# bwvdnbro/CMacIonize

Hardware: AMD Instinct MI355X
Metric: photon packets/sec, 256^3 stromgren (higher is better)
Workload: dtype f64

## Files before the change

### cmacionize_amd/csrc/engine.hip

```cpp
#include "../../include/cmi_gpu.h"

#include "atomic_data.h"
#include "linecooling_data.h"
#include "kernels.h"
#include "dust_kernels.h"
#include "line_image_kernels.h"
#include "line_cube_kernels.h"
#include "sky_image_kernels.h"
#include "sky_cube_kernels.h"
#include "dust_cube_kernels.h"
#include "continuum_kernels.h"
#include "absorbing_cube_kernels.h"
#include "lyman_alpha_kernels.h"
#include "absorption_kernels.h"
#include "sort.h"

#include <algorithm>
#include <climits>
#include <cmath>
#include <cstdarg>
#include <cstdlib>
#include <cstdio>
#include <cstring>
#include <new>
#include <string>
#include <type_traits>
#include <vector>

namespace {

thread_local std::string g_last_error;

int fail(int code, const char *fmt, ...) {
  char buf[512];
  va_list ap;
  va_start(ap, fmt);
  vsnprintf(buf, sizeof buf, fmt, ap);
  va_end(ap);
  g_last_error = buf;
  return code;
}

#define HIP_TRY(expr)                                                          \
  do {                                                                         \
    hipError_t err__ = (expr);                                                 \
    if (err__ != hipSuccess)                                                   \
      return fail(CMI_GPU_EDEVICE, "%s failed: %s (%s:%d)", #expr,             \
                  hipGetErrorString(err__), __FILE__, __LINE__);               \
  } while (0)
#define CMI_TRY(expr)                                                          \
  do {                                                                         \
    const int rc__ = (expr);                                                   \
    if (rc__)                                                                  \
      return rc__;                                                             \
  } while (0)

struct EventPair {
  hipEvent_t start = nullptr, stop = nullptr;
  uint64_t packets = 0;
};

}

struct cmi_gpu_engine {
  cmi_gpu_config config;
  int device = 0;
  hipStream_t stream = nullptr;
  bool own_stream = false;
  int num_cu = 0;

  GridDev grid;
  ModelDev model;
  CellsDev cells_unsettled;
  int64_t ncell = 0;

  double *state_block = nullptr;
  double *acc_block = nullptr;
  bool own_acc = false;
  double2 *opacity = nullptr;
  CountersDev *counters = nullptr;
  TablesDev *tables = nullptr;
  TablesDev *host_tables = nullptr;
  SpectraDev *spectra = nullptr;
  bool spectra_dirty = true;
  double *user_table[4] = {nullptr, nullptr, nullptr, nullptr};
  std::vector<double> user_table_host[4];
  unsigned int *mailbox = nullptr, *mailbox_dev = nullptr;
  double *source_position = nullptr;
  double *source_cumulative = nullptr;
  std::vector<double> source_position_host;
  double discrete_luminosity = 0., continuous_luminosity = 0.;
  bool have_continuous_spectrum = false;

  bool have_sources = false, have_spectrum = false, have_xsec = false,
       have_recomb = false, have_cells = false;
  bool full_ions = false;
  cmi_gpu_temperature_params tparams;

  unsigned int *select_count = nullptr;
  uint32_t *select_ids = nullptr;
  uint64_t select_capacity = 0;
  double *select_rows = nullptr;
  uint64_t select_rows_capacity = 0;
  uint32_t *sort_keys[2] = {nullptr, nullptr};
  uint32_t *sort_ids[2] = {nullptr, nullptr};
  void *sort_temp = nullptr;
  size_t sort_temp_bytes = 0;
  uint64_t sort_capacity = 0;
  uint32_t *span_cursor = nullptr;
#ifdef CMI_EXPERIMENTS
  unsigned long long *phase_clock = nullptr;
  size_t phase_clock_capacity = 0;
  unsigned phase_blocks = 0;
#endif

  double *queue_block = nullptr;
  uint64_t queue_capacity = 0;
  QueueDev ended_queue, ready_queue;
  double *export_rows = nullptr;
  uint64_t export_capacity = 0;
  unsigned int *export_count = nullptr;
  bool own_export_rows = false;
  double *import_rows = nullptr;
  uint64_t import_capacity = 0;
  unsigned int *queue_counts = nullptr;
  char *tile_block = nullptr;
  uint64_t tile_capacity = 0;
  bool tile_has_weights = false;
  FlightRowsDev tile_rows[2];
  uint32_t *tile_iota = nullptr;
  TileItemDev *tile_items = nullptr;
  uint32_t *tile_begin = nullptr;
  uint32_t *tile_blockhist = nullptr, *tile_total = nullptr;
  uint32_t *tile_new_slots = nullptr;
  TrackersDev trackers = {};
  bool trackers_enabled = false;
  EscapeDev escape = {};
  bool escape_counting = false;
  EscapeDev escape_staged = {};
  double *pad_H = nullptr;
  bool pad_valid = false;
  int32_t last_first_build = 0;
  bool last_pad_uniform = false;
  unsigned long long *metal_gate = nullptr;
  bool metals_pending = false;
  bool state_pointer_escaped = false;
  char *temp_pipe_block = nullptr;
  uint32_t temp_pipe_capacity = 0;
  unsigned int *temp_pipe_counts = nullptr;
  uint32_t *tile_ended_slot = nullptr;
  uint32_t *tile_ended_pos = nullptr;
  uint32_t *tile_slot_of[2] = {nullptr, nullptr};
  unsigned int *tile_absorbed_count = nullptr;
  unsigned int *tile_absorbed_before = nullptr;
  unsigned int *tile_counts = nullptr;
  uint64_t tile_rounds_run = 0;
  bool acc_block_dirty = false;

  struct Tuning {
    bool sort_packets = true;
    int sort_tau_bits = -1;
    int sort_dir_bits = -1;
    int class_order = -1;
    int aggregate = CMI_AGG_BLOCK;
    int aggregate_reemit = CMI_AGG_NONE;
    int refill_threshold = CMI_REFILL_THRESHOLD;
    uint32_t chunk = 64;
    int max_blocks_per_cu = 8;
    uint64_t max_packets_per_launch = 1ull << 27;
    int exp_no_atomics = 0;
    bool exact_dda = false;
    bool reemit_passes = true;
    int refill_threshold_reemit = 32;
    int64_t reemit_inline_below = -1;
    int reemit_max_passes = 12;
    bool tile_rounds = true;
    uint64_t tile_min_flights = 100000;
    int tile_min_per_item = -1;
    int tile_refill_threshold = 48;
    bool tile_counting_sort = true;
    bool update_reuse = true;
    bool defer_metals = true;
    bool update_writes_pad = true;
    bool defer_weights = true;
    bool pre_emission = true;
    bool pad_march = true;
    bool pad_uniform = true;
    bool xcd_remap = false;
    bool temperature_pipeline = true;
    uint32_t temperature_finish_slots = 1024;
    int tile_compact_ratio = -1;
    bool park_in_place = true;
    bool span_claim = CMI_SPAN_CLAIM_DEFAULT;
    bool emit_before_flush = CMI_EMIT_BEFORE_FLUSH_DEFAULT;
    bool phase_stamps = false;
    int continuum_channel_block = CMI_CONTINUUM_FB;
    int64_t continuum_launch_rays = 0;
    int absorbing_cube_channel_block = CMI_ABSORBING_CB;
    int absorbing_cube_expm1_call = CMI_ABSORBING_EXPM1_CALL;
    int absorbing_cube_window_skip = 1;
    int64_t absorbing_cube_launch_rays = 0;
    int absorption_slab_rows = 0;
    int absorption_edge_sharing = CMI_ABSORPTION_EDGE_SHARING;
    int absorption_skips = 1;
  } tune;

  DustDev dust = {};
  double dust_kappa = 0.;
  bool have_dust_scattering = false, have_ccd = false, have_dust_source = false;
  double *dust_image = nullptr;
  double *dust_cdf = nullptr;
  double2 *dust_opacity = nullptr;
  DustCountersDev *dust_counters = nullptr;
  bool dust_per_hydrogen = false;
  int dust_source = DUST_SOURCE_GALAXY;
  CellSourceDev cell_source = {};
  double *cell_source_cells = nullptr, *cell_source_blocks = nullptr;
  double *cell_velocities = nullptr;
  std::vector<double> cell_source_blocks_host;
  bool have_cell_source = false, cell_source_from_cells = false;
  uint64_t cells_epoch = 0, cell_source_epoch = 0;
  int dust_camera = DUST_CAMERA_PARALLEL;
  SkyCameraDev sky_camera = {};
  int32_t dust_nviews = 1, dust_probe_view = 0;
  std::vector<DustViewDev> dust_views;
  std::vector<SkyObserverDev> sky_views;
  void *dust_views_dev = nullptr;
  unsigned long long *dust_view_counters = nullptr;
  DustCubeDev dust_cube = {};
  int32_t dust_cube_nviews = 0;
  const char *dust_cube_stale = nullptr;
  int32_t cell_source_line = -1;
  LyaDev lya = {};
  DustDev lya_dust = {};
  int32_t lya_nviews = 0;
  unsigned long long *lya_next = nullptr;
  LyaCountersDev *lya_counters = nullptr;
  const char *lya_stale = nullptr;
  double *lya_field = nullptr;

  bool timing = false;
  unsigned long long *launch_steps = nullptr;
  std::vector<EventPair> shoot_events, update_events, kernel_events;
  std::vector<EventPair> event_pool;
};

namespace {

inline CellsDev &cells_of_iteration(cmi_gpu_engine *e) {
  return e->cells_unsettled;
}
inline const CellsDev &cells_of_iteration(const cmi_gpu_engine *e) {
  return e->cells_unsettled;
}

int settle_metal_fractions(cmi_gpu_engine *e);

template <class T, class N>
int grow(cmi_gpu_engine *e, T *&ptr, N &capacity, N want, size_t bytes) {
  if (capacity >= want)
    return CMI_GPU_OK;
  HIP_TRY(hipStreamSynchronize(e->stream));
  (void)hipFree(ptr);
  ptr = nullptr;
  capacity = 0;
  HIP_TRY(hipMalloc(&ptr, bytes));
  capacity = want;
  return CMI_GPU_OK;
}

#define CMI_MAX_TIMED_LAUNCHES 65536
int timer_begin(cmi_gpu_engine *e, EventPair &ev) {
  ev = EventPair();
  if (!e->timing)
    return CMI_GPU_OK;
  if (!e->event_pool.empty()) {
    ev = e->event_pool.back();
    e->event_pool.pop_back();
  } else {
    HIP_TRY(hipEventCreate(&ev.start));
    hipError_t err = hipEventCreate(&ev.stop);
    if (err != hipSuccess) {
      (void)hipEventDestroy(ev.start);
      HIP_TRY(err);
    }
  }
  hipError_t err = hipEventRecord(ev.start, e->stream);
  if (err != hipSuccess) {
    e->event_pool.push_back(ev);
    HIP_TRY(err);
  }
  return CMI_GPU_OK;
}

__global__ void mailbox_kernel(const unsigned int *src, unsigned int *dst,
                               int n) {
  if ((int)threadIdx.x < n)
    dst[threadIdx.x] = src[threadIdx.x];
}
__global__ void snapshot_steps_kernel(const CountersDev *counters,
                                      unsigned long long *dst) {
  unsigned long long sum = 0;
  for (int k = threadIdx.x; k < CMI_COUNTER_SHARDS; k += 64)
    sum += counters[k].nsteps;
  for (int off = 32; off > 0; off >>= 1)
    sum += __shfl_down(sum, off, 64);
  if (threadIdx.x == 0)
    *dst = sum;
}

__global__ void __launch_bounds__(256)
    counters_sum_kernel(const CountersDev *shards, CountersDev *out) {
  __shared__ CountersDev partial[256];
  CountersDev mine = CountersDev();
  for (int k = threadIdx.x; k < CMI_COUNTER_SHARDS; k += 256) {
    const CountersDev c = shards[k];
// ... 617 lines not shown
  if (config->stream) {
    e->stream = (hipStream_t)config->stream;
  } else {
    HIP_TRY(hipStreamCreateWithFlags(&e->stream, hipStreamNonBlocking));
    e->own_stream = true;
  }

  GridDev &g = e->grid;
  const bool decomposed = config->sub_ncell[0] > 0 || config->sub_ncell[1] > 0 ||
                          config->sub_ncell[2] > 0;
  for (int a = 0; a < 3; ++a) {
    g.anchor[a] = config->anchor[a];
    g.box_sides[a] = config->sides[a];
    g.global_ncell[a] = config->ncell[a];
    g.ncell[a] = decomposed ? config->sub_ncell[a] : config->ncell[a];
    g.offset[a] = decomposed ? config->sub_offset[a] : 0;
    g.global_periodic[a] = config->periodic[a] ? 1 : 0;
    g.periodic[a] = (config->periodic[a] && !decomposed) ? 1 : 0;
    g.cellside[a] = config->sides[a] / config->ncell[a];
    g.inv_cellside[a] = 1. / g.cellside[a];
  }
  g.decomposed = decomposed ? 1 : 0;
  g.copy_rank = 0;
  g.copy_count = 1;
  e->ncell = (int64_t)g.ncell[0] * g.ncell[1] * g.ncell[2];
  g.ncell_total = e->ncell;

  const size_t field_bytes = (size_t)e->ncell * sizeof(double);
  HIP_TRY(hipMalloc(&e->state_block, 16 * field_bytes));
  HIP_TRY(hipMemsetAsync(e->state_block, 0, 16 * field_bytes, e->stream));
  if (config->external_accumulators) {
    e->acc_block = (double *)config->external_accumulators;
  } else {
    HIP_TRY(hipMalloc(&e->acc_block, CMI_NACC * field_bytes));
    e->own_acc = true;
  }
  HIP_TRY(hipMemsetAsync(e->acc_block, 0, CMI_NACC * field_bytes, e->stream));
  HIP_TRY(hipMalloc(&e->opacity, (size_t)e->ncell * sizeof(double2)));
  HIP_TRY(hipMalloc(&e->counters, sizeof(CountersDev) * CMI_COUNTER_SHARDS +
                                      sizeof(EscapeDev)));
  HIP_TRY(hipMemsetAsync(e->counters, 0,
                         sizeof(CountersDev) * CMI_COUNTER_SHARDS +
                             sizeof(EscapeDev),
                         e->stream));
  HIP_TRY(hipMalloc(&e->tables, sizeof(TablesDev)));
  {
    e->host_tables = new TablesDev;
    build_tables(*e->host_tables);
    HIP_TRY(hipMemcpy(e->tables, e->host_tables, sizeof(TablesDev),
                      hipMemcpyHostToDevice));
  }

  CellsDev &c = cells_of_iteration(e);
  c.number_density = e->state_block;
  c.temperature = e->state_block + e->ncell;
  for (int i = 0; i < CMI_NION; ++i)
    c.x[i] = e->state_block + (int64_t)(2 + i) * e->ncell;
  c.acc_base = e->acc_block;
  c.acc_field_stride = e->ncell;
  c.acc_cell_stride = 1;
  c.opacity = e->opacity;

  ModelDev &m = e->model;
  memset(&m, 0, sizeof m);
  m.tables = e->tables;
  m.nu_H = eV_to_Hz(13.6);
  m.nu_He = eV_to_Hz(24.6);
  m.reemit_type = CMI_GPU_REEMIT_NONE;
  m.photon_weight[0] = 1.;
  m.photon_weight[1] = 1.;

  cmi_gpu_temperature_params &tp = e->tparams;
  tp.do_temperature_calculation = 0;
  tp.minimum_number_of_iterations = 3;
  tp.epsilon_convergence = 1.e-3;
  tp.maximum_number_of_iterations = 100;
  tp.pah_heating_factor = 0.;
  tp.cosmic_ray_heating_factor = 0.;
  tp.cosmic_ray_heating_limit = 0.75;
  tp.cosmic_ray_heating_scale_length = 1.33333 * 3.086e19;
  tp.minimum_ionized_temperature = 4000.;
  m.t_epsilon = tp.epsilon_convergence;
  m.t_max_iterations = tp.maximum_number_of_iterations;
  m.crlim = tp.cosmic_ray_heating_limit;
  m.crscale = tp.cosmic_ray_heating_scale_length;
  m.t_min_ionized = tp.minimum_ionized_temperature;

  HIP_TRY(hipStreamSynchronize(e->stream));
  if (const char *env = std::getenv("CMI_GPU_TUNING")) {
    std::string all(env);
    size_t at = 0;
    while (at < all.size()) {
      size_t end = all.find(',', at);
      if (end == std::string::npos)
        end = all.size();
      const std::string item = all.substr(at, end - at);
      const size_t eq = item.find('=');
      if (eq != std::string::npos) {
        const int rc = cmi_gpu_set_tuning(e, item.substr(0, eq).c_str(),
                                          std::atoll(item.c_str() + eq + 1));
        if (rc) {
          cmi_gpu_destroy(e);
          return rc;
        }
      }
      at = end + 1;
    }
  }
  *out = e;
  return CMI_GPU_OK;
}

int cmi_gpu_destroy(cmi_gpu_engine *e) {
  if (!e)
    return CMI_GPU_OK;
  (void)hipSetDevice(e->device);
  (void)hipStreamSynchronize(e->stream);
  release_events(e, e->shoot_events);
  release_events(e, e->update_events);
  release_events(e, e->kernel_events);
  for (auto &p : e->event_pool) {
    (void)hipEventDestroy(p.start);
    (void)hipEventDestroy(p.stop);
  }
  (void)hipFree(e->state_block);
  if (e->own_acc)
    (void)hipFree(e->acc_block);
  (void)hipFree(e->opacity);
  (void)hipFree(e->counters);
  (void)hipFree(e->trackers.counts);
  (void)hipFree(e->trackers.absorption);
  (void)hipFree(e->trackers.flux);
  (void)hipFree(e->escape.sky);
  (void)hipFree(e->temp_pipe_block);
  (void)hipFree(e->pad_H);
  (void)hipFree(e->metal_gate);
  (void)hipFree(e->temp_pipe_counts);
  (void)hipFree(e->tables);
  (void)hipFree(e->spectra);
  for (int k = 0; k < 4; ++k)
    (void)hipFree(e->user_table[k]);
  delete e->host_tables;
  (void)hipFree(e->source_position);
  (void)hipFree(e->source_cumulative);
  (void)hipFree(e->sort_keys[0]);
  (void)hipFree(e->select_count);
  (void)hipFree(e->span_cursor);
#ifdef CMI_EXPERIMENTS
  (void)hipFree(e->phase_clock);
#endif
  (void)hipFree(e->select_ids);
  (void)hipFree(e->select_rows);
  (void)hipFree(e->sort_temp);
  (void)hipFree(e->queue_block);
  (void)hipFree(e->queue_counts);
  if (e->mailbox)
    (void)hipHostFree(e->mailbox);
  (void)hipFree(e->export_count);
  if (e->own_export_rows)
    (void)hipFree(e->export_rows);
  (void)hipFree(e->import_rows);
  (void)hipFree(e->tile_block);
  (void)hipFree(e->tile_counts);
  (void)hipFree(e->launch_steps);
  (void)hipFree(e->dust_image);
  (void)hipFree(e->dust_views_dev);
  (void)hipFree(e->dust_view_counters);
  (void)hipFree(e->dust_cdf);
  (void)hipFree(e->dust_opacity);
  (void)hipFree(e->dust_counters);
  (void)hipFree(e->cell_source_cells);
  (void)hipFree(e->cell_velocities);
  (void)hipFree(const_cast<double *>(e->dust_cube.s2));
  (void)hipFree(const_cast<double *>(e->dust_cube.obs_velocity));
  (void)hipFree(e->dust_cube.cube);
  (void)hipFree(e->cell_source_blocks);
  (void)hipFree(const_cast<LyaRecord *>(e->lya.records));
  (void)hipFree(e->lya.image);
  (void)hipFree(e->lya.cube);
  (void)hipFree(e->lya_next);
  (void)hipFree(e->lya_counters);
  (void)hipFree(e->lya_field);
  if (e->own_stream)
    (void)hipStreamDestroy(e->stream);
  delete e;
  return CMI_GPU_OK;
}

int cmi_gpu_synchronize(cmi_gpu_engine *e) {
  if (!e)
    return fail(CMI_GPU_EINVAL, "null engine");
  HIP_TRY(hipStreamSynchronize(e->stream));
  return CMI_GPU_OK;
}

int64_t cmi_gpu_number_of_cells(const cmi_gpu_engine *e) {
  return e ? e->ncell : -1;
}

static void mix_sources(cmi_gpu_engine *e) {
  ModelDev &m = e->model;
  const double discrete = m.nsource > 0 ? e->discrete_luminosity : 0.;
  const double continuous =
      m.continuous_type != 0 ? e->continuous_luminosity : 0.;
  m.total_luminosity = discrete + continuous;
  m.continuous_probability = 0.;
  m.photon_weight[0] = 1.;
  m.photon_weight[1] = 1.;
  if (m.total_luminosity > 0.) {
    if (discrete > 0.) {
      m.continuous_probability = continuous > 0. ? 0.5 : 0.;
      m.photon_weight[0] = 1.;
      m.photon_weight[1] =
          continuous > 0. ? (1. - m.continuous_probability) * continuous /
                                m.continuous_probability / discrete
                          : 1.;
    } else {
      m.continuous_probability = 1.;
      m.photon_weight[0] = 0.;
      m.photon_weight[1] = 1.;
    }
  }
  e->have_sources = m.total_luminosity > 0.;
}

int cmi_gpu_set_sources(cmi_gpu_engine *e, int32_t n, const double *positions,
                        const double *weights, double total_luminosity) {
  if (!e || n < 0 || (n > 0 && (!positions || !weights)))
    return fail(CMI_GPU_EINVAL, "cmi_gpu_set_sources: bad argument");
  HIP_TRY(hipSetDevice(e->device));
  HIP_TRY(hipStreamSynchronize(e->stream));
  (void)hipFree(e->source_position);
  (void)hipFree(e->source_cumulative);
  e->source_position = nullptr;
  e->source_cumulative = nullptr;
  e->source_position_host.clear();
  e->model.nsource = 0;
  e->model.source_position = nullptr;
  e->model.source_cumulative = nullptr;
  e->discrete_luminosity = 0.;
  if (n == 0) {
    mix_sources(e);
    return CMI_GPU_OK;
  }
  std::vector<double> cumulative(n);
  for (int i = 0; i < n; ++i)
    cumulative[i] = (i > 0 ? cumulative[i - 1] : 0.) + weights[i];
  if (std::abs(cumulative.back() - 1.) > 1.e-9) {
    mix_sources(e);
    return fail(CMI_GPU_EINVAL,
                "Discrete source weights do not sum to 1.0 (%g)!",
                cumulative.back());
  }
  cumulative.back() = 1.;
  HIP_TRY(hipMalloc(&e->source_position, sizeof(double) * 3 * n));
  HIP_TRY(hipMalloc(&e->source_cumulative, sizeof(double) * n));
  HIP_TRY(hipMemcpy(e->source_position, positions, sizeof(double) * 3 * n,
                    hipMemcpyHostToDevice));
  HIP_TRY(hipMemcpy(e->source_cumulative, cumulative.data(),
                    sizeof(double) * n, hipMemcpyHostToDevice));
  e->source_position_host.assign(positions, positions + 3 * (size_t)n);
  e->model.nsource = n;
  e->model.source_position = e->source_position;
  e->model.source_cumulative = e->source_cumulative;
  e->discrete_luminosity = total_luminosity;
  mix_sources(e);
  return CMI_GPU_OK;
}

int cmi_gpu_set_continuous_source(cmi_gpu_engine *e, int32_t type,
                                  double luminosity) {
  if (!e || (type != CMI_GPU_CONTINUOUS_NONE &&
             type != CMI_GPU_CONTINUOUS_ISOTROPIC) ||
      (type != CMI_GPU_CONTINUOUS_NONE && !(luminosity > 0.)))
    return fail(CMI_GPU_EINVAL, "cmi_gpu_set_continuous_source: bad argument");
  e->model.continuous_type = type;
  e->continuous_luminosity = type != CMI_GPU_CONTINUOUS_NONE ? luminosity : 0.;
  e->spectra_dirty = true;
  mix_sources(e);
  return CMI_GPU_OK;
}

int cmi_gpu_set_continuous_source_planar(cmi_gpu_engine *e, int32_t axis,
                                         double intercept,
                                         const double *anchor,
                                         const double *sides,
                                         double luminosity) {
  if (!e || axis < 0 || axis > 2 || !anchor || !sides || !(sides[0] > 0.) ||
      !(sides[1] > 0.) || !(luminosity > 0.))
    return fail(CMI_GPU_EINVAL,
                "cmi_gpu_set_continuous_source_planar: bad argument");
  ModelDev &m = e->model;
  m.continuous_type = CMI_GPU_CONTINUOUS_PLANAR;
  m.continuous_axis = axis;
  m.continuous_intercept = intercept;
  for (int k = 0; k < 2; ++k) {
    m.continuous_anchor[k] = anchor[k];
    m.continuous_side[k] = sides[k];
  }
  e->continuous_luminosity = luminosity;
  e->spectra_dirty = true;
  mix_sources(e);
  return CMI_GPU_OK;
}

int cmi_gpu_set_continuous_spectrum_monochromatic(cmi_gpu_engine *e,
// ... 200 lines not shown
  m.t_min_ionized = params->minimum_ionized_temperature;
  return CMI_GPU_OK;
}

int cmi_gpu_upload_cells(cmi_gpu_engine *e, const double *number_density,
                         const double *temperature,
                         const double *ionic_fractions) {
  if (!e || !number_density || !temperature)
    return fail(CMI_GPU_EINVAL, "upload_cells: bad argument");
  HIP_TRY(hipSetDevice(e->device));
  ++e->cells_epoch;
  CellsDev *cells;
  CMI_TRY(cells_settled(e, cells));
  const size_t bytes = (size_t)e->ncell * sizeof(double);
  HIP_TRY(hipMemcpyAsync(cells->number_density, number_density, bytes,
                         hipMemcpyHostToDevice, e->stream));
  HIP_TRY(hipMemcpyAsync(cells->temperature, temperature, bytes,
                         hipMemcpyHostToDevice, e->stream));
  if (ionic_fractions) {
    HIP_TRY(hipMemcpyAsync(cells->x[0], ionic_fractions, CMI_NION * bytes,
                           hipMemcpyHostToDevice, e->stream));
  } else {
    HIP_TRY(hipMemsetAsync(cells->x[0], 0, CMI_NION * bytes, e->stream));
  }
  CMI_TRY(rebuild_opacity(e));
  HIP_TRY(hipStreamSynchronize(e->stream));
  e->have_cells = true;
  return CMI_GPU_OK;
}

int cmi_gpu_upload_field(cmi_gpu_engine *e, int32_t field,
                         const double *values) {
  if (!e || !values)
    return fail(CMI_GPU_EINVAL, "upload_field: bad argument");
  double *dst = field_pointer(e, field);
  if (!dst)
    return fail(CMI_GPU_EINVAL, "upload_field: unknown field %d", field);
  HIP_TRY(hipSetDevice(e->device));
  if (field < CMI_GPU_FIELD_MEAN_INTENSITY) {
    ++e->cells_epoch;
    CMI_TRY(settle_metal_fractions(e));
  }
  const int64_t stride = field_stride(e, field);
  if (stride == 1) {
    HIP_TRY(hipMemcpyAsync(dst, values, (size_t)e->ncell * sizeof(double),
                           hipMemcpyHostToDevice, e->stream));
  } else {
    double *tmp = nullptr;
    HIP_TRY(hipMalloc(&tmp, (size_t)e->ncell * sizeof(double)));
    hipError_t err = hipMemcpyAsync(tmp, values,
                                    (size_t)e->ncell * sizeof(double),
                                    hipMemcpyHostToDevice, e->stream);
    if (err == hipSuccess) {
      scatter_strided_kernel<<<grid_blocks(e, e->ncell, 8), CMI_BLOCK, 0,
                               e->stream>>>(tmp, dst, stride, e->ncell);
      err = hipGetLastError();
    }
    if (err == hipSuccess)
      err = hipStreamSynchronize(e->stream);
    (void)hipFree(tmp);
    HIP_TRY(err);
  }
  if (field >= CMI_GPU_FIELD_MEAN_INTENSITY)
    e->acc_block_dirty = true;
  if (field == CMI_GPU_FIELD_NUMBER_DENSITY ||
      field == CMI_GPU_FIELD_IONIC_FRACTION + ION_H_n ||
      field == CMI_GPU_FIELD_IONIC_FRACTION + ION_He_n) {
    CMI_TRY(rebuild_opacity(e));
  }
  HIP_TRY(hipStreamSynchronize(e->stream));
  return CMI_GPU_OK;
}

int cmi_gpu_download_field(cmi_gpu_engine *e, int32_t field, double *values) {
  if (!e || !values)
    return fail(CMI_GPU_EINVAL, "download_field: bad argument");
  double *src = field_pointer(e, field);
  if (!src)
    return fail(CMI_GPU_EINVAL, "download_field: unknown field %d", field);
  HIP_TRY(hipSetDevice(e->device));
  if (field >= CMI_GPU_FIELD_IONIC_FRACTION + ION_C_p1 &&
      field < CMI_GPU_FIELD_MEAN_INTENSITY)
    CMI_TRY(settle_metal_fractions(e));
  const int64_t stride = field_stride(e, field);
  if (stride == 1) {
    HIP_TRY(hipMemcpyAsync(values, src, (size_t)e->ncell * sizeof(double),
                           hipMemcpyDeviceToHost, e->stream));
    HIP_TRY(hipStreamSynchronize(e->stream));
  } else {
    double *tmp = nullptr;
    HIP_TRY(hipMalloc(&tmp, (size_t)e->ncell * sizeof(double)));
    gather_strided_kernel<<<grid_blocks(e, e->ncell, 8), CMI_BLOCK, 0,
                            e->stream>>>(src, stride, tmp, e->ncell);
    hipError_t err = hipGetLastError();
    if (err == hipSuccess)
      err = hipMemcpyAsync(values, tmp, (size_t)e->ncell * sizeof(double),
                           hipMemcpyDeviceToHost, e->stream);
    if (err == hipSuccess)
      err = hipStreamSynchronize(e->stream);
    (void)hipFree(tmp);
    HIP_TRY(err);
  }
  return CMI_GPU_OK;
}

int cmi_gpu_accumulator_layout(cmi_gpu_engine *e, int64_t *field_stride_out,
                               int64_t *cell_stride_out) {
  if (!e)
    return fail(CMI_GPU_EINVAL, "null engine");
  if (field_stride_out)
    *field_stride_out = cells_of_iteration(e).acc_field_stride;
  if (cell_stride_out)
    *cell_stride_out = cells_of_iteration(e).acc_cell_stride;
  return CMI_GPU_OK;
}

void *cmi_gpu_field_device_pointer(cmi_gpu_engine *e, int32_t field) {
  if (!e)
    return nullptr;
  if (field >= 0 && field < CMI_GPU_FIELD_MEAN_INTENSITY) {
    if (settle_metal_fractions(e) != CMI_GPU_OK)
      return nullptr;
    e->state_pointer_escaped = true;
  }
  return field_pointer(e, field);
}

int cmi_gpu_get_update_state(cmi_gpu_engine *e, int32_t *metals_pending,
                             int32_t *pad_records_valid,
                             int32_t *deferral_allowed) {
  if (!e)
    return fail(CMI_GPU_EINVAL, "null engine");
  if (metals_pending)
    *metals_pending = e->metals_pending ? 1 : 0;
  if (pad_records_valid)
    *pad_records_valid = e->pad_valid ? 1 : 0;
  if (deferral_allowed)
    *deferral_allowed =
        (e->tune.defer_metals && !e->state_pointer_escaped) ? 1 : 0;
  return CMI_GPU_OK;
}

int cmi_gpu_get_transport_plan(cmi_gpu_engine *e, int32_t *first_build,
                               int32_t *uniform_weight) {
  if (!e)
    return fail(CMI_GPU_EINVAL, "null engine");
  if (first_build)
    *first_build = e->last_first_build;
  if (uniform_weight)
    *uniform_weight = e->last_pad_uniform ? 1 : 0;
  return CMI_GPU_OK;
}

int cmi_gpu_reset_grid(cmi_gpu_engine *e) {
  if (!e)
    return fail(CMI_GPU_EINVAL, "null engine");
  HIP_TRY(hipSetDevice(e->device));
  const size_t field_bytes = (size_t)e->ncell * sizeof(double);
  if (e->full_ions || e->acc_block_dirty) {
    HIP_TRY(hipMemsetAsync(e->acc_block, 0, CMI_NACC * field_bytes,
                           e->stream));
    e->acc_block_dirty = false;
  } else {
    HIP_TRY(hipMemsetAsync(e->acc_block, 0, field_bytes, e->stream));
    if (e->config.track_heating)
      HIP_TRY(hipMemsetAsync(e->acc_block + (size_t)CMI_NION * e->ncell, 0,
                             2 * field_bytes, e->stream));
  }
  HIP_TRY(hipMemsetAsync(e->counters, 0,
                         sizeof(CountersDev) * CMI_COUNTER_SHARDS, e->stream));
  return CMI_GPU_OK;
}

int cmi_gpu_set_tuning(cmi_gpu_engine *e, const char *key, int64_t value) {
  if (!e || !key)
    return fail(CMI_GPU_EINVAL, "set_tuning: bad argument");
  const std::string k(key);
  if (k == "sort_packets")
    e->tune.sort_packets = value != 0;
  else if (k == "sort_dir_bits")
    e->tune.sort_dir_bits =
        (int)(value < 0 ? -1 : (value < 2 ? 2 : (value > 22 ? 22 : value)));
  else if (k == "sort_tau_bits")
    e->tune.sort_tau_bits = (int)(value < 0 ? -1 : (value > 3 ? 3 : value));
  else if (k == "class_order")
    e->tune.class_order = (int)(value < 0 ? -1 : (value != 0 ? 1 : 0));
  else if (k == "aggregate")
    e->tune.aggregate = (int)(value < 0 ? 0 : (value > 2 ? 2 : value));
  else if (k == "aggregate_reemit")
    e->tune.aggregate_reemit = (int)(value < 0 ? 0 : (value > 2 ? 2 : value));
  else if (k == "refill_threshold")
    e->tune.refill_threshold = (int)(value < 1 ? 1 : (value > 64 ? 64 : value));
  else if (k == "chunk")
    e->tune.chunk = (uint32_t)(value < 64 ? 64 : value);
  else if (k == "max_blocks_per_cu")
    e->tune.max_blocks_per_cu = (int)(value < 1 ? 1 : value);
  else if (k == "max_packets_per_launch")
    e->tune.max_packets_per_launch =
        (uint64_t)(value < 1024 ? 1024 : (value > (1ll << 30) ? (1ll << 30) : value));
  else if (k == "exp_no_atomics")
    e->tune.exp_no_atomics = (int)value;
  else if (k == "exact_dda")
    e->tune.exact_dda = value != 0;
  else if (k == "reemit_passes")
    e->tune.reemit_passes = value != 0;
  else if (k == "refill_threshold_reemit")
    e->tune.refill_threshold_reemit =
        (int)(value < 1 ? 1 : (value > 64 ? 64 : value));
  else if (k == "reemit_inline_below")
    e->tune.reemit_inline_below = value < 0 ? -1 : value;
  else if (k == "reemit_max_passes")
    e->tune.reemit_max_passes = (int)(value < 1 ? 1 : value);
  else if (k == "timing")
    e->timing = value != 0;
  else if (k == "tile_rounds")
    e->tune.tile_rounds = value != 0;
  else if (k == "tile_min_flights")
    e->tune.tile_min_flights = (uint64_t)(value < 0 ? 0 : value);
  else if (k == "tile_min_per_item")
    e->tune.tile_min_per_item = (int)(value < 0 ? -1 : value);
  else if (k == "tile_refill_threshold")
    e->tune.tile_refill_threshold =
        (int)(value < 1 ? 1 : (value > 64 ? 64 : value));
  else if (k == "tile_compact_ratio")
    e->tune.tile_compact_ratio = (int)(value < -1 ? -1 : value);
  else if (k == "park_in_place")
    e->tune.park_in_place = value != 0;
  else if (k == "accumulators_dirty")
    e->acc_block_dirty = e->acc_block_dirty || value != 0;
  else if (k == "temperature_finish_slots")
    e->tune.temperature_finish_slots = (uint32_t)(value < 0 ? 0 : value);
  else if (k == "temperature_pipeline")
    e->tune.temperature_pipeline = value != 0;
  else if (k == "pad_march")
    e->tune.pad_march = value != 0;
  else if (k == "pad_uniform")
    e->tune.pad_uniform = value != 0;
  else if (k == "xcd_remap")
    e->tune.xcd_remap = value != 0;
  else if (k == "pre_emission")
    e->tune.pre_emission = value != 0;
  else if (k == "defer_weights")
    e->tune.defer_weights = value != 0;
  else if (k == "tile_counting_sort")
    e->tune.tile_counting_sort = value != 0;
  else if (k == "update_reuse")
    e->tune.update_reuse = value != 0;
  else if (k == "defer_metals")
    e->tune.defer_metals = value != 0;
  else if (k == "update_writes_pad")
    e->tune.update_writes_pad = value != 0;
  else if (k == "span_claim")
    e->tune.span_claim = value != 0;
  else if (k == "emit_before_flush")
    e->tune.emit_before_flush = value != 0;
  else if (k == "phase_stamps")
    e->tune.phase_stamps = value != 0;
  else if (k == "continuum_channel_block") {
    if (value != 4 && value != 8 && value != 16)
      return fail(CMI_GPU_EINVAL, "set_tuning: continuum_channel_block is 4, "
                  "8 or 16 (%lld asked for)", (long long)value);
    e->tune.continuum_channel_block = (int)value;
  } else if (k == "continuum_launch_rays")
    e->tune.continuum_launch_rays = value < 0 ? 0 : value;
  else if (k == "absorbing_cube_channel_block") {
    if (value != 4 && value != 8)
      return fail(CMI_GPU_EINVAL, "set_tuning: absorbing_cube_channel_block "
                  "is 4 or 8 (%lld asked for)", (long long)value);
    e->tune.absorbing_cube_channel_block = (int)value;
  } else if (k == "absorbing_cube_expm1_call")
    e->tune.absorbing_cube_expm1_call = value != 0;
  else if (k == "absorbing_cube_window_skip")
    e->tune.absorbing_cube_window_skip = value != 0;
  else if (k == "absorbing_cube_launch_rays")
    e->tune.absorbing_cube_launch_rays = value < 0 ? 0 : value;
  else if (k == "absorption_slab_rows") {
    if (value != 0 && value != 1 && value != 2 && value != 4)
      return fail(CMI_GPU_EINVAL, "set_tuning: absorption_slab_rows is 1, 2 "
                  "or 4, or 0 for the default (%lld asked for)",
                  (long long)value);
    e->tune.absorption_slab_rows = (int)value;
  } else if (k == "absorption_edge_sharing")
    e->tune.absorption_edge_sharing = value != 0;
  else if (k == "absorption_skips")
    e->tune.absorption_skips = value != 0;
  else
    return fail(CMI_GPU_EINVAL, "set_tuning: unknown key '%s'", key);
  return CMI_GPU_OK;
}

__global__ void iota_kernel(uint32_t *out, uint64_t n) {
  const uint64_t stride = (uint64_t)gridDim.x * blockDim.x;
  for (uint64_t i = (uint64_t)blockIdx.x * blockDim.x + threadIdx.x; i < n;
       i += stride)
    out[i] = (uint32_t)i;
}

static int read_counters(cmi_gpu_engine *e, const unsigned int *src, int n,
                         unsigned int *out) {
  CMI_TRY(ensure_mailbox(e));
  mailbox_kernel<<<1, 16, 0, e->stream>>>(src, e->mailbox_dev, n);
  HIP_TRY(hipGetLastError());
  HIP_TRY(hipStreamSynchronize(e->stream));
  for (int k = 0; k < n; ++k)
    out[k] = ((volatile unsigned int *)e->mailbox)[k];
  return CMI_GPU_OK;
}

#include "transport_driver.h"

int cmi_gpu_shoot(cmi_gpu_engine *e, uint32_t seed, uint32_t iteration,
                  uint64_t first_packet, uint64_t n_packets) {
  return shoot_impl(e, seed, iteration, first_packet, n_packets, nullptr);
}

int cmi_gpu_shoot_flights(cmi_gpu_engine *e, uint32_t seed, uint32_t iteration,
                          uint64_t first_packet, const void *flights,
                          uint64_t n_flights) {
  if (!e || (!flights && n_flights))
    return fail(CMI_GPU_EINVAL, "shoot_flights: bad argument");
  if (!e->grid.decomposed)
    return fail(CMI_GPU_ESTATE,
                "shoot_flights: the engine is not a block of a decomposed "
                "grid");
  return shoot_impl(e, seed, iteration, first_packet, n_flights,
                    (const double *)flights);
}

int cmi_gpu_set_export_buffer(cmi_gpu_engine *e, void *rows,
                              uint64_t capacity) {
  if (!e || capacity >= (1ull << 32))
    return fail(CMI_GPU_EINVAL, "set_export_buffer: bad argument");
  HIP_TRY(hipSetDevice(e->device));
  HIP_TRY(hipStreamSynchronize(e->stream));
  if (!e->export_count)
    HIP_TRY(hipMalloc(&e->export_count, sizeof(unsigned int)));
  HIP_TRY(hipMemsetAsync(e->export_count, 0, sizeof(unsigned int), e->stream));
  if (e->own_export_rows) {
    (void)hipFree(e->export_rows);
    e->own_export_rows = false;
  }
  e->export_rows = (double *)rows;
  if (!rows && capacity) {
    HIP_TRY(hipMalloc(&e->export_rows,
                      sizeof(double) * CMI_FLIGHT_DOUBLES * capacity));
    e->own_export_rows = true;
  }
  e->export_capacity = capacity;
  return CMI_GPU_OK;
}

int cmi_gpu_get_export_count(cmi_gpu_engine *e, uint64_t *count) {
  if (!e || !count)
    return fail(CMI_GPU_EINVAL, "get_export_count: bad argument");
  *count = 0;
  if (!e->export_count)
    return CMI_GPU_OK;
  HIP_TRY(hipSetDevice(e->device));
  unsigned int n = 0;
  HIP_TRY(hipMemcpyAsync(&n, e->export_count, sizeof n, hipMemcpyDeviceToHost,
                         e->stream));
  HIP_TRY(hipStreamSynchronize(e->stream));
  if (n > e->export_capacity)
    return fail(CMI_GPU_ENOMEM,
                "export buffer overflow: %u flights left the block, room for "
                "%llu - flights were lost, the iteration is invalid",
                n, (unsigned long long)e->export_capacity);
  *count = n;
  return CMI_GPU_OK;
}

int cmi_gpu_download_exports(cmi_gpu_engine *e, double *host_rows,
                             uint64_t capacity, uint64_t *count) {
  if (!e || !count || (!host_rows && capacity))
    return fail(CMI_GPU_EINVAL, "download_exports: bad argument");
  uint64_t n = 0;
  CMI_TRY(cmi_gpu_get_export_count(e, &n));
  *count = n;
  if (n > capacity)
    return fail(CMI_GPU_ENOMEM,
                "download_exports: %llu flights, room for %llu",
                (unsigned long long)n, (unsigned long long)capacity);
  if (n) {
    HIP_TRY(hipMemcpyAsync(host_rows, e->export_rows,
                           sizeof(double) * CMI_FLIGHT_DOUBLES * n,
                           hipMemcpyDeviceToHost, e->stream));
    HIP_TRY(hipStreamSynchronize(e->stream));
  }
  return CMI_GPU_OK;
}

int cmi_gpu_shoot_flights_host(cmi_gpu_engine *e, uint32_t seed,
                               uint32_t iteration, uint64_t first_packet,
                               const double *host_rows, uint64_t n_flights) {
  if (!e || (!host_rows && n_flights))
    return fail(CMI_GPU_EINVAL, "shoot_flights_host: bad argument");
  if (n_flights == 0)
    return CMI_GPU_OK;
  HIP_TRY(hipSetDevice(e->device));
  CMI_TRY(grow(e, e->import_rows, e->import_capacity, n_flights,
               sizeof(double) * CMI_FLIGHT_DOUBLES * n_flights));
  HIP_TRY(hipStreamSynchronize(e->stream));
  HIP_TRY(hipMemcpyAsync(e->import_rows, host_rows,
                         sizeof(double) * CMI_FLIGHT_DOUBLES * n_flights,
                         hipMemcpyHostToDevice, e->stream));
  return cmi_gpu_shoot_flights(e, seed, iteration, first_packet, e->import_rows,
                               n_flights);
}

int cmi_gpu_reset_exports(cmi_gpu_engine *e) {
  if (!e)
    return fail(CMI_GPU_EINVAL, "null engine");
  if (!e->export_count)
    return CMI_GPU_OK;
  HIP_TRY(hipSetDevice(e->device));
  HIP_TRY(hipMemsetAsync(e->export_count, 0, sizeof(unsigned int), e->stream));
  return CMI_GPU_OK;
}

int cmi_gpu_get_counters(cmi_gpu_engine *e, double *totweight,
                         double *typecount, uint64_t *nsteps) {
  if (!e)
    return fail(CMI_GPU_EINVAL, "null engine");
  HIP_TRY(hipSetDevice(e->device));
  CountersDev host;
  CMI_TRY(download_counters(e, host));
  if (totweight)
    *totweight = host.totweight;
  if (typecount)
    for (int i = 0; i < 4; ++i)
      typecount[i] = host.typecount[i];
  if (nsteps)
    *nsteps = host.nsteps;
  return CMI_GPU_OK;
}

int cmi_gpu_get_atomic_count(cmi_gpu_engine *e, uint64_t *natomics) {
  if (!e || !natomics)
    return fail(CMI_GPU_EINVAL, "get_atomic_count: bad argument");
  HIP_TRY(hipSetDevice(e->device));
  CountersDev host;
  CMI_TRY(download_counters(e, host));
  *natomics = host.natomics;
  return CMI_GPU_OK;
}

int cmi_gpu_get_phase_clocks(cmi_gpu_engine *e, uint64_t *out,
                             int64_t capacity, int64_t *count) {
  if (!e || !count || capacity < 0 || (!out && capacity))
    return fail(CMI_GPU_EINVAL, "get_phase_clocks: bad argument");
#ifdef CMI_EXPERIMENTS
  if (!e->phase_clock || !e->phase_blocks)
    return fail(CMI_GPU_ESTATE,
                "get_phase_clocks: no launch with phase_stamps yet");
  HIP_TRY(hipSetDevice(e->device));
  HIP_TRY(hipStreamSynchronize(e->stream));
  const int64_t n = CMI_PHASE_COUNT + 1 + (int64_t)e->phase_blocks;
  *count = n;
  if (capacity)
    HIP_TRY(hipMemcpy(out, e->phase_clock,
                      sizeof(uint64_t) * (size_t)(capacity < n ? capacity : n),
                      hipMemcpyDeviceToHost));
  return CMI_GPU_OK;
#else
  return fail(CMI_GPU_ESTATE,
              "get_phase_clocks: not a build with -DCMI_EXPERIMENTS");
#endif
}
// ... 886 lines not shown
```

### cmacionize_amd/csrc/kernels.h

```cpp
#ifndef CMI_KERNELS_H
#define CMI_KERNELS_H

#include "device_transport.h"
#include "device_reemit.h"
#include "device_thermal.h"
#include "device_emissivity.h"

#ifndef CMI_BLOCK
#define CMI_BLOCK 256
#endif
#ifdef CMI_EXPERIMENTS
#define CMI_EXP(a) ((a).exp_no_atomics)
#else
#define CMI_EXP(a) 0
#endif
#ifndef CMI_TABLE_BITS
#define CMI_TABLE_BITS 10
#endif
#define CMI_TABLE_SLOTS (1 << CMI_TABLE_BITS)
#ifndef CMI_TABLE_BLOCK
#define CMI_TABLE_BLOCK 512
#endif
#ifndef CMI_TABLE_BLOCK_BITS
#define CMI_TABLE_BLOCK_BITS 11
// ... 2333 lines not shown
      continue;
    float s;
    if (t.shell <= t.ninn || nu >= t.einn) {
      const float y = (float)(nu * t.A_E_0_inv);
      s = (float)t.A_sigma_0 * ((y - 1.f) * (y - 1.f) + (float)t.A_y_w_sq) *
          __powf(y, (float)t.A_Plconst) *
          __powf(1.f + sqrtf(y * (float)t.A_y_a_inv), -(float)t.A_P);
    } else {
      const float x = (float)(nu * t.B_E_0_inv - t.B_y_0);
      const float y = sqrtf(x * x + (float)t.B_y_1_sq);
      s = (float)t.B_sigma_0 * ((x - 1.f) * (x - 1.f) + (float)t.B_y_w_sq) *
          __powf(y, 0.5f * (float)t.B_P - 5.5f) *
          __powf(1.f + sqrtf(y * (float)t.B_y_a_inv), -(float)t.B_P);
    }
    sum += (t.ion == ION_H_n) ? s : (float)m.abundance[0] * s;
  }
  return sum;
}

__device__ __forceinline__ uint32_t key_class_field(const KeyArgs &a,
                                                    uint32_t hi,
                                                    uint32_t tau_class) {
  const uint32_t top = (1u << a.tau_bits) - 1u;
  return tau_class ^ ((a.class_order != 0u && (hi & 1u) != 0u) ? top : 0u);
}

#ifndef CMI_KEY_WAVES
#define CMI_KEY_WAVES 3
#endif
template <int TRIPS>
__device__ __forceinline__ void
order_by_verner_class(const uint32_t (&cls)[TRIPS], unsigned int n,
                      uint32_t *s_count ,
                      uint16_t *order) {
  if (threadIdx.x < CMI_VERNER_NCLASS)
    s_count[threadIdx.x] = 0;
  __syncthreads();
#pragma unroll
  for (int k = 0; k < TRIPS; ++k)
    if ((unsigned int)k * CMI_BLOCK + threadIdx.x < n)
      atomicAdd(&s_count[cls[k]], 1u);
  __syncthreads();
  if (threadIdx.x == 0) {
    uint32_t at = 0;
    for (int c = 0; c < CMI_VERNER_NCLASS; ++c) {
      const uint32_t here = s_count[c];
      s_count[c] = at;
      at += here;
    }
  }
  __syncthreads();
#pragma unroll
  for (int k = 0; k < TRIPS; ++k) {
    const unsigned int local = (unsigned int)k * CMI_BLOCK + threadIdx.x;
    if (local < n)
      order[atomicAdd(&s_count[cls[k]], 1u)] = (uint16_t)local;
  }
  __syncthreads();
}

#ifndef CMI_KEY_BATCH
#define CMI_KEY_BATCH 8
#endif
__device__ __forceinline__ void
direction_key_batches(const KeyArgs &a) {
  constexpr int TRIPS = CMI_KEY_BATCH;
  constexpr unsigned int BATCH = TRIPS * CMI_BLOCK;
  __shared__ double s_nu[BATCH], s_tau[BATCH];
  __shared__ uint32_t s_src[BATCH], s_morton[BATCH];
  __shared__ uint16_t s_order[BATCH];
  __shared__ uint32_t s_count[CMI_VERNER_NCLASS];
  const uint32_t lo_bits = a.dir_bits - a.dir_hi_bits;
  const uint64_t stride = (uint64_t)gridDim.x * BATCH;
  const PacketOrigin from(a.model);
  for (uint64_t base = (uint64_t)blockIdx.x * BATCH; base < a.n_packets;
       base += stride) {
    const unsigned int n = a.n_packets - base < BATCH
                               ? (unsigned int)(a.n_packets - base)
                               : BATCH;
    uint32_t cls[TRIPS];
#pragma unroll
    for (int k = 0; k < TRIPS; ++k) {
      const unsigned int local = (unsigned int)k * CMI_BLOCK + threadIdx.x;
      cls[k] = 0;
      if (local >= n)
        continue;
      PacketRng rng;
      const uint64_t id =
          a.select ? (uint64_t)a.select[base + local] : base + local;
      rng.init(a.seed, a.iteration, a.first_packet + id);
      uint32_t src;
      const uint32_t origin = from.draw(a.model, rng, src);
      if (origin != 0) {
        (void)rng.next();
        (void)rng.next();
        if (a.model.continuous_type == 1)
          (void)rng.next();
      }
      const double u_cost = rng.next();
      const double u_phi = rng.next();
      const uint32_t ic = (uint32_t)(u_cost * 2048.);
      const uint32_t ip = (uint32_t)(u_phi * 2048.);
      const double nu = sample_source_spectrum(a.model, rng, origin);
      s_nu[local] = nu;
      s_tau[local] = -log(rng.next());
      s_src[local] = src;
      s_morton[local] = (spread_bits_11(ic) | (spread_bits_11(ip) << 1)) >>
                        (22u - a.dir_bits);
      cls[k] = verner_class(a.model, nu);
    }
    order_by_verner_class<TRIPS>(cls, n, s_count, s_order);
    for (unsigned int j = threadIdx.x; j < n; j += CMI_BLOCK) {
      const unsigned int local = s_order[j];
      const uint64_t i = base + local;
      Packet<true> q;
      double weights[CMI_NACC];
      q.nu = s_nu[local];
      set_cross_sections<true>(a.model, q, weights);
      const double tau = s_tau[local];
      weights[CMI_NION] = q.nu;
      weights[CMI_NION + 1] = tau;
      const uint32_t id = a.select ? a.select[i] : (uint32_t)i;
      double4 *row =
          reinterpret_cast<double4 *>(a.pre_rows + (size_t)CMI_NACC * id);
#pragma unroll
      for (int k = 0; k < CMI_NACC; k += 4)
        row[k >> 2] = make_double4(weights[k], weights[k + 1], weights[k + 2],
                                   weights[k + 3]);
      uint32_t tau_class = 0;
      if (a.tau_bits != 0) {
        const double range = tau * a.sigma_ref / (q.sigma_H + q.sigma_He_corr);
        const int octave = (int)floor(log2(range)) + (1 << (a.tau_bits - 1));
        const int top = (1 << a.tau_bits) - 1;
        tau_class = (uint32_t)(octave < 0 ? 0 : (octave > top ? top : octave));
      }
      const uint32_t morton = s_morton[local];
      const uint32_t hi = morton >> lo_bits;
      const uint32_t lo = morton & ((1u << lo_bits) - 1u);
      a.keys[i] = ((s_src[local] & a.source_mask)
                   << (a.dir_bits + a.tau_bits)) |
                  (hi << (a.tau_bits + lo_bits)) |
                  (key_class_field(a, hi, tau_class) << lo_bits) | lo;
      a.ids[i] = id;
    }
    __syncthreads();
  }
}

__global__ void __launch_bounds__(CMI_BLOCK, CMI_KEY_WAVES)
    emission_key_kernel(const KeyArgs a) {
  direction_key_batches(a);
}

__global__ void __launch_bounds__(CMI_BLOCK, 5)
    direction_key_kernel(const KeyArgs a) {
  const uint64_t stride = (uint64_t)gridDim.x * blockDim.x;
  const uint32_t lo_bits = a.dir_bits - a.dir_hi_bits;
  const PacketOrigin from(a.model);
  for (uint64_t i = (uint64_t)blockIdx.x * blockDim.x + threadIdx.x;
       i < a.n_packets; i += stride) {
    PacketRng rng;
    const uint64_t id = a.select ? (uint64_t)a.select[i] : i;
    rng.init(a.seed, a.iteration, a.first_packet + id);
    uint32_t src;
    const uint32_t origin = from.draw(a.model, rng, src);
    if (origin != 0) {
      (void)rng.next();
      (void)rng.next();
      if (a.model.continuous_type == 1)
        (void)rng.next();
    }
    const double u_cost = rng.next();
    const double u_phi = rng.next();
    const uint32_t ic = (uint32_t)(u_cost * 2048.);
    const uint32_t ip = (uint32_t)(u_phi * 2048.);
    const uint32_t morton =
        (spread_bits_11(ic) | (spread_bits_11(ip) << 1)) >> (22u - a.dir_bits);
    uint32_t tau_class = 0;
    if (a.tau_bits != 0) {
      if (!a.full_ions) {
        (void)sample_source_spectrum(a.model, rng, origin);
        const double u_tau = rng.next();
        tau_class = (uint32_t)(u_tau * (double)(1u << a.tau_bits));
      } else {
        const double nu = sample_source_spectrum(a.model, rng, origin);
        const double tau = -log(rng.next());
        const float sigma = approximate_opacity_cross_section(a.model, nu);
        const float range = (float)(tau * a.sigma_ref) / sigma;
        const int octave = (int)floorf(log2f(range)) + (1 << (a.tau_bits - 1));
        const int top = (1 << a.tau_bits) - 1;
        tau_class = (uint32_t)(octave < 0 ? 0 : (octave > top ? top : octave));
      }
    }
    const uint32_t hi = morton >> lo_bits;
    const uint32_t lo = morton & ((1u << lo_bits) - 1u);
    a.keys[i] = ((src & a.source_mask) << (a.dir_bits + a.tau_bits)) |
                (hi << (a.tau_bits + lo_bits)) |
                (key_class_field(a, hi, tau_class) << lo_bits) | lo;
    a.ids[i] = (uint32_t)id;
  }
}


struct UpdateArgs {
  GridDev grid;
  ModelDev model;
  CellsDev cells;
  double jfac;
  double hfac;
  int64_t first, count;
};

#ifndef CMI_IONIZATION_WAVES
#define CMI_IONIZATION_WAVES 4
#endif
template <bool FULL, bool HEATING>
__device__ __forceinline__ void
ionization_load_cell(const UpdateArgs &a, int64_t c, double (&J)[CMI_NION],
                     double (&heating)[2]) {
  if (FULL) {
#pragma unroll
    for (int i = 0; i < CMI_NION; ++i)
      J[i] = (*acc_at(a.cells, i, c));
  } else {
    J[0] = (*acc_at(a.cells, 0, c));
#pragma unroll
    for (int i = 1; i < CMI_NION; ++i)
      J[i] = 0.;
  }
  heating[0] = HEATING ? (*acc_at(a.cells, CMI_NION, c)) : 0.;
  heating[1] = HEATING ? (*acc_at(a.cells, CMI_NION + 1, c)) : 0.;
}
template <bool HEATING, class Terms>
__device__ __forceinline__ void
ionization_update_cell(const UpdateArgs &a, int64_t c, double ntot, double T,
                       const double (&J)[CMI_NION], double (&heating)[2],
                       const Terms &terms) {
  double x[CMI_NION];
  cmi_ionization_state_cell_from(a.model, terms, a.jfac, a.hfac, ntot, T, J,
                                 heating, x);
#pragma unroll
  for (int i = 0; i < CMI_NION; ++i)
    a.cells.x[i][c] = x[i];
  if (HEATING) {
    (*acc_at(a.cells, CMI_NION, c)) = heating[0];
    (*acc_at(a.cells, CMI_NION + 1, c)) = heating[1];
  }
  a.cells.opacity[c] = (ntot > 0.)
                           ? make_double2(ntot * x[ION_H_n], ntot * x[ION_He_n])
                           : make_double2(-1., 0.);
}

template <bool FULL, bool HEATING = true>
__global__ void __launch_bounds__(CMI_BLOCK, FULL ? 2 : CMI_IONIZATION_WAVES)
    ionization_kernel(const UpdateArgs a) {
  const int64_t stride = (int64_t)gridDim.x * blockDim.x;
  for (int64_t c = a.first + (int64_t)blockIdx.x * blockDim.x + threadIdx.x;
       c < a.first + a.count; c += stride) {
    const double ntot = a.cells.number_density[c];
    const double T = a.cells.temperature[c];
    double J[CMI_NION], heating[2];
    ionization_load_cell<FULL, HEATING>(a, c, J, heating);
    const MetalTermsEvaluated terms = {a.model, T, T * 1.e-4};
    ionization_update_cell<HEATING>(a, c, ntot, T, J, heating, terms);
  }
}

#ifndef CMI_UPDATE_CHUNK_ROWS
#define CMI_UPDATE_CHUNK_ROWS 8
#endif
template <bool FULL, bool HEATING>
__global__ void __launch_bounds__(CMI_BLOCK, CMI_IONIZATION_WAVES)
    ionization_kernel(const UpdateArgs a, const int reuse) {
  static_assert(!FULL, "the reuse path is the hydrogen-only update's");
  constexpr int WAVES = CMI_BLOCK / 64;
  __shared__ MetalTerms s_terms[WAVES];
  const int wave_in_block =
      __builtin_amdgcn_readfirstlane((int)(threadIdx.x >> 6));
  MetalTerms &stored = s_terms[wave_in_block];
  const int64_t rows = (a.count + 63) >> 6;
  const int64_t chunks =
      (rows + CMI_UPDATE_CHUNK_ROWS - 1) / CMI_UPDATE_CHUNK_ROWS;
  const int64_t nwaves = (int64_t)gridDim.x * WAVES;
  const int64_t end = a.first + a.count;
  unsigned long long stored_for = 0;
  bool have = false;
  for (int64_t chunk = (int64_t)blockIdx.x * WAVES + wave_in_block;
       chunk < chunks; chunk += nwaves) {
    for (int64_t row = chunk * CMI_UPDATE_CHUNK_ROWS;
         row < (chunk + 1) * CMI_UPDATE_CHUNK_ROWS && row < rows; ++row) {
      const int64_t c = a.first + (row << 6) + (int64_t)(threadIdx.x & 63u);
      if (c >= end)
        continue;
      const double ntot = a.cells.number_density[c];
      const double T = a.cells.temperature[c];
      double J[CMI_NION], heating[2];
      ionization_load_cell<FULL, HEATING>(a, c, J, heating);
      const unsigned long long bits =
          (unsigned long long)__double_as_longlong(T);
      const unsigned long long first =
          ((unsigned long long)__builtin_amdgcn_readfirstlane(
               (uint32_t)(bits >> 32))
           << 32) |
          __builtin_amdgcn_readfirstlane((uint32_t)bits);
      bool use_stored = false;
      if (reuse != 0 && wave_ballot(bits != first) == 0ull) {
        if (!(have && stored_for == first) &&
            wave_ballot(a.jfac * J[ION_H_n] > 0. && ntot > 0.) != 0ull) {
          cmi_metal_terms(a.model, T, stored);
          __builtin_amdgcn_fence(__ATOMIC_RELEASE, "wavefront");
          __builtin_amdgcn_wave_barrier();
          __builtin_amdgcn_fence(__ATOMIC_ACQUIRE, "wavefront");
          stored_for = first;
          have = true;
        }
        use_stored = have && stored_for == first;
      }
      if (use_stored) {
        const MetalTermsStored terms = {&stored};
        ionization_update_cell<HEATING>(a, c, ntot, T, J, heating, terms);
      } else {
        const MetalTermsEvaluated terms = {a.model, T, T * 1.e-4};
        ionization_update_cell<HEATING>(a, c, ntot, T, J, heating, terms);
      }
    }
  }
}

struct HydrogenUpdateArgs {
  UpdateArgs u;
  unsigned long long *gate;
  double *pad_H;
  double pad_sigma;
  uint32_t ny, nz;
};

#ifndef CMI_HYDROGEN_UPDATE_WAVES
#define CMI_HYDROGEN_UPDATE_WAVES 4
#endif
template <bool HEATING>
__global__ void __launch_bounds__(CMI_BLOCK, CMI_HYDROGEN_UPDATE_WAVES)
    hydrogen_update_kernel(const HydrogenUpdateArgs h) {
  constexpr int WAVES = CMI_BLOCK / 64;
  const UpdateArgs &a = h.u;
  const int64_t rows = (a.count + 63) >> 6;
  const int64_t nwaves = (int64_t)gridDim.x * WAVES;
  const uint32_t lane = threadIdx.x & 63u;
  for (int64_t row = (int64_t)blockIdx.x * WAVES + (threadIdx.x >> 6);
       row < rows; row += nwaves) {
    const int64_t c = (row << 6) + (int64_t)lane;
    bool gate = false;
    if (c < a.count) {
      const double ntot = a.cells.number_density[c];
      const double T = a.cells.temperature[c];
// ... 433 lines not shown
```

### cmacionize_amd/csrc/transport_driver.h

```cpp
#ifndef CMI_TRANSPORT_DRIVER_H
#define CMI_TRANSPORT_DRIVER_H

static int reserve_sort_buffers(cmi_gpu_engine *e, uint64_t n) {
  if (e->sort_capacity >= n)
    return CMI_GPU_OK;
  HIP_TRY(hipStreamSynchronize(e->stream));
  (void)hipFree(e->sort_keys[0]);
  (void)hipFree(e->sort_temp);
  e->sort_keys[0] = nullptr;
  e->sort_temp = nullptr;
  e->sort_capacity = 0;
  uint32_t *block = nullptr;
  HIP_TRY(hipMalloc(&block, sizeof(uint32_t) * 4 * n));
  e->sort_keys[0] = block;
  e->sort_keys[1] = block + n;
  e->sort_ids[0] = block + 2 * n;
  e->sort_ids[1] = block + 3 * n;
  size_t bytes = 0;
  HIP_TRY(cmi_sort_pairs_temp_bytes(n, 32, &bytes));
  e->sort_temp_bytes = bytes;
  HIP_TRY(hipMalloc(&e->sort_temp, bytes ? bytes : 16));
  e->sort_capacity = n;
  return CMI_GPU_OK;
}

static int reserve_queues(cmi_gpu_engine *e, uint64_t n) {
  if (e->queue_capacity >= n)
    return CMI_GPU_OK;
  const size_t ended_doubles = 6, ready_doubles = 9;
  CMI_TRY(grow(e, e->queue_block, e->queue_capacity, n,
               sizeof(double) * (ended_doubles + ready_doubles) * n));
  if (!e->queue_counts) {
    HIP_TRY(hipMalloc(&e->queue_counts, 2 * sizeof(unsigned int)));
  }
  QueueDev &q = e->ended_queue;
  double *base = e->queue_block;
  for (int a = 0; a < 3; ++a) {
    q.pos[a] = base + (size_t)a * n;
    q.dir[a] = nullptr;
  }
  q.tau = nullptr;
  q.nu = base + (size_t)3 * n;
  q.cell = (int32_t *)(base + (size_t)4 * n);
  q.id = (uint32_t *)q.cell + n;
  q.meta = q.id + n;
  q.count = e->queue_counts;
  QueueDev &r = e->ready_queue;
  base = e->queue_block + ended_doubles * n;
  for (int a = 0; a < 3; ++a) {
    r.pos[a] = base + (size_t)a * n;
    r.dir[a] = base + (size_t)(3 + a) * n;
  }
  r.tau = base + (size_t)6 * n;
  r.nu = base + (size_t)7 * n;
  r.cell = nullptr;
  r.id = (uint32_t *)(base + (size_t)8 * n);
  r.meta = r.id + n;
  r.count = e->queue_counts + 1;
  return CMI_GPU_OK;
}

static TileGridDev tile_grid(const cmi_gpu_engine *e) {
  TileGridDev t;
  const bool heat = e->config.track_heating != 0;
  if (e->full_ions) {
    t.log2[0] = TileShape<true, true>::LX;
    t.log2[1] = TileShape<true, true>::LY;
    t.log2[2] = TileShape<true, true>::LZ;
  } else if (heat) {
    t.log2[0] = TileShape<false, true>::LX;
    t.log2[1] = TileShape<false, true>::LY;
    t.log2[2] = TileShape<false, true>::LZ;
  } else {
    t.log2[0] = TileShape<false, false>::LX;
    t.log2[1] = TileShape<false, false>::LY;
    t.log2[2] = TileShape<false, false>::LZ;
  }
  int64_t total = 1;
  for (int a = 0; a < 3; ++a) {
    const int side = 1 << t.log2[a];
    t.ntile[a] = (e->grid.ncell[a] + side - 1) / side;
    total *= t.ntile[a];
  }
  t.ntiles = (int32_t)total;
  return t;
}

static int reserve_tile_buffers(cmi_gpu_engine *e, uint64_t n) {
  const bool weights = e->full_ions;
  if (e->tile_capacity >= n && (e->tile_has_weights || !weights))
    return CMI_GPU_OK;
  HIP_TRY(hipStreamSynchronize(e->stream));
  (void)hipFree(e->tile_block);
  e->tile_block = nullptr;
  e->tile_capacity = 0;
  const TileGridDev t = tile_grid(e);
  const size_t row_bytes = sizeof(double) * CMI_FLIGHT_DOUBLES * n;
  const size_t weight_bytes = weights ? sizeof(double) * CMI_NACC * n : 0;
  const size_t key_bytes = (sizeof(uint32_t) * n + 255) & ~(size_t)255;
  const size_t nitems =
      (size_t)t.ntiles + n / CMI_TILE_ITEM_FLIGHTS_FULL + 4;
  const size_t item_bytes = sizeof(TileItemDev) * nitems;
  const size_t begin_bytes =
      (sizeof(uint32_t) * ((size_t)t.ntiles + 2) + 255) & ~(size_t)255;
  const size_t count_bytes =
      (sizeof(unsigned int) * nitems + 255) & ~(size_t)255;
  const bool counting = t.ntiles <= CMI_TILE_SORT_MAX_TILES;
  const size_t hist_bytes =
      counting ? sizeof(uint32_t) * (size_t)t.ntiles * CMI_TILE_SORT_BLOCKS : 0;
  const size_t total = 2 * (row_bytes + weight_bytes + key_bytes) +
                       6 * key_bytes + 2 * begin_bytes + 2 * count_bytes +
                       item_bytes + hist_bytes;
  HIP_TRY(hipMalloc(&e->tile_block, total));
  if (!e->tile_counts)
    HIP_TRY(hipMalloc(&e->tile_counts, 8 * sizeof(unsigned int)));
  char *at = e->tile_block;
  for (int k = 0; k < 2; ++k) {
    FlightRowsDev &r = e->tile_rows[k];
    r.rows = (double *)at;
    at += row_bytes;
    r.weights = weights ? (double *)at : nullptr;
    at += weight_bytes;
    r.keys = (uint32_t *)at;
    at += key_bytes;
    r.count = e->tile_counts + k;
    r.capacity = (unsigned int)n;
  }
  e->tile_iota = (uint32_t *)at;
  at += key_bytes;
  e->tile_ended_slot = (uint32_t *)at;
  at += key_bytes;
  e->tile_ended_pos = (uint32_t *)at;
  at += key_bytes;
  for (int k = 0; k < 2; ++k) {
    e->tile_slot_of[k] = (uint32_t *)at;
    at += key_bytes;
  }
  e->tile_new_slots = (uint32_t *)at;
  at += key_bytes;
  e->tile_begin = (uint32_t *)at;
  at += begin_bytes;
  e->tile_total = counting ? (uint32_t *)at : nullptr;
  at += begin_bytes;
  e->tile_absorbed_count = (unsigned int *)at;
  at += count_bytes;
  e->tile_absorbed_before = (unsigned int *)at;
  at += count_bytes;
  e->tile_items = (TileItemDev *)at;
  at += item_bytes;
  e->tile_blockhist = counting ? (uint32_t *)at : nullptr;
  iota_kernel<<<grid_blocks(e, (int64_t)n, 8), CMI_BLOCK, 0, e->stream>>>(
      e->tile_iota, n);
  HIP_TRY(hipGetLastError());
  e->tile_capacity = n;
  e->tile_has_weights = weights;
  return CMI_GPU_OK;
}

static bool block_emits_nothing(const cmi_gpu_engine *e) {
  if (e->model.continuous_type != 0)
    return false;
  const GridDev &g = e->grid;
  const bool at_origin = (g.offset[0] | g.offset[1] | g.offset[2]) == 0;
  for (int32_t s = 0; s < e->model.nsource; ++s) {
    bool near = true, in_grid = true;
    for (int a = 0; a < 3; ++a) {
      const double x = e->source_position_host[3 * (size_t)s + a];
      const double lo = g.anchor[a] + g.cellside[a] * (g.offset[a] - 1);
      const double hi =
          g.anchor[a] + g.cellside[a] * (g.offset[a] + g.ncell[a] + 1);
      near &= (x >= lo && x <= hi);
      in_grid &= (x >= g.anchor[a] + g.cellside[a] &&
                  x <= g.anchor[a] + g.box_sides[a] - g.cellside[a]);
    }
    if (near || (!in_grid && at_origin))
      return false;
  }
  return e->model.nsource > 0;
}

static uint64_t reemit_inline_below(const cmi_gpu_engine *e) {
  if (e->tune.reemit_inline_below >= 0)
    return (uint64_t)e->tune.reemit_inline_below;
  return e->grid.decomposed ? 262144u : 4096u;
}

typedef void (*ShootKernel)(const ShootArgs);
typedef void (*TileKernel)(const TileArgs);

enum FirstBuild {
  FIRST_GENERIC,
  FIRST_TABLE,
  FIRST_PAD,
  FIRST_PAD_BIG,
  FIRST_PRE
};

struct LaunchPlan {
  bool heat, reemit;
  bool exact;
  bool tracking;
  bool passes;
  bool tiles;
  bool sorted;
  bool select_mode;
  int agg, agg_reemit;
  FirstBuild first;
  bool pad, pad_big;
  bool pad_uniform;
  double uniform_scale;
  int64_t padded_cells;
  ShootKernel kernel, kernel_inline, kernel_first;
  int blocks_per_cu, blocks_per_cu_inline, blocks_per_cu_first;
  int first_threads;
  uint32_t tau_bits, source_bits, dir_bits;
  int key_bits;
  double sigma_ref;
  TileKernel tile_kernel;
  int tile_threads, tile_blocks_per_cu;
};

static ShootKernel shoot_build(bool full, bool heat, bool reemit, bool exact,
                               bool track, FirstBuild first,
                               bool uniform = false) {
  static const ShootKernel generic[2][4][2] = {
      {{shoot_kernel<false, false, false, false>,
        shoot_kernel<false, false, true, false>},
       {shoot_kernel<false, true, false, false>,
        shoot_kernel<false, true, true, false>},
       {shoot_kernel<true, false, false, false>,
        shoot_kernel<true, false, true, false>},
       {shoot_kernel<true, true, false, false>,
        shoot_kernel<true, true, true, false>}},
      {{shoot_kernel<false, false, false, true>,
        shoot_kernel<false, false, true, true>},
       {shoot_kernel<false, true, false, true>,
        shoot_kernel<false, true, true, true>},
       {shoot_kernel<true, false, false, true>,
        shoot_kernel<true, false, true, true>},
       {shoot_kernel<true, true, false, true>,
        shoot_kernel<true, true, true, true>}}};
  static const ShootKernel tracked[4][2] = {
      {shoot_kernel<false, false, false, false, false, false, false, true>,
       shoot_kernel<false, false, true, false, false, false, false, true>},
      {shoot_kernel<false, true, false, false, false, false, false, true>,
       shoot_kernel<false, true, true, false, false, false, false, true>},
      {shoot_kernel<true, false, false, false, false, false, false, true>,
       shoot_kernel<true, false, true, false, false, false, false, true>},
      {shoot_kernel<true, true, false, false, false, false, false, true>,
       shoot_kernel<true, true, true, false, false, false, false, true>}};
  static const ShootKernel table[2][2] = {
      {shoot_kernel<true, true, false, false, true>,
       shoot_kernel<true, false, false, false, true>},
      {shoot_kernel<false, true, false, false, true>,
       shoot_kernel<false, false, false, false, true>}};
  static const ShootKernel pad_big[3] = {
      shoot_kernel<false, true, false, false, true, false, true, false, true>,
      shoot_kernel<false, false, false, false, true, false, true, false, true>,
      shoot_kernel<false, false, false, false, true, false, true, true, true>};
  static const ShootKernel pad[3] = {
      shoot_kernel<false, true, false, false, true, false, true>,
      shoot_kernel<false, false, false, false, true, false, true>,
      shoot_kernel<false, false, false, false, true, false, true, true>};
  static const ShootKernel pre[2] = {
      shoot_kernel<true, true, false, false, true, true>,
      shoot_kernel<true, false, false, false, true, true>};
  switch (first) {
  case FIRST_TABLE:
    return table[!full][!heat];
  case FIRST_PAD:
    return pad[!heat + (!heat && uniform)];
  case FIRST_PAD_BIG:
    return pad_big[!heat + (!heat && uniform)];
  case FIRST_PRE:
    return pre[!heat];
  case FIRST_GENERIC:
    break;
  }
  return track ? tracked[2 * full + heat][reemit]
               : generic[exact][2 * full + heat][reemit];
}

extern "C++" {
template <class Kernel>
static int blocks_per_cu_of(Kernel kernel, int threads, int most, int &out) {
  out = 0;
  HIP_TRY(hipOccupancyMaxActiveBlocksPerMultiprocessor(&out, kernel, threads,
                                                       0));
  if (out < 1)
    out = 1;
  if (out > most)
    out = most;
  return CMI_GPU_OK;
}
}

static int plan_launches(cmi_gpu_engine *e, uint64_t n_packets,
                         const double *flights, LaunchPlan &p) {
  const cmi_gpu_engine::Tuning &tune = e->tune;
  p.heat = e->config.track_heating != 0;
  p.reemit = e->model.reemit_type != CMI_GPU_REEMIT_NONE;
  const bool small_grid = e->ncell < CMI_FAST_MARCHER_MAX_CELLS;
  p.agg = small_grid ? tune.aggregate : CMI_AGG_NONE;
  p.agg_reemit = small_grid ? tune.aggregate_reemit : CMI_AGG_NONE;
  p.tracking = e->trackers_enabled &&
               (e->trackers.n != 0 || e->escape.sky != nullptr);
  p.exact = tune.exact_dda || !small_grid ||
            (p.tracking && !e->grid.decomposed);
  p.passes = p.reemit && tune.reemit_passes &&
             !(flights && n_packets < reemit_inline_below(e));
  p.sorted = tune.sort_packets && !flights;
  p.tiles = p.passes && tune.tile_rounds && !p.exact && !p.tracking;
  p.select_mode = p.sorted && e->grid.decomposed;

  const bool table =
      !flights && !p.exact && !p.tracking && p.agg == CMI_AGG_BLOCK &&
      (p.passes || !p.reemit) &&
      !(e->grid.periodic[0] | e->grid.periodic[1] | e->grid.periodic[2]);
  p.padded_cells = ((int64_t)e->grid.ncell[0] + 2 * CMI_PAD_LAYERS) *
                   ((int64_t)e->grid.ncell[1] + 2 * CMI_PAD_LAYERS) *
                   ((int64_t)e->grid.ncell[2] + 2 * CMI_PAD_LAYERS);
  const double sigma_H = e->model.xsec_fixed[ION_H_n];
  p.pad = table && !e->full_ions && tune.pad_march &&
          p.padded_cells < ((int64_t)1 << 29) && sigma_H >= 0. &&
          std::isfinite(sigma_H);
  p.pad_big = p.pad && e->ncell > CMI_TABLE_BIG_CELLS;
  const double pc = e->model.continuous_probability;
  const double *pw = e->model.photon_weight;
  p.pad_uniform = p.pad && !p.heat && tune.pad_uniform &&
                  (pc <= 0. || pc >= 1. || pw[0] == pw[1]);
  p.uniform_scale = (pc >= 1. ? pw[1] : pw[0]) * sigma_H;
  p.first = FIRST_GENERIC;
  if (p.pad)
    p.first = p.pad_big ? FIRST_PAD_BIG : FIRST_PAD;
  else if (table && e->full_ions && tune.pre_emission && p.sorted &&
           p.tiles)
    p.first = FIRST_PRE;
  else if (table)
    p.first = FIRST_TABLE;
  p.first_threads = (table && !e->full_ions)
                        ? (p.pad_big ? shoot_block_threads<false, true, true>()
                                     : shoot_block_threads<false, true>())
                        : CMI_BLOCK;

  const bool track = p.tracking && !p.exact;
  p.kernel_inline =
      shoot_build(e->full_ions, p.heat, true, p.exact, track, FIRST_GENERIC);
  p.kernel = (p.reemit && !p.passes)
                 ? p.kernel_inline
                 : shoot_build(e->full_ions, p.heat, false, p.exact, track,
                               FIRST_GENERIC);
  p.kernel_first = table ? shoot_build(e->full_ions, p.heat, false, false,
                                       false, p.first, p.pad_uniform)
                         : p.kernel;
  CMI_TRY(blocks_per_cu_of(p.kernel, CMI_BLOCK, tune.max_blocks_per_cu,
                           p.blocks_per_cu));
  CMI_TRY(blocks_per_cu_of(p.kernel_inline, CMI_BLOCK, tune.max_blocks_per_cu,
                           p.blocks_per_cu_inline));
  p.blocks_per_cu_first = p.blocks_per_cu;
  if (table)
    CMI_TRY(blocks_per_cu_of(p.kernel_first, p.first_threads,
                             tune.max_blocks_per_cu, p.blocks_per_cu_first));
  p.tile_kernel = nullptr;
  p.tile_threads = p.tile_blocks_per_cu = 0;
  if (p.tiles) {
    if (e->full_ions)
      p.tile_kernel =
          p.heat ? tile_kernel<true, true> : tile_kernel<true, false>;
    else
      p.tile_kernel =
          p.heat ? tile_kernel<false, true> : tile_kernel<false, false>;
    p.tile_threads = e->full_ions
                         ? TileShape<true, true>::THREADS
                         : (p.heat ? TileShape<false, true>::THREADS
                                   : TileShape<false, false>::THREADS);
    CMI_TRY(blocks_per_cu_of(p.tile_kernel, p.tile_threads, INT_MAX,
                             p.tile_blocks_per_cu));
  }

  const uint64_t max_launch = tune.max_packets_per_launch;
  const uint64_t per_source =
      (n_packets < max_launch ? n_packets : max_launch) /
      (uint64_t)(e->model.nsource > 0 ? e->model.nsource : 1);
  if (tune.sort_tau_bits >= 0)
    p.tau_bits = (uint32_t)tune.sort_tau_bits;
  else
    p.tau_bits = per_source >= (1ull << 24)
                     ? (e->full_ions ? 2u : 3u)
                     : (per_source >= (1ull << 22) ? 2u : 0u);
  p.sigma_ref = 1.;
  if (e->full_ions) {
    double sigma_He;
    const ModelDev host_model = host_model_of(e);
    cmi_cross_sections_H_He(host_model, 1.0001 * e->model.nu_H, p.sigma_ref,
                            sigma_He);
  }
  p.source_bits = 0;
  for (int s = e->model.nsource - (e->model.continuous_type != 0 ? 0 : 1);
       s > 0; s >>= 1)
    ++p.source_bits;
  if (p.source_bits > 10u - p.tau_bits)
    p.source_bits = 10u - p.tau_bits;
  p.dir_bits = 22u;
  if (tune.sort_dir_bits >= 0) {
    p.dir_bits = (uint32_t)tune.sort_dir_bits;
  } else {
    const uint32_t over = (22u + p.tau_bits + p.source_bits) % 8u;
    if (over == 1u || over == 2u)
      p.dir_bits = 22u - over;
  }
  p.key_bits = (int)(p.dir_bits + p.tau_bits + p.source_bits);
  return CMI_GPU_OK;
}

static int reserve_for(cmi_gpu_engine *e, const LaunchPlan &p, uint64_t cap) {
  if (!e->span_cursor)
    HIP_TRY(hipMalloc(&e->span_cursor, sizeof(uint32_t) * CMI_SPAN_CURSORS));
  if (p.sorted || p.tiles)
    CMI_TRY(reserve_sort_buffers(e, cap));
  if (p.passes)
    CMI_TRY(reserve_queues(e, cap));
  if (p.tiles)
    CMI_TRY(reserve_tile_buffers(e, cap));
  return CMI_GPU_OK;
}

static unsigned transport_blocks(const cmi_gpu_engine *e, uint64_t n,
                                 uint32_t chunk, int blocks_per_cu,
                                 int threads) {
  const uint64_t nchunks = (n + chunk - 1) / chunk;
  int64_t blocks = (int64_t)e->num_cu * blocks_per_cu;
  const int64_t need =
      (int64_t)((nchunks + (threads / 64) - 1) / (threads / 64));
  if (blocks > need)
    blocks = need;
  if (blocks < 1)
    blocks = 1;
  return (unsigned)blocks;
}

static QueueDev no_queue() {
  QueueDev q;
  memset(&q, 0, sizeof q);
  return q;
}

static int publish_escape(cmi_gpu_engine *e, bool count) {
  count = count && e->escape.sky != nullptr;
  if (count == e->escape_counting)
    return CMI_GPU_OK;
  e->escape_staged = e->escape;
  if (!count)
    e->escape_staged.sky = nullptr;
  HIP_TRY(hipMemcpyAsync(cmi_escape_of(e->counters), &e->escape_staged,
                         sizeof(EscapeDev), hipMemcpyHostToDevice,
                         e->stream));
  HIP_TRY(hipStreamSynchronize(e->stream));
  e->escape_counting = count;
  return CMI_GPU_OK;
}

static ShootArgs shoot_args(const cmi_gpu_engine *e, const LaunchPlan &p,
                            uint32_t seed, uint32_t iteration,
                            uint64_t first_packet, uint64_t done,
                            uint64_t nids, const double *flights) {
  ShootArgs a;
  a.grid = e->grid;
  a.model = e->model;
  a.cells = cells_of_iteration(e);
  a.counters = e->counters;
  a.first_packet = first_packet;
  a.batch_offset = done;
  a.n_packets = nids;
  a.order = nullptr;
  a.pre_rows = nullptr;
  a.xin = flights ? flights + (size_t)CMI_FLIGHT_DOUBLES * done : nullptr;
  a.xin_local = 0;
  a.xout.rows = e->export_rows;
  a.xout.count = e->export_count;
  a.xout.capacity = (unsigned int)e->export_capacity;
  a.pad_H = p.pad ? e->pad_H : nullptr;
  a.uniform_scale = p.uniform_scale;
  a.xcd_remap = (p.sorted && e->tune.xcd_remap) ? 1 : 0;
  a.pad_ny = e->grid.ncell[1] + 2 * CMI_PAD_LAYERS;
  a.pad_nz = e->grid.ncell[2] + 2 * CMI_PAD_LAYERS;
  a.pad_inv_yz = 1. / ((double)a.pad_ny * (double)a.pad_nz);
  a.pad_inv_z = 1. / (double)a.pad_nz;
  a.chunk = e->tune.chunk;
  a.seed = seed;
  a.iteration = iteration;
  a.refill_threshold = flights ? e->tune.refill_threshold_reemit
                               : e->tune.refill_threshold;
  a.exp_no_atomics = e->tune.exp_no_atomics;
  a.trackers = e->trackers;
  if (!p.tracking)
    a.trackers.n = 0;
  a.aggregate = flights ? p.agg_reemit : p.agg;
  a.qin = no_queue();
  a.qout = no_queue();
  a.park_in_place = 0;
  a.span_cursor = nullptr;
  a.n_spans = 0;
  a.span_claim = 0;
  a.emit_before_flush = e->tune.emit_before_flush ? 1 : 0;
#ifdef CMI_EXPERIMENTS
  a.phase_clock = nullptr;
#endif
  return a;
}

static int pad_records(cmi_gpu_engine *e, const LaunchPlan &p) {
  if (e->pad_valid)
    return CMI_GPU_OK;
  const GridDev &g = e->grid;
  if (!e->pad_H)
    HIP_TRY(hipMalloc(&e->pad_H, sizeof(double) * (size_t)p.padded_cells));
  pad_record_kernel<<<grid_blocks(e, p.padded_cells, 8), CMI_BLOCK, 0,
                      e->stream>>>(cells_of_iteration(e).opacity, e->pad_H,
                                   e->model.xsec_fixed[ION_H_n], g.ncell[0],
                                   g.ncell[1], g.ncell[2]);
  HIP_TRY(hipGetLastError());
  e->pad_valid = true;
  return CMI_GPU_OK;
}

static int select_block_packets(cmi_gpu_engine *e, ShootArgs &a,
                                const uint32_t **select) {
  const uint64_t nids = a.n_packets;
  if (!e->select_count)
    HIP_TRY(hipMalloc(&e->select_count, sizeof(unsigned int)));
  CMI_TRY(grow(e, e->select_ids, e->select_capacity, nids,
               sizeof(uint32_t) * nids));
  HIP_TRY(hipMemsetAsync(e->select_count, 0, sizeof(unsigned int),
                         e->stream));
  SelectArgs sa;
  sa.grid = e->grid;
  sa.model = e->model;
  sa.first_packet = a.first_packet + a.batch_offset;
  sa.batch_offset = a.batch_offset;
  sa.n_packets = nids;
  sa.seed = a.seed;
  sa.iteration = a.iteration;
  sa.select = e->select_ids;
  sa.count = e->select_count;
  block_select_kernel<false>
      <<<grid_blocks(e, (int64_t)nids, 8), CMI_BLOCK, 0, e->stream>>>(sa);
  HIP_TRY(hipGetLastError());
  unsigned int mine = 0;
  CMI_TRY(read_counters(e, e->select_count, 1, &mine));
  a.n_packets = mine;
  *select = e->select_ids;
  return CMI_GPU_OK;
}

static int open_ended_queue(cmi_gpu_engine *e, ShootArgs &a) {
  HIP_TRY(hipMemsetAsync(e->queue_counts, 0, 2 * sizeof(unsigned int),
                         e->stream));
  a.qout = e->ended_queue;
  if (!a.xin && e->tune.park_in_place) {
    a.park_in_place = 1;
    HIP_TRY(hipMemsetAsync(e->ended_queue.id, 0xff,
                           sizeof(uint32_t) * (size_t)a.n_packets, e->stream));
  }
  return CMI_GPU_OK;
}

static int order_packets(cmi_gpu_engine *e, const LaunchPlan &p, ShootArgs &a,
                         uint64_t nids, const uint32_t *select) {
  const uint64_t n = a.n_packets;
  KeyArgs k;
  k.model = e->model;
  k.first_packet = a.first_packet + a.batch_offset;
  k.n_packets = n;
  k.seed = a.seed;
  k.iteration = a.iteration;
  k.tau_bits = p.tau_bits;
  k.class_order =
      e->tune.class_order >= 0
          ? (uint32_t)e->tune.class_order
          : (e->full_ions ? CMI_CLASS_ORDER_FULL_DEFAULT
                          : CMI_CLASS_ORDER_DEFAULT);
  k.full_ions = e->full_ions ? 1 : 0;
  k.sigma_ref = p.sigma_ref;
  k.source_mask = (1u << p.source_bits) - 1u;
  k.dir_hi_bits = 0;
  k.dir_bits = p.dir_bits;
  if (p.tau_bits != 0) {
    const uint64_t per_bin = 64ull << p.tau_bits;
    const uint64_t per_source =
        nids / (uint64_t)(e->model.nsource > 0 ? e->model.nsource : 1);
    while (k.dir_hi_bits < p.dir_bits &&
           (per_source >> (k.dir_hi_bits + 1u)) >= per_bin)
      ++k.dir_hi_bits;
  }
  k.keys = e->sort_keys[0];
  k.ids = e->sort_ids[0];
  k.pre_rows = p.first == FIRST_PRE ? e->tile_rows[1].weights : nullptr;
  if (p.first == FIRST_PRE && select) {
    CMI_TRY(grow(e, e->select_rows, e->select_rows_capacity, nids,
                 sizeof(double) * CMI_NACC * (size_t)nids));
    k.pre_rows = e->select_rows;
  }
  k.select = select;
  a.pre_rows = k.pre_rows;
  if (k.pre_rows)
    emission_key_kernel<<<grid_blocks(e, (int64_t)n, 8), CMI_BLOCK, 0,
                          e->stream>>>(k);
  else
    direction_key_kernel<<<grid_blocks(e, (int64_t)n, 8), CMI_BLOCK, 0,
                           e->stream>>>(k);
  HIP_TRY(hipGetLastError());
  HIP_TRY(cmi_sort_pairs(e->sort_temp, e->sort_temp_bytes, e->sort_keys[0],
                         e->sort_keys[1], e->sort_ids[0], e->sort_ids[1], n,
                         p.key_bits, e->stream));
  a.order = e->sort_ids[1];
  return CMI_GPU_OK;
}

static int launch_first_generation(cmi_gpu_engine *e, const LaunchPlan &p,
                                   const ShootArgs &args) {
  ShootArgs a = args;
  const unsigned blocks = transport_blocks(
      e, a.n_packets, a.chunk, p.blocks_per_cu_first, p.first_threads);
  if (e->tune.span_claim) {
    HIP_TRY(hipMemsetAsync(e->span_cursor, 0,
                           sizeof(uint32_t) * CMI_SPAN_CURSORS, e->stream));
    const uint64_t span = (uint64_t)(p.first_threads / 64) * a.chunk;
    a.span_cursor = e->span_cursor;
    a.n_spans = (uint32_t)((a.n_packets + span - 1) / span);
    a.span_claim = 1;
  }
#ifdef CMI_EXPERIMENTS
  if (e->tune.phase_stamps) {
    const size_t words = CMI_PHASE_COUNT + 1 + (size_t)blocks;
    if (e->phase_clock_capacity < words) {
      (void)hipFree(e->phase_clock);
      e->phase_clock = nullptr;
      e->phase_clock_capacity = 0;
      HIP_TRY(hipMalloc(&e->phase_clock, sizeof(unsigned long long) * words));
      e->phase_clock_capacity = words;
    }
    HIP_TRY(hipMemsetAsync(e->phase_clock, 0,
                           sizeof(unsigned long long) * words, e->stream));
    HIP_TRY(hipMemsetAsync(e->phase_clock + CMI_PHASE_COUNT, 0xff,
                           sizeof(unsigned long long), e->stream));
    e->phase_blocks = blocks;
    a.phase_clock = e->phase_clock;
  }
#endif
  EventPair kev;
  CMI_TRY(timer_begin(e, kev));
  p.kernel_first<<<blocks, p.first_threads, 0, e->stream>>>(a);
  HIP_TRY(hipGetLastError());
  return timer_end(e, e->kernel_events, kev, a.n_packets);
}

static InteractArgs interact_args(const cmi_gpu_engine *e, const ShootArgs &a) {
  InteractArgs ia;
  memset(&ia, 0, sizeof ia);
  ia.model = e->model;
  ia.cells = cells_of_iteration(e);
  ia.counters = e->counters;
  ia.first_packet = a.first_packet;
  ia.seed = a.seed;
  ia.iteration = a.iteration;
  ia.qin = e->ended_queue;
  ia.grid = e->grid;
  return ia;
}

static int launch_pass(cmi_gpu_engine *e, const LaunchPlan &p,
                       const ShootArgs &a, const double *rows,
                       unsigned int count, bool last) {
  ShootArgs b = a;
  b.park_in_place = 0;
  b.order = nullptr;
  b.xin = rows;
  b.xin_local = rows ? 1 : 0;
  b.n_packets = count;
  b.refill_threshold = e->tune.refill_threshold_reemit;
  b.aggregate = p.agg_reemit;
  b.qin = rows ? no_queue() : e->ready_queue;
  b.qout = last ? no_queue() : e->ended_queue;
  if (!last)
    HIP_TRY(hipMemsetAsync(e->ended_queue.count, 0, sizeof(unsigned int),
                           e->stream));
  const unsigned blocks = transport_blocks(
      e, count, b.chunk, last ? p.blocks_per_cu_inline : p.blocks_per_cu,
      CMI_BLOCK);
  EventPair gev;
  CMI_TRY(timer_begin(e, gev));
  (last ? p.kernel_inline : p.kernel)<<<blocks, CMI_BLOCK, 0, e->stream>>>(b);
  HIP_TRY(hipGetLastError());
  return timer_end(e, e->kernel_events, gev, count);
}

#define CMI_TILE_MAX_ROUNDS 1000

struct TileRounds {
  TileGridDev tg;
  int tile_bits;
  uint32_t item_flights;
  bool defer;
  unsigned int *d_nrows, *d_nlive, *d_nitems, *d_next, *d_new;
  InteractArgs ia;
  int cur;
  FlightRowsDev rows;
  uint32_t *keys, *keys_next;
  const uint32_t *slot_of;
  int next_slot_of;
  unsigned int npos;
  unsigned int extent;
  unsigned int nlive, nitems;
  const uint32_t *order;
};

static int tile_rounds_begin(cmi_gpu_engine *e, const ShootArgs &a,
                             TileRounds &t) {
  t.tg = tile_grid(e);
  t.tile_bits = 1;
  while ((1ll << t.tile_bits) < (int64_t)t.tg.ntiles + 1)
    ++t.tile_bits;
  t.item_flights =
      e->full_ions ? CMI_TILE_ITEM_FLIGHTS_FULL : CMI_TILE_ITEM_FLIGHTS_H;
  t.defer = e->full_ions && e->tune.defer_weights;
  t.d_nrows = e->tile_counts;
  t.d_nlive = e->tile_counts + 1;
  t.d_nitems = e->tile_counts + 2;
  t.d_next = e->tile_counts + 3;
  t.d_new = e->tile_counts + 4;
  t.cur = 0;
  t.rows = e->tile_rows[t.cur];
  InteractArgs &ia = t.ia;
  ia = interact_args(e, a);
  ia.n_in = a.park_in_place ? (uint32_t)a.n_packets : 0u;
  ia.tiles = t.tg;
  ia.items = e->tile_items;
  ia.nitems = t.d_nitems;
  ia.absorbed_before = e->tile_absorbed_before;
  ia.ended_slot = e->tile_ended_slot;
  ia.new_slots = e->tile_new_slots;
  ia.new_count = t.d_new;
  ia.rows = t.rows;
  ia.rows.count = t.d_nrows;
  HIP_TRY(hipMemsetAsync(e->tile_counts, 0, 8 * sizeof(unsigned int),
                         e->stream));
  const int iblocks = e->num_cu * 8;
  if (t.defer)
    interaction_kernel<true, true, true>
        <<<iblocks, CMI_BLOCK, 0, e->stream>>>(ia);
  else if (e->full_ions)
    interaction_kernel<true, true><<<iblocks, CMI_BLOCK, 0, e->stream>>>(ia);
  else
    interaction_kernel<false, true><<<iblocks, CMI_BLOCK, 0, e->stream>>>(ia);
  HIP_TRY(hipGetLastError());
  unsigned int nslots = 0;
// ... 121 lines not shown
  ta.absorbed_count = e->tile_absorbed_count;
  ta.xout = a.xout;
  int64_t tb = (int64_t)e->num_cu * p.tile_blocks_per_cu;
  const int64_t most =
      (int64_t)t.tg.ntiles + (int64_t)t.nlive / t.item_flights + 1;
  if (tb > most)
    tb = most;
  EventPair tev;
  CMI_TRY(timer_begin(e, tev));
  p.tile_kernel<<<(unsigned)tb, p.tile_threads, 0, e->stream>>>(ta);
  HIP_TRY(hipGetLastError());
  CMI_TRY(timer_end(e, e->kernel_events, tev, t.nlive));
  ++e->tile_rounds_run;
  return CMI_GPU_OK;
}

static int tile_round_reemit(cmi_gpu_engine *e, TileRounds &t) {
  InteractArgs &ia = t.ia;
  ia.rows = t.rows;
  ia.ended_pos = e->tile_ended_pos;
  ia.key_out = t.keys_next;
  absorbed_scan_kernel<<<1, CMI_TILE_PLAN_THREADS, 0, e->stream>>>(
      t.d_nitems, e->tile_absorbed_count, e->tile_absorbed_before);
  HIP_TRY(hipGetLastError());
  const int sblocks = grid_blocks(e, (int64_t)t.nlive / 2 + 1, 8);
  if (t.defer) {
    HIP_TRY(hipMemsetAsync(t.d_new, 0, sizeof(unsigned int), e->stream));
    interaction_slots_kernel<true, true>
        <<<sblocks, CMI_BLOCK, 0, e->stream>>>(ia);
    HIP_TRY(hipGetLastError());
    FlightWeightsArgs wa;
    wa.model = e->model;
    wa.rows = t.rows;
    wa.slots = e->tile_new_slots;
    wa.count = t.d_new;
    wa.n = 0;
    flight_weights_kernel<<<grid_blocks(e, (int64_t)t.nlive / 4 + 1, 8),
                            CMI_BLOCK, 0, e->stream>>>(wa);
  } else if (e->full_ions)
    interaction_slots_kernel<true><<<sblocks, CMI_BLOCK, 0, e->stream>>>(ia);
  else
    interaction_slots_kernel<false><<<sblocks, CMI_BLOCK, 0, e->stream>>>(ia);
  HIP_TRY(hipGetLastError());
  std::swap(t.keys, t.keys_next);
  t.slot_of = e->tile_slot_of[t.next_slot_of];
  t.next_slot_of = 1 - t.next_slot_of;
  t.npos = t.nlive;
  return CMI_GPU_OK;
}

static int run_tile_rounds(cmi_gpu_engine *e, const LaunchPlan &p,
                           const ShootArgs &a, const double **handover,
                           unsigned int *handover_count) {
  TileRounds t;
  CMI_TRY(tile_rounds_begin(e, a, t));
  const unsigned int compact_ratio =
      e->tune.tile_compact_ratio >= 0
          ? (unsigned int)e->tune.tile_compact_ratio
          : (e->full_ions ? 2u : 0u);
  for (int round = 0; t.npos != 0; ++round) {
    CMI_TRY(tile_round_order(e, t));
    if (t.nlive == 0)
      break;
    const uint64_t per_item = e->tune.tile_min_per_item >= 0
                                  ? (uint64_t)e->tune.tile_min_per_item
                                  : 200u;
    const bool finish = t.nlive < e->tune.tile_min_flights ||
                        (uint64_t)t.nlive < per_item * t.nitems ||
                        round >= CMI_TILE_MAX_ROUNDS;
    if (finish || (compact_ratio != 0 && (uint64_t)compact_ratio * t.nlive <
                                             (uint64_t)t.extent))
      CMI_TRY(tile_round_compact(e, t));
    if (finish) {
      *handover = t.rows.rows;
      *handover_count = t.nlive;
      break;
    }
    CMI_TRY(tile_round_launch(e, p, a, t));
    CMI_TRY(tile_round_reemit(e, t));
  }
  return CMI_GPU_OK;
}

static int run_passes(cmi_gpu_engine *e, const LaunchPlan &p,
                      const ShootArgs &a, const double *handover,
                      unsigned int handover_count) {
  if (handover_count != 0) {
    const bool last = handover_count < reemit_inline_below(e);
    CMI_TRY(launch_pass(e, p, a, handover, handover_count, last));
    if (last)
      handover_count = 0;
  }
  for (int gen = 0; p.passes && (!p.tiles || handover_count != 0); ++gen) {
    InteractArgs ia = interact_args(e, a);
    ia.n_in = (gen == 0 && !p.tiles && a.park_in_place)
                  ? (uint32_t)a.n_packets
                  : 0u;
    ia.qout = e->ready_queue;
    HIP_TRY(hipMemsetAsync(e->ready_queue.count, 0, sizeof(unsigned int),
                           e->stream));
    const int iblocks = e->num_cu * 8;
    if (e->full_ions)
      interaction_kernel<true, false><<<iblocks, CMI_BLOCK, 0, e->stream>>>(ia);
    else
      interaction_kernel<false, false>
          <<<iblocks, CMI_BLOCK, 0, e->stream>>>(ia);
    HIP_TRY(hipGetLastError());
    unsigned int count = 0;
    CMI_TRY(read_counters(e, e->ready_queue.count, 1, &count));
    if (count == 0)
      break;
    const bool last = count < reemit_inline_below(e) ||
                      gen + 2 >= e->tune.reemit_max_passes;
    CMI_TRY(launch_pass(e, p, a, nullptr, count, last));
    if (last)
      break;
  }
  return CMI_GPU_OK;
}

static int shoot_impl(cmi_gpu_engine *e, uint32_t seed, uint32_t iteration,
                      uint64_t first_packet, uint64_t n_packets,
                      const double *flights) {
  if (!e)
    return fail(CMI_GPU_EINVAL, "null engine");
  if (!e->have_sources || (e->model.nsource > 0 && !e->have_spectrum) ||
      (e->model.continuous_type != 0 && !e->have_continuous_spectrum) ||
      !e->have_xsec || !e->have_cells)
    return fail(CMI_GPU_ESTATE,
                "cmi_gpu_shoot: sources, their spectra, cross sections and "
                "cell data must be set first");
  if (n_packets == 0)
    return CMI_GPU_OK;
  if (n_packets >= 0xffffffffull)
    return fail(CMI_GPU_EINVAL,
                "cmi_gpu_shoot: at most 2^32 - 2 packets per call");
  if (e->grid.decomposed &&
      (e->tune.exact_dda || !e->export_rows ||
       e->ncell >= CMI_FAST_MARCHER_MAX_CELLS))
    return fail(CMI_GPU_ESTATE,
                "cmi_gpu_shoot: a block of a decomposed grid needs an export "
                "buffer (cmi_gpu_set_export_buffer) and the incremental "
                "marcher (fewer than 2^28 cells per block)");
  if (!flights && e->grid.decomposed && block_emits_nothing(e))
    return CMI_GPU_OK;
  HIP_TRY(hipSetDevice(e->device));
  CMI_TRY(ensure_spectra(e));

  LaunchPlan plan;
  CMI_TRY(plan_launches(e, n_packets, flights, plan));
  if (!flights) {
    e->last_first_build = (int32_t)plan.first;
    e->last_pad_uniform = plan.pad_uniform;
  }
  CMI_TRY(publish_escape(e, plan.tracking));
  const uint64_t max_launch = e->tune.max_packets_per_launch;
  if (!plan.select_mode)
    CMI_TRY(reserve_for(e, plan, n_packets < max_launch ? n_packets
                                                         : max_launch));
  if (plan.pad)
    CMI_TRY(pad_records(e, plan));

  for (uint64_t done = 0; done < n_packets; done += max_launch) {
    const uint64_t nids = n_packets - done < max_launch ? n_packets - done
                                                        : max_launch;
    ShootArgs a = shoot_args(e, plan, seed, iteration, first_packet, done,
                             nids, flights);
    const uint32_t *select = nullptr;
    if (plan.select_mode) {
      CMI_TRY(select_block_packets(e, a, &select));
      if (a.n_packets == 0)
        continue;
      CMI_TRY(reserve_for(e, plan, a.n_packets + a.n_packets / 16 + 1024));
    }
    if (plan.passes)
      CMI_TRY(open_ended_queue(e, a));

    EventPair ev;
    CMI_TRY(timer_begin(e, ev));
    if (plan.sorted)
      CMI_TRY(order_packets(e, plan, a, nids, select));
    CMI_TRY(launch_first_generation(e, plan, a));
    const double *handover = nullptr;
    unsigned int handover_count = 0;
    if (plan.tiles)
      CMI_TRY(run_tile_rounds(e, plan, a, &handover, &handover_count));
    CMI_TRY(run_passes(e, plan, a, handover, handover_count));
    CMI_TRY(timer_end(e, e->shoot_events, ev, 0));
  }
  return CMI_GPU_OK;
}

#endif
```

### cmacionize_amd/engine.py

```python
import ctypes as C
import os

import numpy as np

_HERE = os.path.dirname(os.path.abspath(__file__))
LIB_PATH = os.environ.get("CMI_GPU_LIBRARY",
                          os.path.join(_HERE, "libcmi_gpu.so"))

NION = 14
TRACKER_SPECTRUM, TRACKER_ABSORPTION, TRACKER_WEIGHTED_SPECTRUM = 0, 1, 2
NACC = 16
NTYPE = 4

FIELD_NUMBER_DENSITY = 0
FIELD_TEMPERATURE = 1
FIELD_IONIC_FRACTION = 2
FIELD_MEAN_INTENSITY = 16
FIELD_HEATING = 30

REEMIT_NONE, REEMIT_PHYSICAL, REEMIT_FIXED = 0, 1, 2
CONTINUOUS_NONE, CONTINUOUS_ISOTROPIC, CONTINUOUS_PLANAR = 0, 1, 2
ROLE_SOURCE, ROLE_CONTINUOUS = 0, 1
TABLE_LINEAR, TABLE_LOGLOG = 0, 1
DUST_PROBE_EMIT, DUST_PROBE_SCATTER, DUST_PROBE_SCATTER_TOWARDS = 0, 1, 2
DUST_PROBE_OPTICAL_DEPTH, DUST_PROBE_TRACE = 3, 4
DUST_PROBE_CELL_SOURCE = 5
DUST_PROBE_SKY_PEEL = 6
DUST_PROBE_CUBE_TRACE = 7
LYA_PROBE_VOIGT, LYA_PROBE_OPTICAL_DEPTH = 0, 1
LYA_PROBE_SAMPLER, LYA_PROBE_TRACE = 2, 3
LYA_MAX_SCATTER = 100000000
LYA_LAMBDA0 = 1215.67e-10
LYA_FIELD_COLUMNS = ("L", "S_H", "S_d", "G_x", "G_y", "G_z", "N_H", "N_d")
MAX_VIEWS = 64

_dp = C.POINTER(C.c_double)


class Config(C.Structure):
    _fields_ = [("anchor", C.c_double * 3), ("sides", C.c_double * 3),
                ("ncell", C.c_int32 * 3), ("periodic", C.c_int32 * 3),
                ("device", C.c_int32), ("track_heating", C.c_int32),
                ("stream", C.c_void_p),
                ("external_accumulators", C.c_void_p),
                ("sub_offset", C.c_int32 * 3), ("sub_ncell", C.c_int32 * 3)]


class TemperatureParams(C.Structure):
    _fields_ = [("do_temperature_calculation", C.c_int32),
                ("minimum_number_of_iterations", C.c_int32),
                ("epsilon_convergence", C.c_double),
                ("maximum_number_of_iterations", C.c_int32),
                ("pah_heating_factor", C.c_double),
                ("cosmic_ray_heating_factor", C.c_double),
                ("cosmic_ray_heating_limit", C.c_double),
                ("cosmic_ray_heating_scale_length", C.c_double),
                ("minimum_ionized_temperature", C.c_double)]


class EngineError(RuntimeError):
    pass


EXPORTED_SYMBOLS = [
    "cmi_gpu_create", "cmi_gpu_destroy", "cmi_gpu_last_error",
    "cmi_gpu_synchronize", "cmi_gpu_number_of_cells", "cmi_gpu_set_sources",
    "cmi_gpu_set_spectrum_monochromatic", "cmi_gpu_set_spectrum_planck",
    "cmi_gpu_set_continuous_source",
    "cmi_gpu_set_continuous_source_planar",
    "cmi_gpu_set_continuous_spectrum_monochromatic",
    "cmi_gpu_set_continuous_spectrum_planck",
    "cmi_gpu_set_cross_sections_fixed", "cmi_gpu_set_cross_sections_verner",
    "cmi_gpu_set_spectrum_table", "cmi_gpu_set_cross_sections_table",
    "cmi_gpu_set_recombination_rates_table",
    "cmi_gpu_set_recombination_rates_fixed",
    "cmi_gpu_set_recombination_rates_verner", "cmi_gpu_set_abundances",
    "cmi_gpu_set_reemission", "cmi_gpu_set_temperature_params",
    "cmi_gpu_upload_cells", "cmi_gpu_upload_field", "cmi_gpu_download_field",
    "cmi_gpu_field_device_pointer", "cmi_gpu_reset_grid", "cmi_gpu_shoot",
    "cmi_gpu_get_counters", "cmi_gpu_update_cells", "cmi_gpu_emit_packets",
    "cmi_gpu_trace_packets", "cmi_gpu_get_timing", "cmi_gpu_set_tuning",
    "cmi_gpu_get_atomic_count", "cmi_gpu_sample_spectrum",
    "cmi_gpu_thermal_probe", "cmi_gpu_accumulator_layout",
    "cmi_gpu_get_kernel_timing", "cmi_gpu_get_wave_steps",
    "cmi_gpu_get_launch_times", "cmi_gpu_set_export_buffer",
    "cmi_gpu_get_export_count", "cmi_gpu_reset_exports",
    "cmi_gpu_shoot_flights", "cmi_gpu_download_exports",
    "cmi_gpu_shoot_flights_host", "cmi_gpu_physics_probe",
    "cmi_gpu_update_cells_range", "cmi_gpu_refresh_transport_records",
    "cmi_gpu_get_launch_steps", "cmi_gpu_group_create",
    "cmi_gpu_group_destroy", "cmi_gpu_group_reduce_accumulators",
    "cmi_gpu_group_update_cells",
    "cmi_gpu_group_exchange_flights", "cmi_gpu_group_exchange_stats",
    "cmi_gpu_compute_emissivities",
    "cmi_gpu_set_spectrum_trackers", "cmi_gpu_enable_trackers",
    "cmi_gpu_get_tracker_counts", "cmi_gpu_set_trackers",
    "cmi_gpu_get_tracker_absorption", "cmi_gpu_set_tracker_frequency_bins",
    "cmi_gpu_get_tracker_flux", "cmi_gpu_projected_areas",
    "cmi_gpu_set_dust_scattering", "cmi_gpu_set_ccd_image",
    "cmi_gpu_set_continuous_source_spiral_galaxy", "cmi_gpu_dust_shoot",
    "cmi_gpu_download_image", "cmi_gpu_reset_image",
    "cmi_gpu_get_dust_counters", "cmi_gpu_dust_probe",
    "cmi_gpu_render_line_images", "cmi_gpu_render_field_images",
    "cmi_gpu_line_image_probe",
    "cmi_gpu_set_dust_scattering_per_hydrogen",
    "cmi_gpu_set_cell_source_line", "cmi_gpu_set_cell_source_field",
    "cmi_gpu_get_cell_source",
    "cmi_gpu_render_line_sky", "cmi_gpu_render_field_sky",
    "cmi_gpu_sky_probe", "cmi_gpu_render_line_sky_map",
    "cmi_gpu_sky_map_directions",
    "cmi_gpu_set_sky_camera", "cmi_gpu_check_sky_camera",
    "cmi_gpu_get_sky_camera_counters",
    "cmi_gpu_set_ccd_images", "cmi_gpu_set_sky_cameras",
    "cmi_gpu_download_image_view", "cmi_gpu_get_dust_view_counters",
    "cmi_gpu_select_probe_view",
    "cmi_gpu_set_cell_velocities", "cmi_gpu_render_line_cube",
    "cmi_gpu_render_field_cube", "cmi_gpu_emission_line_atomic_weight",
    "cmi_gpu_render_field_sky_cube", "cmi_gpu_render_line_sky_cube",
    "cmi_gpu_render_line_sky_map_cube",
    "cmi_gpu_set_scattered_cube", "cmi_gpu_download_cube_view",
    "cmi_gpu_get_phase_clocks",
    "cmi_gpu_free_free_coefficients", "cmi_gpu_render_continuum_images",
    "cmi_gpu_render_field_continuum_images", "cmi_gpu_render_continuum_sky",
    "cmi_gpu_render_field_continuum_sky",
    "cmi_gpu_render_continuum_sky_map", "cmi_gpu_continuum_probe",
    "cmi_gpu_hi_coefficients", "cmi_gpu_render_hi_cube",
    "cmi_gpu_render_hi_sky_cube", "cmi_gpu_render_hi_sky_map_cube",
    "cmi_gpu_render_field_absorbing_cube",
    "cmi_gpu_render_field_absorbing_sky_cube",
    "cmi_gpu_absorbing_cube_probe", "cmi_gpu_get_update_state",
    "cmi_gpu_set_lyman_alpha", "cmi_gpu_lya_shoot", "cmi_gpu_lya_probe",
    "cmi_gpu_download_lya_view", "cmi_gpu_reset_lya",
    "cmi_gpu_get_lya_counters", "cmi_gpu_lyman_alpha_emissivity",
    "cmi_gpu_set_lya_field", "cmi_gpu_download_lya_field",
    "cmi_gpu_lya_spin_temperature",
    "cmi_gpu_render_field_absorption_spectra",
    "cmi_gpu_render_absorption_spectra", "cmi_gpu_absorption_probe",
    "cmi_gpu_set_escape_tally", "cmi_gpu_reset_escape_tally",
    "cmi_gpu_download_escape_tally", "cmi_gpu_escape_pixels",
    "cmi_gpu_cross_sections", "cmi_gpu_get_transport_plan",
]

EMISSION_LINES = [
    "HAlpha", "HBeta", "HII", "BALMER_JUMP_LOW", "BALMER_JUMP_HIGH",
    "OI_6300", "OI_6364", "OII_3727", "OIII_5007", "OIII_4959", "OIII_4363",
    "OIII_52mu", "OIII_88mu", "NII_5755", "NII_6548", "NII_6584",
    "NeIII_3869", "NeIII_3968", "SII_6725", "SII_4072", "SIII_9405",
    "SIII_6312", "SIII_19mu", "SIII_33mu", "avg_T", "avg_T_count",
    "avg_nH_nHe", "avg_nH_nHe_count", "NeII_12mu", "NIII_57mu", "NeIII_15mu",
    "NII_122mu", "CII_158mu", "CII_2325", "CIII_1908", "OII_7325", "SIV_10mu",
    "HeI_5876", "Hrec_s", "WFC2_F439W", "WFC2_F555W", "WFC2_F675W"]

_ELEMENT_WEIGHTS = {"H": 1.00794, "He": 4.002602, "C": 12.0107, "N": 14.0067,
                    "O": 15.9994, "Ne": 20.1797, "S": 32.065}


def _line_element(name):
    if name in ("HAlpha", "HBeta"):
        return "H"
    for element in ("He", "Ne", "C", "N", "O", "S"):
        if name.startswith(element + "I"):
            return element
    return None


LINE_ATOMIC_WEIGHTS = {name: _ELEMENT_WEIGHTS[_line_element(name)]
                       for name in EMISSION_LINES
                       if name != "HII" and _line_element(name)}


def cube_channel_centres(nchan, vmin, vmax):
    dv = (vmax - vmin) / nchan
    edges = vmin + np.arange(nchan + 1) * dv
    return 0.5 * (edges[:-1] + edges[1:])


def cube_moments(cube, centres):
    cube = np.asarray(cube, dtype=np.float64)
    v = np.asarray(centres, dtype=np.float64)[:, None, None]
    m0 = cube.sum(axis=-3)
    with np.errstate(invalid="ignore", divide="ignore"):
        mean = np.where(m0 == 0., np.nan, (cube * v).sum(axis=-3) / m0)
        var = (cube * (v - mean[..., None, :, :]) ** 2).sum(axis=-3) / m0
        sigma = np.where(m0 == 0., np.nan, np.sqrt(np.maximum(var, 0.)))
    return m0, mean, sigma


PLANCK = 6.626070040e-34
BOLTZMANN = 1.38064852e-23
LIGHTSPEED = 299792458.


def planck_function(nu, T):
    nu, T = np.broadcast_arrays(np.asarray(nu, dtype=np.float64),
                                np.asarray(T, dtype=np.float64))
    out = np.zeros(nu.shape)
    ok = T > 0.
    with np.errstate(over="ignore"):
        out[ok] = (2. * PLANCK * nu[ok] * nu[ok] * nu[ok] /
                   (LIGHTSPEED * LIGHTSPEED)) / \
            np.expm1((PLANCK * nu[ok]) / (BOLTZMANN * T[ok]))
    return out if out.ndim else float(out)


def brightness_temperature(I, nu):
    I = np.asarray(I, dtype=np.float64)
    nu = np.asarray(nu, dtype=np.float64)
    if nu.ndim == 1 and I.ndim > 1:
        nu = nu.reshape((-1,) + (1,) * (I.ndim - 1))
    return LIGHTSPEED * LIGHTSPEED * I / (2. * BOLTZMANN * nu * nu)


def continuum_spectral_index(I, freq):
    I = np.asarray(I, dtype=np.float64)
    nu = np.asarray(freq, dtype=np.float64).reshape(-1)
    if len(nu) != I.shape[0] or len(nu) < 2:
        raise ValueError("continuum_spectral_index needs I[nf][...] and "
                         "freq[nf], nf >= 2")
    dlognu = np.log(nu[1:] / nu[:-1]).reshape((-1,) + (1,) * (I.ndim - 1))
    with np.errstate(invalid="ignore", divide="ignore"):
        ok = (I[1:] > 0.) & (I[:-1] > 0.)
        ratio = np.where(ok, I[1:] / np.where(ok, I[:-1], 1.), np.nan)
        return np.log(ratio) / dlognu


def continuum_flux_density(I, pixel_solid_angle):
    I = np.asarray(I, dtype=np.float64)
    w = np.asarray(pixel_solid_angle, dtype=np.float64)
    return (I * w).reshape(I.shape[0], -1).sum(axis=1)


HI_FREQUENCY = 1420405751.768
HI_EINSTEIN_A = 2.8843e-15
HI_COLUMN_CONSTANT = 5.516606267115072e-20

HI_SPIN_KINETIC, HI_SPIN_FIXED, HI_SPIN_CELLS = 0, 1, 2


def hi_column_density(cube, dv):
    T_b = brightness_temperature(np.asarray(cube, dtype=np.float64),
                                 HI_FREQUENCY)
    return T_b.sum(axis=0) * dv / HI_COLUMN_CONSTANT


_lib = None


def load_library():
    global _lib
    if _lib is not None:
        return _lib
    if not os.path.exists(LIB_PATH):
        raise EngineError(
            "HIP engine library not found at %s - build it with "
            "`python -c 'import __graft_entry__ as g; g.build()'` or "
            "`make -C cmacionize_amd/csrc`. There is no CPU fallback." %
            LIB_PATH)
    try:
        import torch
        if torch.cuda.is_available():
            torch.cuda.init()
    except ImportError:
        pass
    L = C.CDLL(LIB_PATH)
    vp = C.c_void_p
    L.cmi_gpu_last_error.restype = C.c_char_p
    L.cmi_gpu_create.argtypes = [C.POINTER(Config), C.POINTER(vp)]
    L.cmi_gpu_destroy.argtypes = [vp]
    L.cmi_gpu_synchronize.argtypes = [vp]
    L.cmi_gpu_number_of_cells.restype = C.c_int64
    L.cmi_gpu_number_of_cells.argtypes = [vp]
    L.cmi_gpu_set_sources.argtypes = [vp, C.c_int32, _dp, _dp, C.c_double]
    L.cmi_gpu_set_spectrum_monochromatic.argtypes = [vp, C.c_double]
    L.cmi_gpu_set_spectrum_planck.argtypes = [vp, C.c_double]
    L.cmi_gpu_set_continuous_source.argtypes = [vp, C.c_int32, C.c_double]
    L.cmi_gpu_set_continuous_source_planar.argtypes = [
        vp, C.c_int32, C.c_double, _dp, _dp, C.c_double]
    L.cmi_gpu_set_continuous_spectrum_monochromatic.argtypes = [vp, C.c_double]
    L.cmi_gpu_set_continuous_spectrum_planck.argtypes = [vp, C.c_double]
    L.cmi_gpu_set_cross_sections_fixed.argtypes = [vp, _dp]
    L.cmi_gpu_set_spectrum_table.argtypes = [vp, C.c_int32, C.c_int32, _dp,
                                             _dp, C.c_int32]
    L.cmi_gpu_set_cross_sections_table.argtypes = [vp, C.c_int32, _dp, _dp,
                                                   C.c_int32]
    L.cmi_gpu_set_recombination_rates_table.argtypes = [vp, C.c_int32, _dp,
                                                        _dp, C.c_int32]
    L.cmi_gpu_set_cross_sections_verner.argtypes = [vp]
    L.cmi_gpu_set_recombination_rates_fixed.argtypes = [vp, _dp]
    L.cmi_gpu_set_recombination_rates_verner.argtypes = [vp]
    L.cmi_gpu_set_abundances.argtypes = [vp, _dp]
    L.cmi_gpu_set_reemission.argtypes = [vp, C.c_int32, C.c_double,
                                         C.c_double]
    L.cmi_gpu_set_temperature_params.argtypes = [
        vp, C.POINTER(TemperatureParams)]
    L.cmi_gpu_upload_cells.argtypes = [vp, _dp, _dp, _dp]
    L.cmi_gpu_upload_field.argtypes = [vp, C.c_int32, _dp]
    L.cmi_gpu_download_field.argtypes = [vp, C.c_int32, _dp]
    L.cmi_gpu_field_device_pointer.restype = C.c_void_p
    L.cmi_gpu_field_device_pointer.argtypes = [vp, C.c_int32]
    if hasattr(L, "cmi_gpu_get_update_state"):
        L.cmi_gpu_get_update_state.argtypes = [vp] + 3 * [C.POINTER(C.c_int32)]
    if hasattr(L, "cmi_gpu_get_transport_plan"):
        L.cmi_gpu_get_transport_plan.argtypes = [vp] + 2 * [
            C.POINTER(C.c_int32)]
    L.cmi_gpu_reset_grid.argtypes = [vp]
    L.cmi_gpu_shoot.argtypes = [vp, C.c_uint32, C.c_uint32, C.c_uint64,
                                C.c_uint64]
    L.cmi_gpu_get_counters.argtypes = [vp, _dp, _dp, C.POINTER(C.c_uint64)]
    L.cmi_gpu_update_cells.argtypes = [vp, C.c_uint32, C.c_double]
    L.cmi_gpu_emit_packets.argtypes = [vp, C.c_uint32, C.c_uint32, C.c_uint64,
                                       C.c_uint64, _dp, _dp, _dp, _dp, _dp]
    L.cmi_gpu_trace_packets.argtypes = [
        vp, C.c_uint64, _dp, _dp, _dp, _dp, _dp, C.c_int32,
        C.POINTER(C.c_int64), _dp, C.POINTER(C.c_int32), C.POINTER(C.c_int64),
        _dp]
    L.cmi_gpu_get_timing.argtypes = [vp, C.c_int32, _dp, C.POINTER(C.c_uint64),
                                     _dp, C.POINTER(C.c_uint64)]
    L.cmi_gpu_get_kernel_timing.argtypes = [vp, _dp, C.POINTER(C.c_uint64)]
    L.cmi_gpu_set_tuning.argtypes = [vp, C.c_char_p, C.c_int64]
    L.cmi_gpu_get_atomic_count.argtypes = [vp, C.POINTER(C.c_uint64)]
    if hasattr(L, "cmi_gpu_get_phase_clocks"):
        L.cmi_gpu_get_phase_clocks.argtypes = [vp, C.POINTER(C.c_uint64),
                                               C.c_int64,
                                               C.POINTER(C.c_int64)]
    L.cmi_gpu_get_wave_steps.argtypes = [vp, C.POINTER(C.c_uint64)]
    L.cmi_gpu_set_export_buffer.argtypes = [vp, vp, C.c_uint64]
    L.cmi_gpu_get_export_count.argtypes = [vp, C.POINTER(C.c_uint64)]
    L.cmi_gpu_reset_exports.argtypes = [vp]
    L.cmi_gpu_download_exports.argtypes = [vp, _dp, C.c_uint64,
                                           C.POINTER(C.c_uint64)]
    L.cmi_gpu_shoot_flights_host.argtypes = [vp, C.c_uint32, C.c_uint32,
                                             C.c_uint64, _dp, C.c_uint64]
    L.cmi_gpu_shoot_flights.argtypes = [vp, C.c_uint32, C.c_uint32,
                                        C.c_uint64, vp, C.c_uint64]
    L.cmi_gpu_get_launch_times.argtypes = [vp, C.c_uint64, _dp,
                                           C.POINTER(C.c_uint64),
                                           C.POINTER(C.c_uint64)]
    L.cmi_gpu_sample_spectrum.argtypes = [vp, C.c_int32, C.c_double,
                                          C.c_uint32, C.c_uint64, _dp]
    L.cmi_gpu_accumulator_layout.argtypes = [vp, C.POINTER(C.c_int64),
                                             C.POINTER(C.c_int64)]
    L.cmi_gpu_thermal_probe.argtypes = [vp, C.c_int64, C.c_int32, _dp, _dp,
                                        _dp, _dp, _dp, _dp, _dp]
    L.cmi_gpu_physics_probe.argtypes = [vp, C.c_int32, C.c_int64, _dp, _dp]
    L.cmi_gpu_compute_emissivities.argtypes = [
        vp, C.c_int32, C.POINTER(C.c_int32), C.c_int64, C.c_int64,
        C.POINTER(C.c_double)]
    L.cmi_gpu_set_spectrum_trackers.argtypes = [vp, C.c_int32, _dp, C.c_int32,
                                                _dp, _dp]
    L.cmi_gpu_set_trackers.argtypes = [vp, C.c_int32, _dp,
                                       C.POINTER(C.c_int32),
                                       C.POINTER(C.c_int32), _dp, _dp]
    L.cmi_gpu_get_tracker_absorption.argtypes = [vp, _dp]
    L.cmi_gpu_enable_trackers.argtypes = [vp, C.c_int32]
    L.cmi_gpu_set_tracker_frequency_bins.argtypes = [
        vp, C.c_int32, C.c_int32, C.c_double, C.c_double]
    L.cmi_gpu_get_tracker_flux.argtypes = [vp, _dp]
    L.cmi_gpu_projected_areas.argtypes = [_dp, C.c_int64, _dp]
    L.cmi_gpu_get_tracker_counts.argtypes = [vp, C.POINTER(C.c_uint64)]
    L.cmi_gpu_set_escape_tally.argtypes = [
        vp, C.c_int32, C.c_int32, _dp, C.c_int32, C.c_int32, C.c_double,
        C.c_double]
    L.cmi_gpu_reset_escape_tally.argtypes = [vp]
    L.cmi_gpu_download_escape_tally.argtypes = [vp, _dp]
    L.cmi_gpu_escape_pixels.argtypes = [_dp, C.c_int32, C.c_int32, C.c_int64,
                                        _dp, C.POINTER(C.c_int32), _dp]
    L.cmi_gpu_cross_sections.argtypes = [vp, C.c_int64, _dp, _dp]
    L.cmi_gpu_update_cells_range.argtypes = [vp, C.c_uint32, C.c_double,
                                             C.c_int64, C.c_int64]
    L.cmi_gpu_refresh_transport_records.argtypes = [vp]
    L.cmi_gpu_get_launch_steps.argtypes = [vp, C.c_uint64,
                                           C.POINTER(C.c_uint64),
                                           C.POINTER(C.c_uint64)]
    L.cmi_gpu_group_create.argtypes = [C.c_int32, C.POINTER(vp),
                                       C.POINTER(vp)]
    L.cmi_gpu_group_destroy.argtypes = [vp]
    L.cmi_gpu_group_reduce_accumulators.argtypes = [vp]
    L.cmi_gpu_group_update_cells.argtypes = [vp, C.c_uint32, C.c_double]
    L.cmi_gpu_group_exchange_flights.argtypes = [
        vp, C.c_uint32, C.c_uint32, C.c_uint64, C.POINTER(C.c_uint64)]
    L.cmi_gpu_group_exchange_stats.argtypes = [
        vp, C.POINTER(C.c_uint64), C.POINTER(C.c_double), C.c_int32]
    L.cmi_gpu_set_dust_scattering.argtypes = [vp, C.c_double, C.c_double,
                                              C.c_double, C.c_double]
    L.cmi_gpu_set_ccd_image.argtypes = [vp, C.c_double, C.c_double, C.c_int32,
                                        C.c_int32, _dp, _dp]
    L.cmi_gpu_set_continuous_source_spiral_galaxy.argtypes = [
        vp, C.c_double, C.c_double, C.c_double]
    L.cmi_gpu_dust_shoot.argtypes = [vp, C.c_uint32, C.c_uint64, C.c_uint64]
    L.cmi_gpu_download_image.argtypes = [vp, _dp, _dp, _dp]
    L.cmi_gpu_reset_image.argtypes = [vp]
    L.cmi_gpu_get_dust_counters.argtypes = [vp, C.POINTER(C.c_uint64)]
    L.cmi_gpu_dust_probe.argtypes = [vp, C.c_int32, C.c_uint32, C.c_uint64,
                                     C.c_int64, _dp, _dp, C.c_int32]
    L.cmi_gpu_render_line_images.argtypes = [
        vp, C.c_int32, C.POINTER(C.c_int32), C.c_double, C.c_double,
        C.c_int32, C.c_int32, _dp, _dp, C.c_int32, C.c_double, _dp]
    L.cmi_gpu_render_field_images.argtypes = [
        vp, C.c_int32, _dp, C.c_double, C.c_double, C.c_int32, C.c_int32, _dp,
        _dp, C.c_int32, _dp, _dp]
    L.cmi_gpu_set_cell_velocities.argtypes = [vp, _dp]
    L.cmi_gpu_emission_line_atomic_weight.argtypes = [C.c_int32]
    L.cmi_gpu_emission_line_atomic_weight.restype = C.c_double
    L.cmi_gpu_render_line_cube.argtypes = [
        vp, C.c_int32, C.POINTER(C.c_int32), C.c_double, C.c_double,
        C.c_int32, C.c_int32, _dp, _dp, C.c_int32, C.c_double, C.c_int32,
        C.c_double, C.c_double, C.c_double, _dp]
    L.cmi_gpu_render_field_cube.argtypes = [
        vp, C.c_int32, _dp, _dp, _dp, _dp, C.c_double, C.c_double, C.c_int32,
        C.c_int32, _dp, _dp, C.c_int32, C.c_int32, C.c_double, C.c_double,
        _dp]
    L.cmi_gpu_set_dust_scattering_per_hydrogen.argtypes = [
        vp, C.c_double, C.c_double, C.c_double, C.c_double]
    L.cmi_gpu_set_cell_source_line.argtypes = [vp, C.c_int32]
    L.cmi_gpu_set_cell_source_field.argtypes = [vp, _dp]
    L.cmi_gpu_get_cell_source.argtypes = [vp, _dp, _dp, _dp]
    L.cmi_gpu_line_image_probe.argtypes = [vp, C.c_double, C.c_double,
                                           C.c_int64, _dp, C.c_int32, _dp]
    L.cmi_gpu_render_line_sky.argtypes = [
        vp, C.c_int32, C.POINTER(C.c_int32), _dp, C.c_int64, _dp, C.c_double,
        _dp]
    L.cmi_gpu_render_field_sky.argtypes = [
        vp, C.c_int32, _dp, _dp, C.c_int64, _dp, _dp, _dp]
    L.cmi_gpu_sky_probe.argtypes = [vp, _dp, C.c_int64, _dp, C.c_int32, _dp]
    L.cmi_gpu_render_line_sky_map.argtypes = [
        vp, C.c_int32, C.POINTER(C.c_int32), _dp, _dp, C.c_double, C.c_double,
        C.c_double, C.c_double, C.c_int32, C.c_int32, C.c_double, _dp]
    L.cmi_gpu_render_field_sky_cube.argtypes = [
        vp, C.c_int32, _dp, _dp, _dp, _dp, _dp, _dp, C.c_int64, _dp,
        C.c_int32, C.c_double, C.c_double, _dp]
    L.cmi_gpu_render_line_sky_cube.argtypes = [
        vp, C.c_int32, C.POINTER(C.c_int32), _dp, _dp, C.c_int64, _dp,
        C.c_double, C.c_int32, C.c_double, C.c_double, C.c_double, _dp]
    L.cmi_gpu_render_line_sky_map_cube.argtypes = [
        vp, C.c_int32, C.POINTER(C.c_int32), _dp, _dp, C.c_double, C.c_double,
        C.c_double, C.c_double, C.c_int32, C.c_int32, C.c_double, _dp,
        C.c_int32, C.c_double, C.c_double, C.c_double, _dp]
    L.cmi_gpu_sky_map_directions.argtypes = [
        _dp, C.c_double, C.c_double, C.c_double, C.c_double, C.c_int32,
        C.c_int32, _dp, _dp]
    L.cmi_gpu_set_sky_camera.argtypes = [
        vp, _dp, _dp, C.c_double, C.c_double, C.c_double, C.c_double,
        C.c_int32, C.c_int32, C.c_double, C.c_int32]
    L.cmi_gpu_check_sky_camera.argtypes = [
        _dp, _dp, _dp, _dp, C.c_double, C.c_double, C.c_double, C.c_double,
        C.c_int32, C.c_int32, C.c_double]
    L.cmi_gpu_get_sky_camera_counters.argtypes = [vp, C.POINTER(C.c_uint64)]
    L.cmi_gpu_set_ccd_images.argtypes = [vp, C.c_int32, _dp, _dp, C.c_int32,
                                         C.c_int32, _dp, _dp]
    L.cmi_gpu_set_sky_cameras.argtypes = [
        vp, C.c_int32, _dp, _dp, C.c_double, C.c_double, C.c_double,
        C.c_double, C.c_int32, C.c_int32, _dp, C.c_int32]
    L.cmi_gpu_download_image_view.argtypes = [vp, C.c_int32, _dp, _dp, _dp]
    L.cmi_gpu_get_dust_view_counters.argtypes = [vp, C.c_int32,
                                                 C.POINTER(C.c_uint64)]
    L.cmi_gpu_select_probe_view.argtypes = [vp, C.c_int32]
    L.cmi_gpu_set_scattered_cube.argtypes = [
# ... 312 lines not shown
                                          for a in range(3)]))
        self.set_tuning(timing=1)

    def _check(self, rc):
        if rc != 0:
            raise EngineError("cmi_gpu error %d: %s" % (
                rc, self._lib.cmi_gpu_last_error().decode()))

    def close(self):
        if getattr(self, "_h", None) and self._h.value:
            self._lib.cmi_gpu_destroy(self._h)
            self._h = C.c_void_p()

    def __del__(self):
        try:
            self.close()
        except Exception:
            pass

    def set_sources(self, positions, weights, luminosity):
        w = _f64(weights)
        if len(w) == 0:
            self._check(self._lib.cmi_gpu_set_sources(self._h, 0, None, None,
                                                      0.))
            return
        pos = _f64(positions).reshape(-1, 3)
        self._check(self._lib.cmi_gpu_set_sources(self._h, len(w), _p(pos),
                                                  _p(w), luminosity))

    def set_continuous_source(self, kind, luminosity):
        self._check(self._lib.cmi_gpu_set_continuous_source(self._h, kind,
                                                            luminosity))

    def set_continuous_source_planar(self, axis, intercept, anchor, sides,
                                     luminosity):
        a = _f64(anchor)
        s = _f64(sides)
        self._check(self._lib.cmi_gpu_set_continuous_source_planar(
            self._h, axis, intercept, _p(a), _p(s), luminosity))

    def set_continuous_spectrum_monochromatic(self, frequency):
        self._check(self._lib.cmi_gpu_set_continuous_spectrum_monochromatic(
            self._h, frequency))

    def set_continuous_spectrum_planck(self, temperature):
        self._check(self._lib.cmi_gpu_set_continuous_spectrum_planck(
            self._h, temperature))

    def set_spectrum_monochromatic(self, frequency):
        self._check(self._lib.cmi_gpu_set_spectrum_monochromatic(self._h,
                                                                 frequency))

    def set_spectrum_planck(self, temperature):
        self._check(self._lib.cmi_gpu_set_spectrum_planck(self._h,
                                                          temperature))

    def set_spectrum_table(self, frequency, cumulative, role=ROLE_SOURCE,
                           interpolation=TABLE_LINEAR):
        f, c = _f64(frequency), _f64(cumulative)
        assert f.shape == c.shape and f.ndim == 1
        self._check(self._lib.cmi_gpu_set_spectrum_table(
            self._h, role, len(f), _p(f), _p(c), interpolation))

    def set_cross_sections_table(self, frequency, sigma,
                                 interpolation=TABLE_LINEAR):
        f, s = _f64(frequency), _f64(sigma)
        assert s.shape == (NION, len(f))
        self._check(self._lib.cmi_gpu_set_cross_sections_table(
            self._h, len(f), _p(f), _p(s), interpolation))

    def set_recombination_rates_table(self, temperature, alpha,
                                      interpolation=TABLE_LOGLOG):
        t, a = _f64(temperature), _f64(alpha)
        assert a.shape == (NION, len(t))
        self._check(self._lib.cmi_gpu_set_recombination_rates_table(
            self._h, len(t), _p(t), _p(a), interpolation))

    def set_cross_sections_fixed(self, sigma):
        s = _f64(sigma)
        assert s.shape == (NION,)
        self._check(self._lib.cmi_gpu_set_cross_sections_fixed(self._h, _p(s)))

    def set_cross_sections_verner(self):
        self._check(self._lib.cmi_gpu_set_cross_sections_verner(self._h))

    def set_recombination_rates_fixed(self, alpha):
        a = _f64(alpha)
        assert a.shape == (NION,)
        self._check(self._lib.cmi_gpu_set_recombination_rates_fixed(self._h,
                                                                    _p(a)))

    def set_recombination_rates_verner(self):
        self._check(self._lib.cmi_gpu_set_recombination_rates_verner(self._h))

    def set_abundances(self, abundances):
        a = _f64(abundances)
        assert a.shape == (6,)
        self._check(self._lib.cmi_gpu_set_abundances(self._h, _p(a)))
        self._abundances = a.copy()

    def set_reemission(self, kind, probability=0., frequency=0.):
        self._check(self._lib.cmi_gpu_set_reemission(self._h, kind,
                                                     probability, frequency))

    def set_temperature_params(self, **kw):
        p = TemperatureParams(0, 3, 1.e-3, 100, 0., 0., 0.75,
                              1.33333 * 3.086e19, 4000.)
        for k, v in kw.items():
            setattr(p, k, v)
        self._check(self._lib.cmi_gpu_set_temperature_params(self._h,
                                                             C.byref(p)))

    def upload_cells(self, number_density, temperature, ionic_fractions=None):
        n = _f64(number_density).ravel()
        t = _f64(temperature).ravel()
        assert n.size == self.n and t.size == self.n
        x = None
        if ionic_fractions is not None:
            x = _f64(ionic_fractions).reshape(NION, self.n)
        self._check(self._lib.cmi_gpu_upload_cells(
            self._h, _p(n), _p(t), _p_or_none(x)))

    def upload_field(self, field, values):
        v = _f64(values).ravel()
        assert v.size == self.n
        self._check(self._lib.cmi_gpu_upload_field(self._h, field, _p(v)))

    def download_field(self, field):
        out = np.empty(self.n)
        self._check(self._lib.cmi_gpu_download_field(self._h, field, _p(out)))
        return out

    def accumulator_layout(self):
        fs, cs = C.c_int64(), C.c_int64()
        self._check(self._lib.cmi_gpu_accumulator_layout(
            self._h, C.byref(fs), C.byref(cs)))
        return fs.value, cs.value

    def field_device_pointer(self, field):
        return self._lib.cmi_gpu_field_device_pointer(self._h, field)

    def update_state(self):
        v = [C.c_int32() for _ in range(3)]
        self._check(self._lib.cmi_gpu_get_update_state(
            self._h, *[C.byref(x) for x in v]))
        return tuple(bool(x.value) for x in v)

    def transport_plan(self):
        first, uniform = C.c_int32(), C.c_int32()
        self._check(self._lib.cmi_gpu_get_transport_plan(
            self._h, C.byref(first), C.byref(uniform)))
        return first.value, bool(uniform.value)

    def field_tensor(self, field):
        import torch
        ptr = self.field_device_pointer(field)
        n = self.n

        class _View:
            __cuda_array_interface__ = {
                "shape": (n,), "typestr": "<f8", "data": (int(ptr), False),
                "version": 2}
        return torch.as_tensor(_View(), device="cuda")

    def refresh_transport_records(self):
        self._check(self._lib.cmi_gpu_refresh_transport_records(self._h))

    def reset_grid(self):
        self._check(self._lib.cmi_gpu_reset_grid(self._h))

    def shoot(self, seed, iteration, first_packet, n_packets):
        self._check(self._lib.cmi_gpu_shoot(self._h, seed, iteration,
                                            first_packet, n_packets))

    def get_counters(self):
        tw = C.c_double()
        tc = np.zeros(NTYPE)
        ns = C.c_uint64()
        self._check(self._lib.cmi_gpu_get_counters(self._h, C.byref(tw),
                                                   _p(tc), C.byref(ns)))
        return tw.value, tc, ns.value

    def get_atomic_count(self):
        n = C.c_uint64()
        self._check(self._lib.cmi_gpu_get_atomic_count(self._h, C.byref(n)))
        return n.value

    def get_phase_clocks(self):
        n = C.c_int64()
        self._check(self._lib.cmi_gpu_get_phase_clocks(self._h, None, 0,
                                                       C.byref(n)))
        out = np.zeros(n.value, dtype=np.uint64)
        self._check(self._lib.cmi_gpu_get_phase_clocks(
            self._h, out.ctypes.data_as(C.POINTER(C.c_uint64)), n.value,
            C.byref(n)))
        return out[:5], int(out[5]), out[6:]

    def get_launch_times(self):
        n = C.c_uint64()
        self._check(self._lib.cmi_gpu_get_launch_times(self._h, 0, None, None,
                                                       C.byref(n)))
        ms = np.zeros(max(n.value, 1))
        pk = np.zeros(max(n.value, 1), dtype=np.uint64)
        self._check(self._lib.cmi_gpu_get_launch_times(
            self._h, n.value, _p(ms),
            pk.ctypes.data_as(C.POINTER(C.c_uint64)), C.byref(n)))
        return list(zip(ms[:n.value].tolist(), pk[:n.value].tolist()))

    def get_launch_steps(self):
        n = C.c_uint64()
        self._check(self._lib.cmi_gpu_get_launch_steps(self._h, 0, None,
                                                       C.byref(n)))
        st = np.zeros(max(n.value, 1), dtype=np.uint64)
        self._check(self._lib.cmi_gpu_get_launch_steps(
            self._h, n.value, st.ctypes.data_as(C.POINTER(C.c_uint64)),
            C.byref(n)))
        return st[:n.value].tolist()

    def set_export_buffer(self, device_pointer, capacity):
        self._check(self._lib.cmi_gpu_set_export_buffer(
            self._h, device_pointer, int(capacity)))

    def get_export_count(self):
        n = C.c_uint64()
        self._check(self._lib.cmi_gpu_get_export_count(self._h, C.byref(n)))
        return n.value

    def reset_exports(self):
        self._check(self._lib.cmi_gpu_reset_exports(self._h))

    def shoot_flights(self, seed, iteration, first_packet, device_pointer, n):
        self._check(self._lib.cmi_gpu_shoot_flights(
            self._h, seed, iteration, int(first_packet), device_pointer,
            int(n)))

    def get_wave_steps(self):
        n = C.c_uint64()
        self._check(self._lib.cmi_gpu_get_wave_steps(self._h, C.byref(n)))
        return n.value

    def update_cells(self, loop, totweight):
        self._check(self._lib.cmi_gpu_update_cells(self._h, loop, totweight))

    def update_cells_range(self, loop, totweight, first_cell, ncell):
        self._check(self._lib.cmi_gpu_update_cells_range(
            self._h, loop, totweight, first_cell, ncell))

    def compute_emissivities(self, lines=None, first_cell=0, ncell=None):
        names = list(EMISSION_LINES if lines is None else lines)
        idx = _line_indices(names)
        if ncell is None:
            ncell = self.n - first_cell
        out = np.empty((len(names), ncell))
        self._check(self._lib.cmi_gpu_compute_emissivities(
            self._h, len(names), idx,
            first_cell, ncell, out.ctypes.data_as(C.POINTER(C.c_double))))
        return dict(zip(names, out))

    def set_spectrum_trackers(self, positions, nbins=100, opening_angles=None,
                              reference_directions=None):
        pos = _f64(positions).reshape(-1, 3)
        n = len(pos)
        ang = None if opening_angles is None else _f64(opening_angles)
        ref = None if reference_directions is None else \
            _f64(reference_directions).reshape(-1, 3)
        self._check(self._lib.cmi_gpu_set_spectrum_trackers(
            self._h, n, _p(pos) if n else None, nbins,
            None if ang is None else _p(ang),
            None if ref is None else _p(ref)))
        self._trackers = (n, nbins)

    def set_trackers(self, positions, kinds, nbins=100, opening_angles=None,
                     reference_directions=None):
        pos = _f64(positions).reshape(-1, 3)
        n = len(pos)
        kinds = np.ascontiguousarray(kinds, dtype=np.int32)
        assert kinds.size == n
        bins = np.ascontiguousarray(
            np.broadcast_to(np.asarray(nbins, dtype=np.int32), (n,)))
        ang = None if opening_angles is None else _f64(opening_angles)
        ref = None if reference_directions is None else \
            _f64(reference_directions).reshape(-1, 3)
        self._check(self._lib.cmi_gpu_set_trackers(
            self._h, n, _p(pos) if n else None,
            kinds.ctypes.data_as(C.POINTER(C.c_int32)),
            bins.ctypes.data_as(C.POINTER(C.c_int32)),
            None if ang is None else _p(ang),
            None if ref is None else _p(ref)))
        self._trackers = (n, bins.tolist())

    def get_tracker_absorption(self):
        n, _ = self._trackers
        out = np.zeros((n, 4, NION))
        self._check(self._lib.cmi_gpu_get_tracker_absorption(self._h, _p(out)))
        return out

    def set_tracker_frequency_bins(self, tracker, kind="Linear",
                                   minimum_frequency=0., maximum_frequency=0.):
        self._check(self._lib.cmi_gpu_set_tracker_frequency_bins(
            self._h, tracker, {"Linear": 0, "Level": 1}[kind],
            minimum_frequency, maximum_frequency))

    def get_tracker_flux(self):
        n, nbins = self._trackers
        bins = [nbins] * n if np.isscalar(nbins) else list(nbins)
        flat = np.zeros(4 * max(sum(bins), 1))
        self._check(self._lib.cmi_gpu_get_tracker_flux(self._h, _p(flat)))
        out, at = [], 0
        for b in bins:
            out.append(flat[at:at + 4 * b].reshape(4, b))
            at += 4 * b
        return out

    def enable_trackers(self, on=True):
        self._check(self._lib.cmi_gpu_enable_trackers(self._h, int(on)))

    def get_tracker_counts(self):
        n, nbins = self._trackers
        bins = [nbins] * n if np.isscalar(nbins) else list(nbins)
        flat = np.zeros(3 * max(sum(bins), 1), dtype=np.uint64)
        self._check(self._lib.cmi_gpu_get_tracker_counts(
            self._h, flat.ctypes.data_as(C.POINTER(C.c_uint64))))
        out, at = [], 0
        for b in bins:
            out.append(flat[at:at + 3 * b].reshape(3, b))
            at += 3 * b
        if len(set(bins)) <= 1:
            return np.array(out).reshape(n, 3, bins[0] if bins else 0)
        return out

    def set_escape_tally(self, nlon, nmu, frame=IDENTITY_FRAME, nfreq=1,
                         bins="Linear", minimum_frequency=3.289e15,
                         maximum_frequency=4. * 3.289e15):
        kind = {"Linear": 0, "Level": 1}[bins]
        if kind == 1:
            nfreq = NION
        self._check(self._lib.cmi_gpu_set_escape_tally(
            self._h, int(nlon), int(nmu), _p(_f64(frame).reshape(9)),
            int(nfreq), kind, minimum_frequency, maximum_frequency))
        self._escape = (int(nfreq), int(nlon), int(nmu)) if nlon else None

    def reset_escape_tally(self):
        self._check(self._lib.cmi_gpu_reset_escape_tally(self._h))

    def escape_tally(self):
        shape = self._escape if self._escape is not None else (1, 1, 1)
        out = np.zeros((3,) + shape)
        self._check(self._lib.cmi_gpu_download_escape_tally(self._h, _p(out)))
        return out

    def cross_sections(self, frequencies):
        nu = _f64(frequencies).reshape(-1)
        out = np.zeros((len(nu), NION))
        self._check(self._lib.cmi_gpu_cross_sections(self._h, len(nu), _p(nu),
                                                     _p(out)))
        return out

    def ionizing_columns(self, origin, directions):
        n_H = self.download_field(FIELD_NUMBER_DENSITY)
        abundance = {"H": 1.}
        abundance.update(zip(("He", "C", "N", "O", "Ne", "S"),
                             self._abundances))
        fields = np.empty((NION, self.n))
        for ion in range(NION):
            fields[ion] = (n_H * abundance[_ION_ELEMENTS[ion]] *
                           self.download_field(FIELD_IONIC_FRACTION + ion))
        return np.ascontiguousarray(
            4. * np.pi * self.render_field_sky(fields, origin, directions).T)

    def ionizing_optical_depths(self, origin, directions, frequencies):
        return (self.ionizing_columns(origin, directions) @
                self.cross_sections(frequencies).T)

    def set_tuning(self, **kw):
        for k, v in kw.items():
            self._check(self._lib.cmi_gpu_set_tuning(self._h, k.encode(),
                                                     int(v)))

    def synchronize(self):
        self._check(self._lib.cmi_gpu_synchronize(self._h))

    def emit_packets(self, seed, iteration, first_packet, n):
        pos = np.empty((n, 3))
        dirn = np.empty((n, 3))
        nu = np.empty(n)
        sig = np.empty((n, NION))
        tau = np.empty(n)
        self._check(self._lib.cmi_gpu_emit_packets(
            self._h, seed, iteration, first_packet, n, _p(pos), _p(dirn),
            _p(nu), _p(sig), _p(tau)))
        return pos, dirn, nu, sig, tau

    def trace_packets(self, position, direction, tau, sigma_H, sigma_He_corr,
                      max_steps):
        pos = _f64(position).reshape(-1, 3)
        n = pos.shape[0]
        dirn = _f64(direction).reshape(n, 3)
        tau = _f64(tau).reshape(n)
        sh = _f64(sigma_H).reshape(n)
        she = _f64(sigma_He_corr).reshape(n)
        cells = np.empty((n, max_steps), dtype=np.int64)
        ds = np.empty((n, max_steps))
        nsteps = np.empty(n, dtype=np.int32)
        last = np.empty(n, dtype=np.int64)
        final = np.empty((n, 3))
        self._check(self._lib.cmi_gpu_trace_packets(
            self._h, n, _p(pos), _p(dirn), _p(tau), _p(sh), _p(she), max_steps,
            cells.ctypes.data_as(C.POINTER(C.c_int64)), _p(ds),
            nsteps.ctypes.data_as(C.POINTER(C.c_int32)),
            last.ctypes.data_as(C.POINTER(C.c_int64)), _p(final)))
        return cells, ds, nsteps, last, final

    def sample_spectrum(self, kind, temperature, seed, n):
        out = np.empty(n)
        self._check(self._lib.cmi_gpu_sample_spectrum(
            self._h, kind, temperature, seed, n, _p(out)))
        return out

    def thermal_probe(self, solve, J, heating, temperature, number_density):
        J = _f64(J).reshape(-1, NION)
        n = J.shape[0]
        heating = _f64(heating).reshape(n, 2)
        T = _f64(temperature).reshape(n)
        dens = _f64(number_density).reshape(n)
        x = np.empty((n, NION))
        Tout = np.empty(n)
        pair = np.empty((n, 2))
        self._check(self._lib.cmi_gpu_thermal_probe(
            self._h, n, int(solve), _p(J), _p(heating), _p(T), _p(dens),
            _p(x), _p(Tout), _p(pair)))
        return x, Tout, pair

    def physics_probe(self, kind, rows):
        width_in = (1, 1, 15, 1, 1)[kind]
        width_out = (14, 14, 1, 5, 42)[kind]
        rows = _f64(rows).reshape(-1, width_in)
        out = np.zeros((rows.shape[0], width_out))
        self._check(self._lib.cmi_gpu_physics_probe(
            self._h, kind, rows.shape[0], _p(rows), _p(out)))
        return out

    def set_dust_scattering(self, g, p_l, albedo, kappa):
        self._check(self._lib.cmi_gpu_set_dust_scattering(
            self._h, g, p_l, albedo, kappa))

    def set_dust_scattering_per_hydrogen(self, g, p_l, albedo, sigma):
        self._check(self._lib.cmi_gpu_set_dust_scattering_per_hydrogen(
            self._h, g, p_l, albedo, sigma))

    def set_cell_source_line(self, line):
        self._check(self._lib.cmi_gpu_set_cell_source_line(
            self._h, EMISSION_LINES.index(line)))

    def set_cell_source_field(self, field):
        f = _f64(field).reshape(self.n)
        self._check(self._lib.cmi_gpu_set_cell_source_field(self._h, _p(f)))

    def get_cell_source(self, tables=True):
        total = C.c_double()
        if not tables:
            self._check(self._lib.cmi_gpu_get_cell_source(
                self._h, C.byref(total), None, None))
            return total.value
        blocks = np.zeros((self.n + 255) // 256)
        cells = np.zeros(self.n)
        self._check(self._lib.cmi_gpu_get_cell_source(
            self._h, C.byref(total), _p(blocks), _p(cells)))
        return total.value, blocks, cells

    def set_ccd_image(self, theta, phi, nx, ny, anchor, sides):
        a = _f64(anchor).reshape(2)
        s = _f64(sides).reshape(2)
        self._check(self._lib.cmi_gpu_set_ccd_image(
            self._h, theta, phi, int(nx), int(ny), _p(a), _p(s)))
        self.image_shape = (int(nx), int(ny))
        self.nviews = 1

    def set_ccd_images(self, theta, phi, nx, ny, anchors, sides):
        t = _f64(theta).reshape(-1)
        f = _f64(phi).reshape(-1)
        n = len(t)
        if len(f) != n:
            raise ValueError("theta and phi differ in length")
        a = _f64(np.broadcast_to(_f64(anchors), (n, 2)))
        s = _f64(np.broadcast_to(_f64(sides), (n, 2)))
        self._check(self._lib.cmi_gpu_set_ccd_images(
            self._h, n, _p(t), _p(f), int(nx), int(ny), _p(a), _p(s)))
        self.image_shape = (int(nx), int(ny))
        self.nviews = n

    def download_images(self):
        out = np.zeros((self.nviews, 3) + self.image_shape)
        for v in range(self.nviews):
            out[v] = self.download_image_view(v)
        return out

    def download_image_view(self, view):
        out = np.zeros((3,) + self.image_shape)
        self._check(self._lib.cmi_gpu_download_image_view(
            self._h, int(view), _p(out[0]), _p(out[1]), _p(out[2])))
        return out

    def get_dust_view_counters(self, view):
        c = (C.c_uint64 * 4)()
        self._check(self._lib.cmi_gpu_get_dust_view_counters(
            self._h, int(view), c))
        return dict(zip(("nsteps", "natomics", "nexcluded", "noutside"),
                        (int(v) for v in c)))

    def select_probe_view(self, view):
        self._check(self._lib.cmi_gpu_select_probe_view(self._h, int(view)))

    def set_continuous_source_spiral_galaxy(self, r_stars, h_stars,
                                            bulge_over_total):
        self._check(self._lib.cmi_gpu_set_continuous_source_spiral_galaxy(
            self._h, r_stars, h_stars, bulge_over_total))

    def dust_shoot(self, seed, first_packet, n):
        self._check(self._lib.cmi_gpu_dust_shoot(self._h, seed, first_packet,
                                                 n))

    def download_image(self):
        out = np.zeros((3,) + self.image_shape)
        self._check(self._lib.cmi_gpu_download_image(
            self._h, _p(out[0]), _p(out[1]), _p(out[2])))
        return out

    def reset_image(self):
        self._check(self._lib.cmi_gpu_reset_image(self._h))

    def get_dust_counters(self):
        c = (C.c_uint64 * 6)()
        self._check(self._lib.cmi_gpu_get_dust_counters(self._h, c))
        return dict(zip(("nsteps", "nscatter", "ncapped", "natomics",
                         "npackets", "nsource_capped"), (int(v) for v in c)))

    def dust_probe(self, kind, seed, first_packet, n, rows=None,
                   max_events=0):
        width = {DUST_PROBE_EMIT: 6, DUST_PROBE_SCATTER: 12,
                 DUST_PROBE_SCATTER_TOWARDS: 5,
                 DUST_PROBE_OPTICAL_DEPTH: 2 + max_events,
                 DUST_PROBE_TRACE: 4 + 8 * max_events,
                 DUST_PROBE_CELL_SOURCE: 7, DUST_PROBE_SKY_PEEL: 9,
                 DUST_PROBE_CUBE_TRACE: 4 + 10 * max_events}[kind]
# ... 810 lines not shown
```

### include/cmi_gpu.h

```cpp
#ifndef CMI_GPU_H
#define CMI_GPU_H

#include <stddef.h>
#include <stdint.h>

#ifdef __cplusplus
extern "C" {
#endif

#define CMI_GPU_NION 14
#define CMI_GPU_NHEATING 2
#define CMI_GPU_NTYPE 4
#define CMI_GPU_NACC (CMI_GPU_NION + CMI_GPU_NHEATING)

enum {
  CMI_GPU_OK = 0,
  CMI_GPU_EINVAL = 1,
  CMI_GPU_EDEVICE = 2,
  CMI_GPU_ESTATE = 3,
  CMI_GPU_ENOMEM = 4
};

enum {
  CMI_GPU_FIELD_NUMBER_DENSITY = 0,
  CMI_GPU_FIELD_TEMPERATURE = 1,
  CMI_GPU_FIELD_IONIC_FRACTION = 2,
  CMI_GPU_FIELD_MEAN_INTENSITY = 16,
  CMI_GPU_FIELD_HEATING = 30,
  CMI_GPU_NFIELD = 32
};

enum {
  CMI_GPU_SPECTRUM_MONOCHROMATIC = 0,
  CMI_GPU_SPECTRUM_PLANCK = 1,
  CMI_GPU_SPECTRUM_TABLE = 2
};
enum { CMI_GPU_ROLE_SOURCE = 0, CMI_GPU_ROLE_CONTINUOUS = 1 };
enum { CMI_GPU_TABLE_LINEAR = 0, CMI_GPU_TABLE_LOGLOG = 1 };
enum { CMI_GPU_REEMIT_NONE = 0, CMI_GPU_REEMIT_PHYSICAL = 1,
       CMI_GPU_REEMIT_FIXED = 2 };

typedef struct cmi_gpu_engine cmi_gpu_engine;

typedef struct {
  double anchor[3];
  double sides[3];
  int32_t ncell[3];
  int32_t periodic[3];
  int32_t device;
  int32_t track_heating;
  void *stream;
  void *external_accumulators;
  int32_t sub_offset[3];
  int32_t sub_ncell[3];
} cmi_gpu_config;


int cmi_gpu_create(const cmi_gpu_config *config, cmi_gpu_engine **engine);
int cmi_gpu_destroy(cmi_gpu_engine *engine);
const char *cmi_gpu_last_error(void);
int cmi_gpu_synchronize(cmi_gpu_engine *engine);
int64_t cmi_gpu_number_of_cells(const cmi_gpu_engine *engine);


int cmi_gpu_set_sources(cmi_gpu_engine *engine, int32_t n,
                        const double *positions, const double *weights,
                        double total_luminosity);

enum {
  CMI_GPU_CONTINUOUS_NONE = 0,
  CMI_GPU_CONTINUOUS_ISOTROPIC = 1,
  CMI_GPU_CONTINUOUS_PLANAR = 2
};
int cmi_gpu_set_continuous_source(cmi_gpu_engine *engine, int32_t type,
                                  double luminosity);
int cmi_gpu_set_continuous_source_planar(cmi_gpu_engine *engine, int32_t axis,
                                         double intercept,
                                         const double *anchor,
                                         const double *sides,
                                         double luminosity);
int cmi_gpu_set_continuous_spectrum_monochromatic(cmi_gpu_engine *engine,
                                                  double frequency);
int cmi_gpu_set_continuous_spectrum_planck(cmi_gpu_engine *engine,
                                           double temperature);

int cmi_gpu_set_spectrum_monochromatic(cmi_gpu_engine *engine,
                                       double frequency);
int cmi_gpu_set_spectrum_planck(cmi_gpu_engine *engine, double temperature);

int cmi_gpu_set_spectrum_table(cmi_gpu_engine *engine, int32_t role, int32_t n,
                               const double *frequency,
                               const double *cumulative,
                               int32_t interpolation);
int cmi_gpu_set_cross_sections_table(cmi_gpu_engine *engine, int32_t n,
                                     const double *frequency,
                                     const double *sigma,
                                     int32_t interpolation);
int cmi_gpu_set_recombination_rates_table(cmi_gpu_engine *engine, int32_t n,
                                          const double *temperature,
                                          const double *alpha,
                                          int32_t interpolation);

int cmi_gpu_set_cross_sections_fixed(cmi_gpu_engine *engine,
                                     const double *sigma);
int cmi_gpu_set_cross_sections_verner(cmi_gpu_engine *engine);

int cmi_gpu_set_recombination_rates_fixed(cmi_gpu_engine *engine,
                                          const double *alpha);
int cmi_gpu_set_recombination_rates_verner(cmi_gpu_engine *engine);

int cmi_gpu_set_abundances(cmi_gpu_engine *engine, const double *abundances);

int cmi_gpu_set_reemission(cmi_gpu_engine *engine, int32_t type,
                           double fixed_probability, double fixed_frequency);

typedef struct {
  int32_t do_temperature_calculation;
  int32_t minimum_number_of_iterations;
  double epsilon_convergence;
  int32_t maximum_number_of_iterations;
  double pah_heating_factor;
  double cosmic_ray_heating_factor;
  double cosmic_ray_heating_limit;
  double cosmic_ray_heating_scale_length;
  double minimum_ionized_temperature;
} cmi_gpu_temperature_params;
int cmi_gpu_set_temperature_params(cmi_gpu_engine *engine,
                                   const cmi_gpu_temperature_params *params);


int cmi_gpu_upload_cells(cmi_gpu_engine *engine, const double *number_density,
                         const double *temperature,
                         const double *ionic_fractions);
int cmi_gpu_upload_field(cmi_gpu_engine *engine, int32_t field,
                         const double *values);
int cmi_gpu_download_field(cmi_gpu_engine *engine, int32_t field,
                           double *values);
void *cmi_gpu_field_device_pointer(cmi_gpu_engine *engine, int32_t field);
int cmi_gpu_get_update_state(cmi_gpu_engine *engine, int32_t *metals_pending,
                             int32_t *pad_records_valid,
                             int32_t *deferral_allowed);
int cmi_gpu_get_transport_plan(cmi_gpu_engine *engine, int32_t *first_build,
                               int32_t *uniform_weight);
int cmi_gpu_accumulator_layout(cmi_gpu_engine *engine, int64_t *field_stride,
                               int64_t *cell_stride);


int cmi_gpu_reset_grid(cmi_gpu_engine *engine);

int cmi_gpu_shoot(cmi_gpu_engine *engine, uint32_t seed, uint32_t iteration,
                  uint64_t first_packet, uint64_t n_packets);

#define CMI_GPU_FLIGHT_DOUBLES 16
int cmi_gpu_set_export_buffer(cmi_gpu_engine *engine, void *device_rows,
                              uint64_t capacity);
int cmi_gpu_get_export_count(cmi_gpu_engine *engine, uint64_t *count);
int cmi_gpu_reset_exports(cmi_gpu_engine *engine);
int cmi_gpu_download_exports(cmi_gpu_engine *engine, double *host_rows,
                             uint64_t capacity, uint64_t *count);
int cmi_gpu_shoot_flights_host(cmi_gpu_engine *engine, uint32_t seed,
                               uint32_t iteration, uint64_t first_packet,
                               const double *host_rows, uint64_t n_flights);
int cmi_gpu_shoot_flights(cmi_gpu_engine *engine, uint32_t seed,
                          uint32_t iteration, uint64_t first_packet,
                          const void *device_rows, uint64_t n_flights);

int cmi_gpu_get_counters(cmi_gpu_engine *engine, double *totweight,
                         double *typecount, uint64_t *nsteps);

int cmi_gpu_get_atomic_count(cmi_gpu_engine *engine, uint64_t *natomics);

int cmi_gpu_get_wave_steps(cmi_gpu_engine *engine, uint64_t *nwavesteps);

int cmi_gpu_get_phase_clocks(cmi_gpu_engine *engine, uint64_t *out,
                             int64_t capacity, int64_t *count);

int cmi_gpu_update_cells(cmi_gpu_engine *engine, uint32_t loop,
                         double totweight);
int cmi_gpu_refresh_transport_records(cmi_gpu_engine *engine);

int cmi_gpu_update_cells_range(cmi_gpu_engine *engine, uint32_t loop,
                               double totweight, int64_t first_cell,
                               int64_t ncell);

#define CMI_GPU_NUMBER_OF_EMISSIONLINES 42
int cmi_gpu_compute_emissivities(cmi_gpu_engine *engine, int32_t nlines,
                                 const int32_t *lines, int64_t first_cell,
                                 int64_t ncell, double *emissivities);

int cmi_gpu_set_spectrum_trackers(cmi_gpu_engine *engine, int32_t n,
                                  const double *positions, int32_t nbins,
                                  const double *opening_angles,
                                  const double *reference_directions);
#define CMI_GPU_TRACKER_SPECTRUM 0
#define CMI_GPU_TRACKER_ABSORPTION 1
#define CMI_GPU_TRACKER_WEIGHTED_SPECTRUM 2
int cmi_gpu_set_trackers(cmi_gpu_engine *engine, int32_t n,
                         const double *positions, const int32_t *kinds,
                         const int32_t *nbins, const double *opening_angles,
                         const double *reference_directions);
int cmi_gpu_enable_trackers(cmi_gpu_engine *engine, int32_t enable);
#define CMI_GPU_FREQUENCY_BINS_LINEAR 0
#define CMI_GPU_FREQUENCY_BINS_LEVEL 1
int cmi_gpu_set_tracker_frequency_bins(cmi_gpu_engine *engine, int32_t tracker,
                                       int32_t type, double minimum_frequency,
                                       double maximum_frequency);
int cmi_gpu_get_tracker_flux(cmi_gpu_engine *engine, double *flux);
int cmi_gpu_projected_areas(const double *directions, int64_t n,
                            double *areas);
int cmi_gpu_get_tracker_absorption(cmi_gpu_engine *engine,
                                   double *absorption);
int cmi_gpu_get_tracker_counts(cmi_gpu_engine *engine, uint64_t *counts);

int cmi_gpu_set_escape_tally(cmi_gpu_engine *engine, int32_t nlon, int32_t nmu,
                             const double frame[9], int32_t nfreq,
                             int32_t bins_type, double minimum_frequency,
                             double maximum_frequency);
int cmi_gpu_reset_escape_tally(cmi_gpu_engine *engine);
int cmi_gpu_download_escape_tally(cmi_gpu_engine *engine, double *sky);
int cmi_gpu_escape_pixels(const double frame[9], int32_t nlon, int32_t nmu,
                          int64_t n, const double *directions, int32_t *pixels,
                          double *centres);
int cmi_gpu_cross_sections(cmi_gpu_engine *engine, int64_t n,
                           const double *frequencies, double *sigma);

int cmi_gpu_set_tuning(cmi_gpu_engine *engine, const char *key, int64_t value);


typedef struct cmi_gpu_group cmi_gpu_group;
int cmi_gpu_group_create(int32_t n, cmi_gpu_engine *const *engines,
                         cmi_gpu_group **out);
int cmi_gpu_group_destroy(cmi_gpu_group *group);

int cmi_gpu_group_reduce_accumulators(cmi_gpu_group *group);

int cmi_gpu_group_update_cells(cmi_gpu_group *group, uint32_t loop,
                               double totweight);

int cmi_gpu_group_exchange_flights(cmi_gpu_group *group, uint32_t seed,
                                   uint32_t iteration, uint64_t first_packet,
                                   uint64_t *total_flights);
int cmi_gpu_group_exchange_stats(cmi_gpu_group *group, uint64_t *rounds,
                                 double *microseconds, int32_t reset);


int cmi_gpu_emit_packets(cmi_gpu_engine *engine, uint32_t seed,
                         uint32_t iteration, uint64_t first_packet, uint64_t n,
                         double *position, double *direction,
                         double *frequency, double *cross_sections,
                         double *tau);

int cmi_gpu_trace_packets(cmi_gpu_engine *engine, uint64_t n,
                          const double *position, const double *direction,
                          const double *tau, const double *sigma_H,
                          const double *sigma_He_corr, int32_t max_steps,
                          int64_t *out_cell, double *out_ds,
                          int32_t *out_nsteps, int64_t *out_last_cell,
                          double *out_position);

int cmi_gpu_sample_spectrum(cmi_gpu_engine *engine, int32_t kind,
                            double temperature, uint32_t seed, uint64_t n,
                            double *frequencies);

int cmi_gpu_thermal_probe(cmi_gpu_engine *engine, int64_t n, int32_t solve,
                          const double *J, const double *heating,
                          const double *temperature,
                          const double *number_density, double *out_fractions,
                          double *out_temperature, double *out_pair);

int cmi_gpu_physics_probe(cmi_gpu_engine *engine, int32_t kind, int64_t n,
                          const double *in, double *out);

int cmi_gpu_get_timing(cmi_gpu_engine *engine, int32_t reset,
                       double *shoot_ms, uint64_t *shoot_launches,
                       double *update_ms, uint64_t *update_launches);

int cmi_gpu_get_kernel_timing(cmi_gpu_engine *engine, double *kernel_ms,
                              uint64_t *kernel_launches);
int cmi_gpu_get_launch_times(cmi_gpu_engine *engine, uint64_t capacity,
                             double *ms, uint64_t *packets, uint64_t *count);
int cmi_gpu_get_launch_steps(cmi_gpu_engine *engine, uint64_t capacity,
                             uint64_t *steps, uint64_t *count);


int cmi_gpu_set_dust_scattering(cmi_gpu_engine *engine, double g, double p_l,
                                double albedo, double kappa);

int cmi_gpu_set_dust_scattering_per_hydrogen(cmi_gpu_engine *engine, double g,
                                             double p_l, double albedo,
                                             double sigma);

int cmi_gpu_set_ccd_image(cmi_gpu_engine *engine, double theta, double phi,
                          int32_t nx, int32_t ny, const double *anchor,
                          const double *sides);

int cmi_gpu_set_continuous_source_spiral_galaxy(cmi_gpu_engine *engine,
                                                double r_stars, double h_stars,
                                                double bulge_over_total);

int cmi_gpu_set_cell_source_line(cmi_gpu_engine *engine, int32_t line);
int cmi_gpu_set_cell_source_field(cmi_gpu_engine *engine, const double *field);

int cmi_gpu_get_cell_source(cmi_gpu_engine *engine, double *total_luminosity,
                            double *block_sums, double *cell_sums);

int cmi_gpu_dust_shoot(cmi_gpu_engine *engine, uint32_t seed,
                       uint64_t first_packet, uint64_t n);

int cmi_gpu_download_image(cmi_gpu_engine *engine, double *I, double *Q,
                           double *U);
int cmi_gpu_reset_image(cmi_gpu_engine *engine);

int cmi_gpu_get_dust_counters(cmi_gpu_engine *engine, uint64_t *counters);

int cmi_gpu_dust_probe(cmi_gpu_engine *engine, int32_t kind, uint32_t seed,
                       uint64_t first_packet, int64_t n, const double *in,
                       double *out, int32_t max_events);

int cmi_gpu_set_sky_camera(cmi_gpu_engine *engine, const double origin[3],
                           const double frame[9], double lon_min,
                           double lon_max, double lat_min, double lat_max,
                           int32_t nlon, int32_t nlat, double exclusion_radius,
                           int32_t direct_light);

int cmi_gpu_check_sky_camera(const double box_anchor[3],
                             const double box_sides[3], const double origin[3],
                             const double frame[9], double lon_min,
                             double lon_max, double lat_min, double lat_max,
                             int32_t nlon, int32_t nlat,
                             double exclusion_radius);

int cmi_gpu_get_sky_camera_counters(cmi_gpu_engine *engine,
                                    uint64_t *counters);

#define CMI_GPU_MAX_VIEWS 64

int cmi_gpu_set_ccd_images(cmi_gpu_engine *engine, int32_t nviews,
                           const double *theta, const double *phi, int32_t nx,
                           int32_t ny, const double *anchors,
                           const double *sides);

int cmi_gpu_set_sky_cameras(cmi_gpu_engine *engine, int32_t nviews,
                            const double *origins, const double *frames,
                            double lon_min, double lon_max, double lat_min,
                            double lat_max, int32_t nlon, int32_t nlat,
                            const double *exclusion_radii,
                            int32_t direct_light);

int cmi_gpu_download_image_view(cmi_gpu_engine *engine, int32_t view,
                                double *I, double *Q, double *U);

int cmi_gpu_get_dust_view_counters(cmi_gpu_engine *engine, int32_t view,
                                   uint64_t *counters);

int cmi_gpu_select_probe_view(cmi_gpu_engine *engine, int32_t view);


int cmi_gpu_render_line_images(cmi_gpu_engine *engine, int32_t nlines,
                               const int32_t *lines, double theta, double phi,
                               int32_t nx, int32_t ny, const double *anchor,
                               const double *sides, int32_t supersample,
                               double dust_cross_section, double *images);

int cmi_gpu_render_field_images(cmi_gpu_engine *engine, int32_t nfields,
                                const double *fields, double theta, double phi,
                                int32_t nx, int32_t ny, const double *anchor,
                                const double *sides, int32_t supersample,
                                const double *extinction, double *images);

int cmi_gpu_line_image_probe(cmi_gpu_engine *engine, double theta, double phi,
                             int64_t n, const double *xy, int32_t max_cells,
                             double *out);


double cmi_gpu_emission_line_atomic_weight(int32_t line);

int cmi_gpu_set_cell_velocities(cmi_gpu_engine *engine,
                                const double *velocities);

int cmi_gpu_render_line_cube(cmi_gpu_engine *engine, int32_t nlines,
                             const int32_t *lines, double theta, double phi,
                             int32_t nx, int32_t ny, const double *anchor,
                             const double *sides, int32_t supersample,
                             double dust_cross_section, int32_t nchan,
                             double vmin, double vmax, double sigma_turb,
                             double *cube);

int cmi_gpu_render_field_cube(cmi_gpu_engine *engine, int32_t nfields,
                              const double *fields, const double *extinction,
                              const double *velocity, const double *widths,
                              double theta, double phi, int32_t nx, int32_t ny,
                              const double *anchor, const double *sides,
                              int32_t supersample, int32_t nchan, double vmin,
                              double vmax, double *cube);


int cmi_gpu_render_line_sky(cmi_gpu_engine *engine, int32_t nlines,
                            const int32_t *lines, const double origin[3],
                            int64_t nrays,
                            const double *directions ,
                            double dust_cross_section,
                            double *out );

int cmi_gpu_render_field_sky(cmi_gpu_engine *engine, int32_t nfields,
// ... 234 lines not shown
```

Before: 4.113 billion.

## Order packets with a two-level bucket sort instead of full radix sort

Adds a bucket-ordering path for packet sorting. Keys are generated and scattered straight into coarse regions in one fused kernel, then split into leaves and ordered within each leaf, replacing the multi-pass radix sort over keys and ids. The aim is to cut the sort's memory passes and the separate key-write step when launches are large. Buckets that overflow their capacity fall back to an unordered tail, which can weaken packet coherence. The change also adds more scratch memory and a debug/probe API.

```diff
diff --git a/cmacionize_amd/csrc/engine.hip b/cmacionize_amd/csrc/engine.hip
--- a/cmacionize_amd/csrc/engine.hip
+++ b/cmacionize_amd/csrc/engine.hip
@@ -107,6 +107,10 @@
   void *sort_temp = nullptr;
   size_t sort_temp_bytes = 0;
   uint64_t sort_capacity = 0;
+  uint64_t sort_block_words = 0;
+  uint32_t *bucket_meta = nullptr;
+  int32_t last_order_path = 0;
+  int32_t last_bucket_bits[2] = {0, 0};
   uint32_t *span_cursor = nullptr;
 #ifdef CMI_EXPERIMENTS
   unsigned long long *phase_clock = nullptr;
@@ -162,6 +166,10 @@
     int sort_tau_bits = -1;
     int sort_dir_bits = -1;
     int class_order = -1;
+    bool bucket_order = true;
+    int bucket_bits1 = -1, bucket_bits2 = -1;
+    int bucket_slack_permille = -1;
+    uint64_t bucket_min_packets = 1000000;
     int aggregate = CMI_AGG_BLOCK;
     int aggregate_reemit = CMI_AGG_NONE;
     int refill_threshold = CMI_REFILL_THRESHOLD;
@@ -1085,6 +1093,7 @@
   (void)hipFree(e->select_ids);
   (void)hipFree(e->select_rows);
   (void)hipFree(e->sort_temp);
+  (void)hipFree(e->bucket_meta);
   (void)hipFree(e->queue_block);
   (void)hipFree(e->queue_counts);
   if (e->mailbox)
@@ -1591,6 +1600,44 @@
   return CMI_GPU_OK;
 }
 
+#define CMI_BUCKET_META_LEAF_CURSOR                                            \
+  ((size_t)CMI_BUCKET_MAX * CMI_BUCKET_REGION_CURSOR_STRIDE)
+#define CMI_BUCKET_META_OVERFLOW                                               \
+  (CMI_BUCKET_META_LEAF_CURSOR + (size_t)CMI_BUCKET_MAX * CMI_BUCKET_MAX)
+#define CMI_BUCKET_META_ORDERED (CMI_BUCKET_META_OVERFLOW + 1)
+#define CMI_BUCKET_META_CLEARED (CMI_BUCKET_META_OVERFLOW + 8)
+#define CMI_BUCKET_META_LEAF_OFFSET CMI_BUCKET_META_CLEARED
+#define CMI_BUCKET_META_WORDS                                                  \
+  (CMI_BUCKET_META_LEAF_OFFSET + (size_t)CMI_BUCKET_MAX * CMI_BUCKET_MAX)
+static uint32_t *bucket_overflow_cursor(const cmi_gpu_engine *e) {
+  return e->bucket_meta + CMI_BUCKET_META_OVERFLOW;
+}
+
+int cmi_gpu_get_order_plan(cmi_gpu_engine *e, int32_t *path, int32_t *bits1,
+                           int32_t *bits2, uint64_t *overflow) {
+  if (!e)
+    return fail(CMI_GPU_EINVAL, "null engine");
+  const bool bucket = e->last_order_path == CMI_GPU_ORDER_BUCKET;
+  if (path)
+    *path = e->last_order_path;
+  if (bits1)
+    *bits1 = bucket ? e->last_bucket_bits[0] : 0;
+  if (bits2)
+    *bits2 = bucket ? e->last_bucket_bits[1] : 0;
+  if (overflow) {
+    *overflow = 0;
+    if (bucket) {
+      uint32_t sent = 0;
+      HIP_TRY(hipSetDevice(e->device));
+      HIP_TRY(hipStreamSynchronize(e->stream));
+      HIP_TRY(hipMemcpy(&sent, bucket_overflow_cursor(e), sizeof sent,
+                        hipMemcpyDeviceToHost));
+      *overflow = sent;
+    }
+  }
+  return CMI_GPU_OK;
+}
+
 int cmi_gpu_reset_grid(cmi_gpu_engine *e) {
   if (!e)
     return fail(CMI_GPU_EINVAL, "null engine");
@@ -1624,8 +1671,19 @@
     e->tune.sort_tau_bits = (int)(value < 0 ? -1 : (value > 3 ? 3 : value));
   else if (k == "class_order")
     e->tune.class_order = (int)(value < 0 ? -1 : (value != 0 ? 1 : 0));
+  else if (k == "bucket_order")
+    e->tune.bucket_order = value != 0;
+  else if (k == "bucket_bits1")
+    e->tune.bucket_bits1 = (int)(value < 0 ? -1 : (value > 8 ? 8 : value));
+  else if (k == "bucket_bits2")
+    e->tune.bucket_bits2 = (int)(value < 0 ? -1 : (value > 8 ? 8 : value));
+  else if (k == "bucket_slack_permille")
+    e->tune.bucket_slack_permille =
+        (int)(value < 0 ? -1 : (value > 1000000 ? 1000000 : value));
+  else if (k == "bucket_min_packets")
+    e->tune.bucket_min_packets = (uint64_t)(value < 0 ? 0 : value);
   else if (k == "aggregate")
-    e->tune.aggregate = (int)(value < 0 ? 0 : (value > 2 ? 2 : value));
+    e->tune.aggregate =(int)(value < 0 ? 0 : (value > 2 ? 2 : value));
   else if (k == "aggregate_reemit")
     e->tune.aggregate_reemit = (int)(value < 0 ? 0 : (value > 2 ? 2 : value));
   else if (k == "refill_threshold")
@@ -1753,6 +1811,55 @@
   return shoot_impl(e, seed, iteration, first_packet, n_packets, nullptr);
 }
 
+int cmi_gpu_order_packets(cmi_gpu_engine *e, uint32_t seed, uint32_t iteration,
+                          uint64_t first_packet, uint64_t n, uint32_t *out_ids,
+                          uint32_t *out_keys) {
+  if (!e)
+    return fail(CMI_GPU_EINVAL, "null engine");
+  if (!e->have_sources || (e->model.nsource > 0 && !e->have_spectrum) ||
+      (e->model.continuous_type != 0 && !e->have_continuous_spectrum) ||
+      !e->have_xsec || !e->have_cells)
+    return fail(CMI_GPU_ESTATE,
+                "order_packets: sources, their spectra, cross sections and "
+                "cell data must be set first");
+  if (n == 0)
+    return CMI_GPU_OK;
+  if (n > e->tune.max_packets_per_launch)
+    return fail(CMI_GPU_EINVAL, "order_packets: %llu packets are more than "
+                "one launch (max_packets_per_launch)", (unsigned long long)n);
+  HIP_TRY(hipSetDevice(e->device));
+  CMI_TRY(ensure_spectra(e));
+  LaunchPlan plan;
+  CMI_TRY(plan_launches(e, n, nullptr, plan));
+  if (!plan.sorted || plan.select_mode)
+    return fail(CMI_GPU_ESTATE, "order_packets: a transport call of this "
+                "engine %s", plan.sorted ? "orders a block's selection"
+                                         : "does not order its packets");
+  CMI_TRY(reserve_for(e, plan, n));
+  ShootArgs a = shoot_args(e, plan, seed, iteration, first_packet, 0, n,
+                           nullptr);
+  CMI_TRY(order_packets(e, plan, a, n, nullptr));
+  uint32_t *dkeys = nullptr;
+  if (out_keys) {
+    HIP_TRY(hipMalloc(&dkeys, sizeof(uint32_t) * n));
+    const KeyArgs k = key_args(e, plan, a, n, nullptr);
+    order_probe_kernel<<<grid_blocks(e, (int64_t)n, 8), CMI_BLOCK, 0,
+                         e->stream>>>(k, a.order, dkeys);
+  }
+  hipError_t err = hipGetLastError();
+  if (err == hipSuccess)
+    err = hipStreamSynchronize(e->stream);
+  if (err == hipSuccess && out_ids)
+    err = hipMemcpy(out_ids, a.order, sizeof(uint32_t) * n,
+                    hipMemcpyDeviceToHost);
+  if (err == hipSuccess && out_keys)
+    err = hipMemcpy(out_keys, dkeys, sizeof(uint32_t) * n,
+                    hipMemcpyDeviceToHost);
+  (void)hipFree(dkeys);
+  HIP_TRY(err);
+  return CMI_GPU_OK;
+}
+
 int cmi_gpu_shoot_flights(cmi_gpu_engine *e, uint32_t seed, uint32_t iteration,
                           uint64_t first_packet, const void *flights,
                           uint64_t n_flights) {
diff --git a/cmacionize_amd/csrc/kernels.h b/cmacionize_amd/csrc/kernels.h
--- a/cmacionize_amd/csrc/kernels.h
+++ b/cmacionize_amd/csrc/kernels.h
@@ -2509,54 +2509,65 @@
   direction_key_batches(a);
 }
 
+__device__ __forceinline__ uint32_t direction_key_of(const KeyArgs &a,
+                                                     const PacketOrigin &from,
+                                                     uint64_t i,
+                                                     uint32_t &id_out) {
+  const uint32_t lo_bits = a.dir_bits - a.dir_hi_bits;
+  PacketRng rng;
+  const uint64_t id = a.select ? (uint64_t)a.select[i] : i;
+  rng.init(a.seed, a.iteration, a.first_packet + id);
+  uint32_t src;
+  const uint32_t origin = from.draw(a.model, rng, src);
+  if (origin != 0) {
+    (void)rng.next();
+    (void)rng.next();
+    if (a.model.continuous_type == 1)
+      (void)rng.next();
+  }
+  const double u_cost = rng.next();
+  const double u_phi = rng.next();
+  const uint32_t ic = (uint32_t)(u_cost * 2048.);
+  const uint32_t ip = (uint32_t)(u_phi * 2048.);
+  const uint32_t morton =
+      (spread_bits_11(ic) | (spread_bits_11(ip) << 1)) >> (22u - a.dir_bits);
+  uint32_t tau_class = 0;
+  if (a.tau_bits != 0) {
+    if (!a.full_ions) {
+      (void)sample_source_spectrum(a.model, rng, origin);
+      const double u_tau = rng.next();
+      tau_class = (uint32_t)(u_tau * (double)(1u << a.tau_bits));
+    } else {
+      const double nu = sample_source_spectrum(a.model, rng, origin);
+      const double tau = -log(rng.next());
+      const float sigma = approximate_opacity_cross_section(a.model, nu);
+      const float range = (float)(tau * a.sigma_ref) / sigma;
+      const int octave = (int)floorf(log2f(range)) + (1 << (a.tau_bits - 1));
+      const int top = (1 << a.tau_bits) - 1;
+      tau_class = (uint32_t)(octave < 0 ? 0 : (octave > top ? top : octave));
+    }
+  }
+  const uint32_t hi = morton >> lo_bits;
+  const uint32_t lo = morton & ((1u << lo_bits) - 1u);
+  id_out = (uint32_t)id;
+  return ((src & a.source_mask) << (a.dir_bits + a.tau_bits)) |
+         (hi << (a.tau_bits + lo_bits)) |
+         (key_class_field(a, hi, tau_class) << lo_bits) | lo;
+}
+
 __global__ void __launch_bounds__(CMI_BLOCK, 5)
     direction_key_kernel(const KeyArgs a) {
   const uint64_t stride = (uint64_t)gridDim.x * blockDim.x;
-  const uint32_t lo_bits = a.dir_bits - a.dir_hi_bits;
   const PacketOrigin from(a.model);
   for (uint64_t i = (uint64_t)blockIdx.x * blockDim.x + threadIdx.x;
        i < a.n_packets; i += stride) {
-    PacketRng rng;
-    const uint64_t id = a.select ? (uint64_t)a.select[i] : i;
-    rng.init(a.seed, a.iteration, a.first_packet + id);
-    uint32_t src;
-    const uint32_t origin = from.draw(a.model, rng, src);
-    if (origin != 0) {
-      (void)rng.next();
-      (void)rng.next();
-      if (a.model.continuous_type == 1)
-        (void)rng.next();
-    }
-    const double u_cost = rng.next();
-    const double u_phi = rng.next();
-    const uint32_t ic = (uint32_t)(u_cost * 2048.);
-    const uint32_t ip = (uint32_t)(u_phi * 2048.);
-    const uint32_t morton =
-        (spread_bits_11(ic) | (spread_bits_11(ip) << 1)) >> (22u - a.dir_bits);
-    uint32_t tau_class = 0;
-    if (a.tau_bits != 0) {
-      if (!a.full_ions) {
-        (void)sample_source_spectrum(a.model, rng, origin);
-        const double u_tau = rng.next();
-        tau_class = (uint32_t)(u_tau * (double)(1u << a.tau_bits));
-      } else {
-        const double nu = sample_source_spectrum(a.model, rng, origin);
-        const double tau = -log(rng.next());
-        const float sigma = approximate_opacity_cross_section(a.model, nu);
-        const float range = (float)(tau * a.sigma_ref) / sigma;
-        const int octave = (int)floorf(log2f(range)) + (1 << (a.tau_bits - 1));
-        const int top = (1 << a.tau_bits) - 1;
-        tau_class = (uint32_t)(octave < 0 ? 0 : (octave > top ? top : octave));
-      }
-    }
-    const uint32_t hi = morton >> lo_bits;
-    const uint32_t lo = morton & ((1u << lo_bits) - 1u);
-    a.keys[i] = ((src & a.source_mask) << (a.dir_bits + a.tau_bits)) |
-                (hi << (a.tau_bits + lo_bits)) |
-                (key_class_field(a, hi, tau_class) << lo_bits) | lo;
-    a.ids[i] = (uint32_t)id;
-  }
-}
+    uint32_t id;
+    a.keys[i] = direction_key_of(a, from, i, id);
+    a.ids[i] = id;
+  }
+}
+
+#include "packet_order.h"
 
 
 struct UpdateArgs {
diff --git a/cmacionize_amd/csrc/packet_order.h b/cmacionize_amd/csrc/packet_order.h
--- /dev/null
+++ b/cmacionize_amd/csrc/packet_order.h
@@ -0,0 +1,306 @@
+#ifndef CMI_PACKET_ORDER_H
+#define CMI_PACKET_ORDER_H
+
+#include "packet_order_plan.h"
+
+#ifndef CMI_BUCKET_THREADS
+#define CMI_BUCKET_THREADS 512
+#endif
+#ifndef CMI_BUCKET_PER_THREAD
+#define CMI_BUCKET_PER_THREAD 8
+#endif
+#define CMI_BUCKET_TILE (CMI_BUCKET_THREADS * CMI_BUCKET_PER_THREAD)
+#define CMI_BUCKET_MAX (1 << CMI_BUCKET_LEVEL_BITS)
+#define CMI_BUCKET_REGION_CURSOR_STRIDE 32
+#define CMI_BUCKET_LEAF_THREADS 256
+#define CMI_BUCKET_LEAF_PER_THREAD                                             \
+  (CMI_BUCKET_LEAF_PAIRS / CMI_BUCKET_LEAF_THREADS)
+#define CMI_BUCKET_SCAN_THREADS 1024
+
+struct BucketArgs {
+  uint32_t n;
+  uint32_t key_bits, bits1, bits2, rem_bits;
+  uint32_t region_cap, leaf_cap;
+  uint2 *regions;
+  uint2 *leaves;
+  uint32_t *order;
+  uint32_t *region_cursor, *leaf_cursor, *overflow_cursor;
+  uint32_t *leaf_offset;
+  uint32_t *ordered;
+};
+
+struct BucketTileShared {
+  uint32_t count[CMI_BUCKET_MAX], start[CMI_BUCKET_MAX], base[CMI_BUCKET_MAX],
+      room[CMI_BUCKET_MAX], overflow_at[CMI_BUCKET_MAX];
+  uint2 stage[CMI_BUCKET_TILE];
+};
+
+__device__ __forceinline__ void bucket_scan_256(const uint32_t *count,
+                                                uint32_t *start, uint32_t nb) {
+  if (threadIdx.x < 64) {
+    uint32_t c[4], total = 0;
+#pragma unroll
+    for (int q = 0; q < 4; ++q) {
+      const uint32_t bkt = 4u * threadIdx.x + q;
+      c[q] = bkt < nb ? count[bkt] : 0u;
+      total += c[q];
+    }
+    uint32_t incl = total;
+#pragma unroll
+    for (int off = 1; off < 64; off <<= 1) {
+      const uint32_t below = __shfl_up(incl, off, 64);
+      if ((int)threadIdx.x >= off)
+        incl += below;
+    }
+    uint32_t at = incl - total;
+#pragma unroll
+    for (int q = 0; q < 4; ++q) {
+      const uint32_t bkt = 4u * threadIdx.x + q;
+      if (bkt < nb)
+        start[bkt] = at;
+      at += c[q];
+    }
+  }
+}
+
+__device__ __forceinline__ void
+bucket_scatter_tile(BucketTileShared &s,
+                    const uint32_t (&key)[CMI_BUCKET_PER_THREAD],
+                    const uint32_t (&id)[CMI_BUCKET_PER_THREAD], uint32_t m,
+                    uint32_t shift, uint32_t nb, uint32_t keep,
+                    uint32_t *cursor, uint32_t cursor_stride, uint32_t cap,
+                    uint2 *dest, const BucketArgs &a) {
+  const uint32_t mask = nb - 1u;
+  for (uint32_t d = threadIdx.x; d < nb; d += CMI_BUCKET_THREADS)
+    s.count[d] = 0;
+  __syncthreads();
+  uint32_t rank[CMI_BUCKET_PER_THREAD];
+#pragma unroll
+  for (int k = 0; k < CMI_BUCKET_PER_THREAD; ++k) {
+    rank[k] = 0;
+    if ((uint32_t)k * CMI_BUCKET_THREADS + threadIdx.x < m)
+      rank[k] = atomicAdd(&s.count[(key[k] >> shift) & mask], 1u);
+  }
+  __syncthreads();
+  for (uint32_t d = threadIdx.x; d < nb; d += CMI_BUCKET_THREADS) {
+    const uint32_t cnt = s.count[d];
+    const uint32_t base =
+        cnt != 0 ? atomicAdd(&cursor[d * cursor_stride], cnt) : 0u;
+    const uint32_t left = base < cap ? cap - base : 0u;
+    const uint32_t room = cnt < left ? cnt : left;
+    s.base[d] = base;
+    s.room[d] = room;
+    s.overflow_at[d] =
+        cnt != room ? atomicAdd(a.overflow_cursor, cnt - room) : 0u;
+  }
+  bucket_scan_256(s.count, s.start, nb);
+  __syncthreads();
+#pragma unroll
+  for (int k = 0; k < CMI_BUCKET_PER_THREAD; ++k)
+    if ((uint32_t)k * CMI_BUCKET_THREADS + threadIdx.x < m) {
+      const uint32_t pos = s.start[(key[k] >> shift) & mask] + rank[k];
+      if (pos < CMI_BUCKET_TILE)
+        s.stage[pos] = make_uint2(key[k], id[k]);
+    }
+  __syncthreads();
+  for (uint32_t j = threadIdx.x; j < m; j += CMI_BUCKET_THREADS) {
+    const uint2 pair = s.stage[j];
+    const uint32_t d = (pair.x >> shift) & mask;
+    const uint32_t r = j - s.start[d];
+    if (r < s.room[d]) {
+      const uint32_t slot = s.base[d] + r;
+      if (slot < cap)
+        dest[(uint64_t)d * cap + slot] = make_uint2(pair.x & keep, pair.y);
+    } else {
+      const uint32_t o = s.overflow_at[d] + (r - s.room[d]);
+      if (o < a.n)
+        a.order[a.n - 1u - o] = pair.y;
+    }
+  }
+}
+
+__global__ void __launch_bounds__(CMI_BUCKET_THREADS)
+    bucket_key_kernel(const KeyArgs a, const BucketArgs b) {
+  __shared__ BucketTileShared s;
+  const PacketOrigin from(a.model);
+  const uint32_t ntiles = (b.n + CMI_BUCKET_TILE - 1u) / CMI_BUCKET_TILE;
+  for (uint32_t tile = blockIdx.x; tile < ntiles; tile += gridDim.x) {
+    const uint32_t first = tile * CMI_BUCKET_TILE;
+    const uint32_t m =
+        b.n - first < CMI_BUCKET_TILE ? b.n - first : CMI_BUCKET_TILE;
+#pragma unroll 1
+    for (uint32_t local = threadIdx.x; local < m;
+         local += CMI_BUCKET_THREADS) {
+      uint32_t id;
+      const uint32_t key = direction_key_of(a, from, (uint64_t)first + local, id);
+      s.stage[local] = make_uint2(key, id);
+    }
+    uint32_t key[CMI_BUCKET_PER_THREAD], id[CMI_BUCKET_PER_THREAD];
+#pragma unroll
+    for (int k = 0; k < CMI_BUCKET_PER_THREAD; ++k) {
+      const uint32_t local = (uint32_t)k * CMI_BUCKET_THREADS + threadIdx.x;
+      const uint2 pair = local < m ? s.stage[local] : make_uint2(0u, 0u);
+      key[k] = pair.x;
+      id[k] = pair.y;
+    }
+    bucket_scatter_tile(s, key, id, m, b.key_bits - b.bits1, 1u << b.bits1,
+                        0xffffffffu, b.region_cursor,
+                        CMI_BUCKET_REGION_CURSOR_STRIDE, b.region_cap,
+                        b.regions, b);
+    __syncthreads();
+  }
+}
+
+__global__ void __launch_bounds__(CMI_BUCKET_THREADS)
+    bucket_split_kernel(const BucketArgs b) {
+  __shared__ BucketTileShared s;
+  const uint32_t region = blockIdx.y;
+  const uint32_t sent =
+      b.region_cursor[region * CMI_BUCKET_REGION_CURSOR_STRIDE];
+  const uint32_t held = sent < b.region_cap ? sent : b.region_cap;
+  const uint64_t first = (uint64_t)blockIdx.x * CMI_BUCKET_TILE;
+  if (first >= held)
+    return;
+  const uint32_t m = held - first < CMI_BUCKET_TILE ? (uint32_t)(held - first)
+                                                    : CMI_BUCKET_TILE;
+  const uint2 *from = b.regions + (uint64_t)region * b.region_cap + first;
+  uint32_t key[CMI_BUCKET_PER_THREAD], id[CMI_BUCKET_PER_THREAD];
+#pragma unroll
+  for (int k = 0; k < CMI_BUCKET_PER_THREAD; ++k) {
+    const uint32_t local = (uint32_t)k * CMI_BUCKET_THREADS + threadIdx.x;
+    const uint2 pair = local < m ? from[local] : make_uint2(0u, 0u);
+    key[k] = pair.x;
+    id[k] = pair.y;
+  }
+  const uint64_t leaf0 = (uint64_t)region << b.bits2;
+  bucket_scatter_tile(s, key, id, m, b.rem_bits, 1u << b.bits2,
+                      (1u << b.rem_bits) - 1u, b.leaf_cursor + leaf0, 1u,
+                      b.leaf_cap, b.leaves + leaf0 * b.leaf_cap, b);
+}
+
+__device__ __forceinline__ uint32_t bucket_leaf_held(const BucketArgs &b,
+                                                     uint32_t leaf,
+                                                     uint32_t nleaves) {
+  if (leaf >= nleaves)
+    return 0u;
+  const uint32_t sent = b.leaf_cursor[leaf];
+  return sent < b.leaf_cap ? sent : b.leaf_cap;
+}
+
+__global__ void __launch_bounds__(CMI_BUCKET_SCAN_THREADS)
+    bucket_offsets_kernel(const BucketArgs b) {
+  constexpr uint32_t WAVES = CMI_BUCKET_SCAN_THREADS / 64;
+  __shared__ uint32_t wave_ahead[WAVES], wave_total[WAVES];
+  const uint32_t nleaves = 1u << (b.bits1 + b.bits2);
+  const uint32_t lane = threadIdx.x & 63u, wave = threadIdx.x >> 6;
+  uint32_t ahead = 0;
+#pragma unroll 8
+  for (uint32_t c = 0; c < blockIdx.x; ++c)
+    ahead += bucket_leaf_held(b, c * CMI_BUCKET_SCAN_THREADS + threadIdx.x,
+                              nleaves);
+  const uint32_t leaf = blockIdx.x * CMI_BUCKET_SCAN_THREADS + threadIdx.x;
+  const uint32_t mine = bucket_leaf_held(b, leaf, nleaves);
+  uint32_t incl = mine;
+#pragma unroll
+  for (int off = 1; off < 64; off <<= 1) {
+    const uint32_t below = __shfl_up(incl, off, 64);
+    const uint32_t more = __shfl_xor(ahead, off, 64);
+    if ((int)lane >= off)
+      incl += below;
+    ahead += more;
+  }
+  if (lane == 63) {
+    wave_total[wave] = incl;
+    wave_ahead[wave] = ahead;
+  }
+  __syncthreads();
+  uint32_t at = incl - mine, all = 0;
+  for (uint32_t w = 0; w < WAVES; ++w) {
+    at += wave_ahead[w];
+    if (w < wave)
+      at += wave_total[w];
+    all += wave_ahead[w] + wave_total[w];
+  }
+  if (leaf < nleaves)
+    b.leaf_offset[leaf] = at;
+  if (threadIdx.x == 0 && blockIdx.x == gridDim.x - 1)
+    *b.ordered = all;
+}
+
+__global__ void __launch_bounds__(CMI_BUCKET_LEAF_THREADS)
+    bucket_leaf_kernel(const BucketArgs b) {
+  __shared__ uint32_t s_count[CMI_BUCKET_MAX], s_start[CMI_BUCKET_MAX];
+  __shared__ uint32_t s_binned[CMI_BUCKET_LEAF_PAIRS];
+  __shared__ uint32_t s_sorted[CMI_BUCKET_LEAF_PAIRS];
+  const uint32_t leaf = blockIdx.x;
+  const uint32_t room =
+      b.leaf_cap < CMI_BUCKET_LEAF_PAIRS ? b.leaf_cap : CMI_BUCKET_LEAF_PAIRS;
+  const uint2 *from = b.leaves + (uint64_t)leaf * b.leaf_cap;
+  uint2 pair[CMI_BUCKET_LEAF_PER_THREAD];
+#pragma unroll
+  for (int k = 0; k < CMI_BUCKET_LEAF_PER_THREAD; ++k) {
+    const uint32_t j = (uint32_t)k * CMI_BUCKET_LEAF_THREADS + threadIdx.x;
+    pair[k] = j < room ? from[j] : make_uint2(0u, 0u);
+  }
+  const uint32_t sent = b.leaf_cursor[leaf];
+  const uint32_t held = sent < room ? sent : room;
+  if (held == 0)
+    return;
+  const uint32_t offset = b.leaf_offset[leaf];
+  const uint32_t nb = 1u << b.rem_bits, mask = nb - 1u;
+  for (uint32_t d = threadIdx.x; d < nb; d += CMI_BUCKET_LEAF_THREADS)
+    s_count[d] = 0;
+  __syncthreads();
+  uint32_t rank[CMI_BUCKET_LEAF_PER_THREAD];
+#pragma unroll
+  for (int k = 0; k < CMI_BUCKET_LEAF_PER_THREAD; ++k) {
+    const uint32_t j = (uint32_t)k * CMI_BUCKET_LEAF_THREADS + threadIdx.x;
+    pair[k].x &= mask;
+    rank[k] = j < held ? atomicAdd(&s_count[pair[k].x], 1u) : 0u;
+  }
+  __syncthreads();
+  bucket_scan_256(s_count, s_start, nb);
+  __syncthreads();
+#pragma unroll
+  for (int k = 0; k < CMI_BUCKET_LEAF_PER_THREAD; ++k) {
+    const uint32_t j = (uint32_t)k * CMI_BUCKET_LEAF_THREADS + threadIdx.x;
+    if (j < held) {
+      const uint32_t pos = s_start[pair[k].x] + rank[k];
+      if (pos < CMI_BUCKET_LEAF_PAIRS)
+        s_binned[pos] = pair[k].y;
+    }
+  }
+  __syncthreads();
+#pragma unroll
+  for (int k = 0; k < CMI_BUCKET_LEAF_PER_THREAD; ++k) {
+    const uint32_t j = (uint32_t)k * CMI_BUCKET_LEAF_THREADS + threadIdx.x;
+    if (j < held) {
+      const uint32_t begin = s_start[pair[k].x];
+      const uint32_t end = begin + s_count[pair[k].x];
+      uint32_t smaller = 0;
+      for (uint32_t i = begin; i < end && i < CMI_BUCKET_LEAF_PAIRS; ++i)
+        smaller += s_binned[i] < pair[k].y ? 1u : 0u;
+      if (begin + smaller < CMI_BUCKET_LEAF_PAIRS)
+        s_sorted[begin + smaller] = pair[k].y;
+    }
+  }
+  __syncthreads();
+  for (uint32_t j = threadIdx.x; j < held; j += CMI_BUCKET_LEAF_THREADS)
+    if ((uint64_t)offset + j < b.n)
+      b.order[offset + j] = s_sorted[j];
+}
+
+__global__ void order_probe_kernel(const KeyArgs a, const uint32_t *order,
+                                   uint32_t *keys) {
+  const uint64_t stride = (uint64_t)gridDim.x * blockDim.x;
+  const PacketOrigin from(a.model);
+  for (uint64_t j = (uint64_t)blockIdx.x * blockDim.x + threadIdx.x;
+       j < a.n_packets; j += stride) {
+    const uint32_t id = order[j];
+    uint32_t unused;
+    keys[j] = id < a.n_packets ? direction_key_of(a, from, id, unused)
+                               : 0xffffffffu;
+  }
+}
+
+#endif
diff --git a/cmacionize_amd/csrc/packet_order_plan.h b/cmacionize_amd/csrc/packet_order_plan.h
--- /dev/null
+++ b/cmacionize_amd/csrc/packet_order_plan.h
@@ -0,0 +1,70 @@
+#ifndef CMI_PACKET_ORDER_PLAN_H
+#define CMI_PACKET_ORDER_PLAN_H
+
+#include <cmath>
+#include <cstdint>
+
+#define CMI_BUCKET_LEVEL_BITS 8
+#define CMI_BUCKET_REM_BITS 8
+#define CMI_BUCKET_LEAF_PAIRS 2560
+#define CMI_BUCKET_TIE_PAIRS 256
+#define CMI_BUCKET_SIGMAS_REGION 12.
+#define CMI_BUCKET_SIGMAS_LEAF 9.
+
+struct BucketPlan {
+  int take;
+  int bits1, bits2;
+  int rem_bits;
+  uint32_t region_cap, leaf_cap;
+  uint64_t region_begin, region_words, leaf_begin, total_words;
+};
+
+static inline uint64_t cmi_bucket_capacity(double mean, double sigmas,
+                                           int slack_permille) {
+  const double cap = slack_permille >= 0
+                         ? mean * (1000. + (double)slack_permille) / 1000.
+                         : mean + sigmas * std::sqrt(mean) + 8.;
+  const uint64_t c = (uint64_t)std::ceil(cap);
+  return c < 1 ? 1 : c;
+}
+
+static inline BucketPlan cmi_bucket_plan(uint64_t n, int key_bits, int bits1,
+                                         int bits2, int slack_permille,
+                                         uint64_t min_packets) {
+  BucketPlan b = {};
+  if (n == 0 || n < min_packets || n >= ((uint64_t)1 << 31) || key_bits < 0 ||
+      key_bits > 32)
+    return b;
+  int total = 0;
+  while (total < 2 * CMI_BUCKET_LEVEL_BITS && (n >> (total + 1)) >= 1024)
+    ++total;
+  if (total > key_bits)
+    total = key_bits;
+  b.bits1 = bits1 >= 0 ? bits1 : (total + 1) / 2;
+  b.bits2 = bits2 >= 0 ? bits2 : total - (total + 1) / 2;
+  if (b.bits1 > CMI_BUCKET_LEVEL_BITS || b.bits2 > CMI_BUCKET_LEVEL_BITS)
+    return b;
+  b.rem_bits = key_bits - b.bits1 - b.bits2;
+  if (b.rem_bits < 0 || b.rem_bits > CMI_BUCKET_REM_BITS)
+    return b;
+  const double mean1 = (double)n / (double)((uint64_t)1 << b.bits1);
+  const double mean2 = mean1 / (double)((uint64_t)1 << b.bits2);
+  if (mean2 / (double)(1u << b.rem_bits) > (double)CMI_BUCKET_TIE_PAIRS)
+    return b;
+  const uint64_t cap1 =
+      cmi_bucket_capacity(mean1, CMI_BUCKET_SIGMAS_REGION, slack_permille);
+  const uint64_t cap2 =
+      cmi_bucket_capacity(mean2, CMI_BUCKET_SIGMAS_LEAF, slack_permille);
+  if (cap2 > CMI_BUCKET_LEAF_PAIRS || cap1 >= ((uint64_t)1 << 31))
+    return b;
+  b.region_cap = (uint32_t)cap1;
+  b.leaf_cap = (uint32_t)cap2;
+  b.region_words = 2 * (cap1 << b.bits1);
+  b.region_begin = (n + 63) & ~(uint64_t)63;
+  b.leaf_begin = (b.region_begin + b.region_words + 63) & ~(uint64_t)63;
+  b.total_words = b.leaf_begin + 2 * (cap2 << (b.bits1 + b.bits2));
+  b.take = 1;
+  return b;
+}
+
+#endif
diff --git a/cmacionize_amd/csrc/transport_driver.h b/cmacionize_amd/csrc/transport_driver.h
--- a/cmacionize_amd/csrc/transport_driver.h
+++ b/cmacionize_amd/csrc/transport_driver.h
@@ -1,17 +1,24 @@
 #ifndef CMI_TRANSPORT_DRIVER_H
 #define CMI_TRANSPORT_DRIVER_H
 
-static int reserve_sort_buffers(cmi_gpu_engine *e, uint64_t n) {
-  if (e->sort_capacity >= n)
+static int reserve_sort_buffers(cmi_gpu_engine *e, uint64_t n,
+                                uint64_t words = 0) {
+  if (e->sort_capacity >= n && e->sort_block_words >= words)
     return CMI_GPU_OK;
+  if (n < e->sort_capacity)
+    n = e->sort_capacity;
+  if (words < 4 * n)
+    words = 4 * n;
   HIP_TRY(hipStreamSynchronize(e->stream));
   (void)hipFree(e->sort_keys[0]);
   (void)hipFree(e->sort_temp);
   e->sort_keys[0] = nullptr;
   e->sort_temp = nullptr;
   e->sort_capacity = 0;
+  e->sort_block_words = 0;
   uint32_t *block = nullptr;
-  HIP_TRY(hipMalloc(&block, sizeof(uint32_t) * 4 * n));
+  HIP_TRY(hipMalloc(&block, sizeof(uint32_t) * words));
+  e->sort_block_words = words;
   e->sort_keys[0] = block;
   e->sort_keys[1] = block + n;
   e->sort_ids[0] = block + 2 * n;
@@ -216,6 +223,7 @@
   uint32_t tau_bits, source_bits, dir_bits;
   int key_bits;
   double sigma_ref;
+  bool bucket_order;
   TileKernel tile_kernel;
   int tile_threads, tile_blocks_per_cu;
 };
@@ -410,14 +418,30 @@
       p.dir_bits = 22u - over;
   }
   p.key_bits = (int)(p.dir_bits + p.tau_bits + p.source_bits);
-  return CMI_GPU_OK;
+  p.bucket_order = p.sorted && !p.select_mode && p.first != FIRST_PRE &&
+                   !e->full_ions && tune.bucket_order;
+  return CMI_GPU_OK;
+}
+
+static BucketPlan bucket_plan_of(const cmi_gpu_engine *e, const LaunchPlan &p,
+                                 uint64_t n) {
+  if (!p.bucket_order) {
+    BucketPlan none = {};
+    return none;
+  }
+  return cmi_bucket_plan(n, p.key_bits, e->tune.bucket_bits1,
+                         e->tune.bucket_bits2, e->tune.bucket_slack_permille,
+                         e->tune.bucket_min_packets);
 }
 
 static int reserve_for(cmi_gpu_engine *e, const LaunchPlan &p, uint64_t cap) {
   if (!e->span_cursor)
     HIP_TRY(hipMalloc(&e->span_cursor, sizeof(uint32_t) * CMI_SPAN_CURSORS));
   if (p.sorted || p.tiles)
-    CMI_TRY(reserve_sort_buffers(e, cap));
+    CMI_TRY(reserve_sort_buffers(e, cap, bucket_plan_of(e, p, cap).total_words));
+  if (p.bucket_order && !e->bucket_meta)
+    HIP_TRY(hipMalloc(&e->bucket_meta,
+                      sizeof(uint32_t) * CMI_BUCKET_META_WORDS));
   if (p.passes)
     CMI_TRY(reserve_queues(e, cap));
   if (p.tiles)
@@ -565,8 +589,15 @@
   return CMI_GPU_OK;
 }
 
-static int order_packets(cmi_gpu_engine *e, const LaunchPlan &p, ShootArgs &a,
-                         uint64_t nids, const uint32_t *select) {
+enum OrderPath {
+  ORDER_NONE = CMI_GPU_ORDER_NONE,
+  ORDER_RADIX = CMI_GPU_ORDER_RADIX,
+  ORDER_BUCKET = CMI_GPU_ORDER_BUCKET
+};
+
+static KeyArgs key_args(const cmi_gpu_engine *e, const LaunchPlan &p,
+                        const ShootArgs &a, uint64_t nids,
+                        const uint32_t *select) {
   const uint64_t n = a.n_packets;
   KeyArgs k;
   k.model = e->model;
@@ -593,6 +624,69 @@
            (per_source >> (k.dir_hi_bits + 1u)) >= per_bin)
       ++k.dir_hi_bits;
   }
+  k.keys = nullptr;
+  k.ids = nullptr;
+  k.pre_rows = nullptr;
+  k.select = select;
+  return k;
+}
+
+static int order_packets_bucket(cmi_gpu_engine *e, const BucketPlan &bp,
+                                const KeyArgs &k, ShootArgs &a) {
+  uint32_t *block = e->sort_keys[0];
+  uint32_t *meta = e->bucket_meta;
+  BucketArgs b;
+  b.n = (uint32_t)a.n_packets;
+  b.key_bits = (uint32_t)(bp.bits1 + bp.bits2 + bp.rem_bits);
+  b.bits1 = (uint32_t)bp.bits1;
+  b.bits2 = (uint32_t)bp.bits2;
+  b.rem_bits = (uint32_t)bp.rem_bits;
+  b.region_cap = bp.region_cap;
+  b.leaf_cap = bp.leaf_cap;
+  b.order = block;
+  b.regions = reinterpret_cast<uint2 *>(block + bp.region_begin);
+  b.leaves = reinterpret_cast<uint2 *>(block + bp.leaf_begin);
+  b.region_cursor = meta;
+  b.leaf_cursor = meta + CMI_BUCKET_META_LEAF_CURSOR;
+  b.overflow_cursor = meta + CMI_BUCKET_META_OVERFLOW;
+  b.ordered = meta + CMI_BUCKET_META_ORDERED;
+  b.leaf_offset = meta + CMI_BUCKET_META_LEAF_OFFSET;
+  HIP_TRY(hipMemsetAsync(meta, 0, sizeof(uint32_t) * CMI_BUCKET_META_CLEARED,
+                         e->stream));
+  const uint32_t ntiles =
+      (b.n + CMI_BUCKET_TILE - 1u) / CMI_BUCKET_TILE;
+  int per_cu = 0;
+  CMI_TRY(blocks_per_cu_of(bucket_key_kernel, CMI_BUCKET_THREADS, 8, per_cu));
+  const uint32_t most = (uint32_t)(e->num_cu * per_cu);
+  bucket_key_kernel<<<ntiles < most ? ntiles : most, CMI_BUCKET_THREADS, 0,
+                      e->stream>>>(k, b);
+  const uint32_t region_tiles =
+      (b.region_cap + CMI_BUCKET_TILE - 1u) / CMI_BUCKET_TILE;
+  bucket_split_kernel<<<dim3(region_tiles, 1u << b.bits1), CMI_BUCKET_THREADS,
+                        0, e->stream>>>(b);
+  const uint32_t nleaves = 1u << (b.bits1 + b.bits2);
+  bucket_offsets_kernel<<<(nleaves + CMI_BUCKET_SCAN_THREADS - 1u) /
+                              CMI_BUCKET_SCAN_THREADS,
+                          CMI_BUCKET_SCAN_THREADS, 0, e->stream>>>(b);
+  bucket_leaf_kernel<<<nleaves, CMI_BUCKET_LEAF_THREADS, 0, e->stream>>>(b);
+  HIP_TRY(hipGetLastError());
+  a.order = b.order;
+  return CMI_GPU_OK;
+}
+
+static int order_packets(cmi_gpu_engine *e, const LaunchPlan &p, ShootArgs &a,
+                         uint64_t nids, const uint32_t *select) {
+  const uint64_t n = a.n_packets;
+  KeyArgs k = key_args(e, p, a, nids, select);
+  const BucketPlan bp = bucket_plan_of(e, p, n);
+  if (bp.take && !select && e->bucket_meta &&
+      bp.total_words <= e->sort_block_words) {
+    e->last_order_path = ORDER_BUCKET;
+    e->last_bucket_bits[0] = bp.bits1;
+    e->last_bucket_bits[1] = bp.bits2;
+    return order_packets_bucket(e, bp, k, a);
+  }
+  e->last_order_path = ORDER_RADIX;
   k.keys = e->sort_keys[0];
   k.ids = e->sort_ids[0];
   k.pre_rows = p.first == FIRST_PRE ? e->tile_rows[1].weights : nullptr;
@@ -601,7 +695,6 @@
                  sizeof(double) * CMI_NACC * (size_t)nids));
     k.pre_rows = e->select_rows;
   }
-  k.select = select;
   a.pre_rows = k.pre_rows;
   if (k.pre_rows)
     emission_key_kernel<<<grid_blocks(e, (int64_t)n, 8), CMI_BLOCK, 0,
@@ -1029,6 +1122,8 @@
   if (!flights) {
     e->last_first_build = (int32_t)plan.first;
     e->last_pad_uniform = plan.pad_uniform;
+    if (!plan.sorted)
+      e->last_order_path = ORDER_NONE;
   }
   CMI_TRY(publish_escape(e, plan.tracking));
   const uint64_t max_launch = e->tune.max_packets_per_launch;
diff --git a/cmacionize_amd/engine.py b/cmacionize_amd/engine.py
--- a/cmacionize_amd/engine.py
+++ b/cmacionize_amd/engine.py
@@ -19,6 +19,7 @@
 FIELD_HEATING = 30
 
 REEMIT_NONE, REEMIT_PHYSICAL, REEMIT_FIXED = 0, 1, 2
+ORDER_NONE, ORDER_RADIX, ORDER_BUCKET = 0, 1, 2
 CONTINUOUS_NONE, CONTINUOUS_ISOTROPIC, CONTINUOUS_PLANAR = 0, 1, 2
 ROLE_SOURCE, ROLE_CONTINUOUS = 0, 1
 TABLE_LINEAR, TABLE_LOGLOG = 0, 1
@@ -139,6 +140,7 @@
     "cmi_gpu_set_escape_tally", "cmi_gpu_reset_escape_tally",
     "cmi_gpu_download_escape_tally", "cmi_gpu_escape_pixels",
     "cmi_gpu_cross_sections", "cmi_gpu_get_transport_plan",
+    "cmi_gpu_get_order_plan", "cmi_gpu_order_packets",
 ]
 
 EMISSION_LINES = [
@@ -303,6 +305,12 @@
     if hasattr(L, "cmi_gpu_get_transport_plan"):
         L.cmi_gpu_get_transport_plan.argtypes = [vp] + 2 * [
             C.POINTER(C.c_int32)]
+    if hasattr(L, "cmi_gpu_get_order_plan"):
+        L.cmi_gpu_get_order_plan.argtypes = [vp] + 3 * [
+            C.POINTER(C.c_int32)] + [C.POINTER(C.c_uint64)]
+        L.cmi_gpu_order_packets.argtypes = [
+            vp, C.c_uint32, C.c_uint32, C.c_uint64, C.c_uint64,
+            C.POINTER(C.c_uint32), C.POINTER(C.c_uint32)]
     L.cmi_gpu_reset_grid.argtypes = [vp]
     L.cmi_gpu_shoot.argtypes = [vp, C.c_uint32, C.c_uint32, C.c_uint64,
                                 C.c_uint64]
@@ -921,6 +929,14 @@
             self._h, C.byref(first), C.byref(uniform)))
         return first.value, bool(uniform.value)
 
+    def order_plan(self):
+        path, b1, b2 = C.c_int32(), C.c_int32(), C.c_int32()
+        overflow = C.c_uint64()
+        self._check(self._lib.cmi_gpu_get_order_plan(
+            self._h, C.byref(path), C.byref(b1), C.byref(b2),
+            C.byref(overflow)))
+        return path.value, b1.value, b2.value, overflow.value
+
     def field_tensor(self, field):
         import torch
         ptr = self.field_device_pointer(field)
@@ -1159,6 +1175,15 @@
             self._h, seed, iteration, first_packet, n, _p(pos), _p(dirn),
             _p(nu), _p(sig), _p(tau)))
         return pos, dirn, nu, sig, tau
+
+    def order_packets(self, seed, iteration, first_packet, n):
+        ids = np.empty(n, dtype=np.uint32)
+        keys = np.empty(n, dtype=np.uint32)
+        u32 = C.POINTER(C.c_uint32)
+        self._check(self._lib.cmi_gpu_order_packets(
+            self._h, seed, iteration, first_packet, n,
+            ids.ctypes.data_as(u32), keys.ctypes.data_as(u32)))
+        return ids, keys
 
     def trace_packets(self, position, direction, tau, sigma_H, sigma_He_corr,
                       max_steps):
diff --git a/include/cmi_gpu.h b/include/cmi_gpu.h
--- a/include/cmi_gpu.h
+++ b/include/cmi_gpu.h
@@ -142,6 +142,12 @@
                              int32_t *deferral_allowed);
 int cmi_gpu_get_transport_plan(cmi_gpu_engine *engine, int32_t *first_build,
                                int32_t *uniform_weight);
+#define CMI_GPU_ORDER_NONE 0
+#define CMI_GPU_ORDER_RADIX 1
+#define CMI_GPU_ORDER_BUCKET 2
+int cmi_gpu_get_order_plan(cmi_gpu_engine *engine, int32_t *path,
+                           int32_t *bits1, int32_t *bits2,
+                           uint64_t *overflow);
 int cmi_gpu_accumulator_layout(cmi_gpu_engine *engine, int64_t *field_stride,
                                int64_t *cell_stride);
 
@@ -250,6 +256,10 @@
                          double *frequency, double *cross_sections,
                          double *tau);
 
+int cmi_gpu_order_packets(cmi_gpu_engine *engine, uint32_t seed,
+                          uint32_t iteration, uint64_t first_packet,
+                          uint64_t n, uint32_t *out_ids, uint32_t *out_keys);
+
 int cmi_gpu_trace_packets(cmi_gpu_engine *engine, uint64_t n,
                           const double *position, const double *direction,
                           const double *tau, const double *sigma_H,
```

Measured after the change: 4.311 billion, median of 6. +4.8%, better.
